# iacopo97/Multimodal-SAM-Adapter

Hardware: AMD Instinct MI355X
Metric: images/sec encoder fwd @1024x1024 RGB+LiDAR ViT-L (higher is better)
Workload: dtype split-operand MFMA: fp16 hi + e5m2 cross terms (h8c / h8 planes, ViT / interaction / up-conv GEMMs) fp16 hi/lo pairs x3 (TwinConvNeXt: f3 planes) and bf16 hi/lo x3 (neck, head); attention blocks with the rel-pos terms fused: every contraction on one fp16 MFMA (q, k, v, P rounded to fp16) in the bloc

## Files before the change

### include/mmsa.h

```cpp
#ifndef MMSA_H
#define MMSA_H
#include <stddef.h>
#include <stdint.h>
#ifdef __cplusplus
extern "C" {
#endif

#ifdef MMSA_BUILDING_LIBRARY
typedef hipStream_t mmsa_stream_t;
#else
typedef void* mmsa_stream_t;
#endif

#include "mmsa_version.h"
int mmsa_version(void);
const char* mmsa_last_error(void);

int mmsa_debug_poison_lds(unsigned pattern, mmsa_stream_t stream);
int mmsa_event_create(void** ev);
int mmsa_event_record(void* ev, mmsa_stream_t stream);
int mmsa_event_elapsed_ms(void* start, void* stop, float* ms);
int mmsa_event_destroy(void* ev);

enum { MMSA_ACT_NONE = 0, MMSA_ACT_GELU = 1, MMSA_ACT_RELU = 2, MMSA_ACT_RELU6 = 3, MMSA_ACT_HSWISH = 4, MMSA_ACT_SIGMOID = 5 };

enum { MMSA_DT_F32 = 0, MMSA_DT_F16 = 1, MMSA_DT_F64 = 2 };

enum { MMSA_FMT_B3 = 0, MMSA_FMT_H8 = 1, MMSA_FMT_H8C = 2, MMSA_FMT_F3 = 3, MMSA_FMT_W8 = 4  };

int mmsa_ms_deform_attn_forward(const void* value, const int64_t* spatial_shapes, const int64_t* level_start_index,
                                const void* sampling_loc, const void* attn_weight, void* out, int batch,
                                int spatial_size, int num_heads, int channels, int num_levels, int num_query,
                                int num_point, int im2col_step, int dtype, mmsa_stream_t stream);

int mmsa_ms_deform_attn_backward(const void* value, const int64_t* spatial_shapes, const int64_t* level_start_index,
                                 const void* sampling_loc, const void* attn_weight, const void* grad_output,
                                 void* grad_value, void* grad_sampling_loc, void* grad_attn_weight, int batch,
                                 int spatial_size, int num_heads, int channels, int num_levels, int num_query,
                                 int num_point, int im2col_step, int dtype, mmsa_stream_t stream);

int mmsa_msda_fused(const float* value, const int64_t* spatial_shapes, const int64_t* level_start_index,
                    const float* raw, long ldraw, const float* ref_points, float* out, long ldo,
                    uint16_t* out_planes, long ldop , int out_fmt , int batch,
                    int spatial_size, int num_heads, int channels, int num_levels, int num_query, int num_point,
                    float* clamp_max , mmsa_stream_t stream);

int mmsa_msda_fused_planes(const uint16_t* value_planes, long ldvp, int lo_bytes, const int64_t* spatial_shapes, const int64_t* level_start_index,
                           const float* raw, long ldraw, const float* ref_points, float* out, long ldo,
                           uint16_t* out_planes, long ldop, int out_fmt, int batch,
                           int spatial_size, int num_heads, int channels, int num_levels, int num_query, int num_point,
                           float* clamp_max, mmsa_stream_t stream);

int mmsa_rowstats_finalize(const float* rowstats, int rows, int strips, int D, float eps, float* mean_rstd, mmsa_stream_t stream);

int mmsa_zero_bytes(void* p, size_t bytes, mmsa_stream_t stream);
int mmsa_gemm_split3(const float* A, const uint16_t* Ap, long lda, long strideA,
                     const uint16_t* Wp, long strideW,
                     const float* bias, long strideBias, const float* colscale, const float* resid, long ldr,
                     long strideR, int resid_mod, float beta, float* C, long ldc, long strideC,
                     uint16_t* Cp, long ldcp, long strideCp, int M, int N, int K,
                     int batch, int act, float alpha, int out_mode, int ps_H, int ps_W, int ps_C, int fmt, int cp_fmt,
                     int max_grid, float* rowstats_out, const float* rownorm_mean_rstd, const float* rownorm_colsum, int flavour,
                     float* clamp_max , mmsa_stream_t stream);

int mmsa_convnext_mlp_fused(const uint16_t* Ap, long lda, long strideA, const uint16_t* W1p, long strideW1, const uint16_t* W2p,
                            long strideW2, const float* b1, const float* b2, const float* gamma, float* x, long ldx, long strideX,
                            int M, int C, int batch, int max_grid, int fmt,
                            float* clamp_max , mmsa_stream_t stream);

int mmsa_split_planes(const float* src, long ld, int rows, int cols, int cols_pad, uint16_t* planes, int kind,
                      float* clamp_max , mmsa_stream_t stream);

int mmsa_attention(const float* qkv, long ldq, const float* qkv_bias, const float* rp, float* out, long ldo, int B,
                   int H, int W, int heads, int head_dim, int window_size, float scale, mmsa_stream_t stream);
int mmsa_attention_planes(const uint16_t* qkv_planes, long ldq, const uint16_t* bias_planes, const float* rp,
                          uint16_t* out_planes, long ldo, int B, int H, int W, int heads, int head_dim,
                          int window_size, float scale, int out_fmt ,
                          int v_fmt ,
                          float* max_abs_logit , mmsa_stream_t stream);

int mmsa_relpos_bias(const float* qkv, long ldq, const float* Rh, const float* Rw, float* rp, int B, int H, int W,
                     int heads, int head_dim, int window_size, mmsa_stream_t stream);
int mmsa_relpos_bias_planes(const uint16_t* qkv_planes, long ldq, const float* Rh, const float* Rw,
                            float* rp, int B, int H, int W, int heads, int head_dim, int window_size, mmsa_stream_t stream);

int mmsa_layernorm_rows(const float* x, long ldx, const float* w, const float* b, float eps, float* y, long ldy,
                        float* y2, long ldy2, uint16_t* y_planes, long ldp ,
                        int rows, int C, int map_mode, int map_H, int map_W, int group_rows, long w_gstride, long y_gcol,
                        int y_wrap, int plane_fmt , float* clamp_max ,
                        mmsa_stream_t stream);

int mmsa_colstats(const float* x, long ldx, long strideB, const float* wrow, int B, int HW, int C, double* out,
                  int out_is_zero , mmsa_stream_t stream);

int mmsa_ffrm_finalize(const double* stats, int B, int HW, int C, float mean_w, float mean_b, const float* Wc,
                       const float* gn_w, const float* gn_b, float* mean_o, float* rstd_o, float* mult_o,
                       float* scratch , mmsa_stream_t stream);
int mmsa_lnhw_apply(const float* x, long ldx, const float* mean, const float* rstd, const float* mult, const float* w,
                    const float* bias, float* y, long ldy, int B, int HW, int C, mmsa_stream_t stream);

int mmsa_dwconv_nhwc(const float* x, long ldx, long xstrideB, const float* w, const float* bias, float* y, long ldy,
                     long ystrideB, uint16_t* y_planes, long ldp, long pstrideB , int planes_fmt ,
                     int B, int H, int W, int C, int k, int act,
                     int imgs_per_group ,
                     float* rowstats ,
                     float* clamp_max , mmsa_stream_t stream);
int mmsa_gconv_nhwc(const float* x, long ldx, const float* w, const float* bias, float* y, long ldy, int B, int H,
                    int W, int G, int cin_g, int cout_g, int k, int act, mmsa_stream_t stream);
int mmsa_gfe_qkv_conv(const float* x, long ldx, const float* w, float* y, long ldy, int B, int H, int W, int G, int cin_g, int cout_g,
                      int* covered, mmsa_stream_t stream);
int mmsa_dwpair_gate(const float* x, long ldx, const float* w, float* y, long ldy, uint16_t* y_planes, long ldp, int B, int H,
                     int W, int C, mmsa_stream_t stream);
int mmsa_im2col_nchw(const float* x, int B, int Ctot, int c0, int Cin, int H, int W, int p, float* out, int Kpad,
                     mmsa_stream_t stream);

long mmsa_gram_tn_scratch_bytes(int B, int P, int c);
int mmsa_gram_tn(const float* X, long ldx, const float* Y, long ldy, long strideB, double* G , int B, int P, int c,
                 int nblk, void* scratch, long scratch_bytes, mmsa_stream_t stream);
int mmsa_chanattn_build(const double* G, const double* sq, long sq_strideB, const double* sk, long sk_strideB,
                        const float* temp, const float* Wp, uint16_t* planes , int B, int c, int cpad,
                        int heads, mmsa_stream_t stream);
int mmsa_gffm_build(const double* E, uint16_t* x_planes, uint16_t* y_planes , int B, int c,
                    int cpad, mmsa_stream_t stream);
int mmsa_gelu_gate(const float* x, long ldx, float* y, long ldy, long rows, int C, mmsa_stream_t stream);
int mmsa_pool_hw(const float* z, long ldz, float* out, long ldo, int B, int H, int W, int C, mmsa_stream_t stream);
int mmsa_ca_apply(const float* z, long ldz, const float* att, long lda, float* out, long ldo,
                  uint16_t* out_planes, long ldp , int B, int H, int W, int C, mmsa_stream_t stream);

int mmsa_tail_fuse(const float* cmap, long ldc, long cstrideB, const float* xtok, long ldx, const float* bn_scale,
                   const float* bn_shift, float* out, uint16_t* out_planes , long ldp,
                   int B, int Hc, int Wc, int Hx, int Wx, int C, mmsa_stream_t stream);

int mmsa_global_attention_planes(const uint16_t* qkv_planes, long ldq, const uint16_t* bias_planes, const uint16_t* relpos_planes,
                                 uint16_t* out_planes, long ldo, int B, int H, int W, int heads, int head_dim, float scale,
                                 int out_fmt , int v_fmt ,
                                 float* max_abs_logit , mmsa_stream_t stream);

int mmsa_window_attention_planes(const uint16_t* qkv_planes, long ldq, const uint16_t* bias_planes,
                                 const uint16_t* relpos_planes, const uint16_t* selector, uint16_t* out_planes, long ldo, int B, int H, int W,
                                 int heads, int head_dim, int window_size, float scale, int out_fmt ,
                                 int v_fmt , float* max_abs_logit , mmsa_stream_t stream);

int mmsa_nchw_to_planes(const float* src, long strideB, uint16_t* planes, long ldp, int B, int C, long HW,
                        mmsa_stream_t stream);
int mmsa_head_fuse(const float* z0, const float* z1, int H1, int W1, const float* z2, int H2, int W2, const float* z3,
                   int H3, int W3, long ld, const float* bn_scale, const float* bn_shift, uint16_t* planes, long ldp,
                   float* out32, long ldo, int B, int H, int W, int C, int act, mmsa_stream_t stream);
int mmsa_tokens_to_nchw(const float* src, long ld, float* dst, int B, long HW, int C, mmsa_stream_t stream);

int mmsa_bilinear_accum_nchw(const float* src, long src_strideB, int B, int C, int hs, int ws, float* dst, int Hd, int Wd, int y0, int x0,
                             int hc, int wc, float* count, int accumulate, mmsa_stream_t stream);
int mmsa_div_count_nchw(float* x, const float* count, int B, int C, long HW, mmsa_stream_t stream);
int mmsa_argmax_nchw(const float* x, unsigned char* out, int B, int C, long HW, mmsa_stream_t stream);
int mmsa_crop_batch_nchw(const float* src, int B, int C, int H, int W, const int* windows, int n, float* dst, int hc, int wc,
                         mmsa_stream_t stream);
int mmsa_slide_argmax(const float* logits, int n, int C, int hs, int ws, const int* windows, unsigned char* out, int B, int H, int W,
                      int hc, int wc, int* uncovered, mmsa_stream_t stream);
int mmsa_slide_argmax_resized(const float* logits, int n, int C, int hs, int ws, const int* windows, unsigned char* out, int B, int H, int W,
                              int hc, int wc, int Hd, int Wd, int Hcut, int Wcut, int* uncovered, mmsa_stream_t stream);

int mmsa_softmax_flip_accum_nchw(const float* logits, float* acc, int B, int C, int H, int W, int flip, int accumulate, int finish_div, mmsa_stream_t stream);
int mmsa_aug_argmax(const float* const* logits, const int* views, int A, int C, const int* windows, const int* windows_host, int total,
                    unsigned char* out, int B, int Ho, int Wo, int* uncovered, mmsa_stream_t stream);

int mmsa_argmax_max_nchw(const float* x, unsigned char* out, float* maxval, int B, int C, long HW, mmsa_stream_t stream);
int mmsa_slide_argmax_conf(const float* logits, int n, int C, int hs, int ws, const int* windows, unsigned char* out, float* conf, int B, int H, int W,
                           int hc, int wc, int* uncovered, mmsa_stream_t stream);
int mmsa_slide_argmax_resized_conf(const float* logits, int n, int C, int hs, int ws, const int* windows, unsigned char* out, float* conf, int B, int H,
                                   int W, int hc, int wc, int Hd, int Wd, int Hcut, int Wcut, int* uncovered, mmsa_stream_t stream);
int mmsa_aug_argmax_conf(const float* const* logits, const int* views, int A, int C, const int* windows, const int* windows_host, int total,
                         unsigned char* out, float* conf, int B, int Ho, int Wo, int* uncovered, mmsa_stream_t stream);

enum { MMSA_PRE_U8 = 0, MMSA_PRE_F32 = 1 };
int mmsa_preprocess_nhwc(const void* src0, int dtype0, const void* src1, int dtype1, int B, int Hs, int Ws, const float* mean,
                         const float* sinv, const int* div255, const int* swap, const float* pad_val, float* dst, int H, int W,
                         mmsa_stream_t stream);
int mmsa_preprocess_crops(const void* src0, int dtype0, const void* src1, int dtype1, int B, int Hs, int Ws, const float* mean,
                          const float* sinv, const int* div255, const int* swap, const float* pad_val, int H, int W, const int* windows,
                          int n, float* dst, int hc, int wc, mmsa_stream_t stream);
int mmsa_preprocess_resize_nhwc(const void* src0, int dtype0, const void* src1, int dtype1, int B, int Hs, int Ws, const float* mean,
                                const float* sinv, const int* div255, const int* swap, const float* pad_val, float* dst, int H, int W,
                                int Hr, int Wr, const int* xofs, const void* xcoef, const int* yofs, const void* ycoef, int fixed_point,
                                mmsa_stream_t stream);
int mmsa_preprocess_resize_crops(const void* src0, int dtype0, const void* src1, int dtype1, int B, int Hs, int Ws, const float* mean,
                                 const float* sinv, const int* div255, const int* swap, const float* pad_val, int H, int W, const int* windows,
                                 int n, float* dst, int hc, int wc, int Hr, int Wr, const int* xofs, const void* xcoef, const int* yofs,
                                 const void* ycoef, int fixed_point, mmsa_stream_t stream);

int mmsa_eval_confusion_u8(const unsigned char* pred, const unsigned char* label, int B, int H, int W, int Hl, int Wl, const unsigned char* lut,
                           int C, const int* ymap, const int* xmap, const int* slots, int n_slots, int64_t* counts, mmsa_stream_t stream);
int mmsa_slide_argmax_eval(const float* logits, int n, int C, int hs, int ws, const int* windows, unsigned char* out, int B, int H, int W,
                           int hc, int wc, int* uncovered, const unsigned char* label, int Hl, int Wl, const unsigned char* lut, const int* ymap,
                           const int* xmap, const int* slots, int n_slots, int64_t* counts, mmsa_stream_t stream);

int mmsa_eval_calibration(const unsigned char* pred, const float* conf, const unsigned char* label, int B, int H, int W, int Hl, int Wl,
                          const unsigned char* lut, int C, const int* ymap, const int* xmap, const int* slots, int n_slots, int bins, int64_t* cal,
                          mmsa_stream_t stream);

int mmsa_eval_selective(const unsigned char* pred, const float* conf, const unsigned char* label, int B, int H, int W, int Hl, int Wl,
                        const unsigned char* lut, int C, const int* ymap, const int* xmap, const int* slots, int n_slots, int bins, int64_t* counts,
                        mmsa_stream_t stream);
int mmsa_abstain_u8(const unsigned char* pred, const float* conf, long n, int bins, int min_bin, unsigned char* out, mmsa_stream_t stream);

int mmsa_slide_argmax_conf_t(const float* logits, int n, int C, int hs, int ws, const int* windows, unsigned char* out, float* conf, int B, int H, int W,
                             int hc, int wc, int* uncovered, float inv_temperature, mmsa_stream_t stream);
int mmsa_slide_argmax_resized_conf_t(const float* logits, int n, int C, int hs, int ws, const int* windows, unsigned char* out, float* conf, int B, int H,
                                     int W, int hc, int wc, int Hd, int Wd, int Hcut, int Wcut, int* uncovered, float inv_temperature, mmsa_stream_t stream);
int mmsa_softmax_flip_accum_nchw_t(const float* logits, float* acc, int B, int C, int H, int W, int flip, int accumulate, int finish_div,
                                   float inv_temperature, mmsa_stream_t stream);
int mmsa_temperature_sweep_nchw(const float* logits, const unsigned char* label, int B, int C, int H, int W, int Hl, int Wl, const unsigned char* lut,
                                const int* ymap, const int* xmap, const int* slots, int n_slots, const float* inv_temperatures, int J, int bins,
                                int64_t* sweep, mmsa_stream_t stream);

int mmsa_render_u8(const unsigned char* pred, long pred_image_stride, long pred_row_stride, int B, int h, int w, const unsigned* palette, int npal,
                   int palette_reverse, const unsigned char* src, int Hs, int Ws, int src_reverse, double opacity, double one_minus_opacity,
                   unsigned char* out, mmsa_stream_t stream);
int mmsa_render_denorm_f32(const unsigned char* pred, long pred_image_stride, long pred_row_stride, int B, int h, int w, const unsigned* palette, int npal,
                           int palette_reverse, const float* src, int Cs, int Hs, int Ws, const float* mean, const float* std, int to_rgb, int mul255,
                           double opacity, double one_minus_opacity, unsigned char* out, mmsa_stream_t stream);

#ifdef __cplusplus
}
#endif
#endif
```

### multimodal-sam-adapter_amd/csrc/gemm_h8c.hip

```cpp
#include "common.h"
#include "gemm_h8c_shared.h"

#define HC_H_UNIT 49152
#define HC_L_UNIT 24576
#define HC_LDS_H(i_) ((i_) * HC_H_UNIT)
#define HC_LDS_L(i_) (2 * HC_H_UNIT + (i_) * (HC_L_UNIT + 16384))
#define HC_LDS_TOTAL (2 * HC_H_UNIT + 2 * HC_L_UNIT + 16384)

#ifdef HC_EPI_STAMP
__device__ unsigned long long g_hc_estamps[8 * 16];
extern "C" int mmsa_debug_epi_stamps(unsigned long long* host_out) { return (int)hipMemcpyFromSymbol(host_out, HIP_SYMBOL(g_hc_estamps), sizeof(g_hc_estamps)); }
#define EPI_STAMP(i_) { if (estamp_on_) { __builtin_amdgcn_sched_barrier(0); et_[i_] = __builtin_readcyclecounter(); __builtin_amdgcn_sched_barrier(0); } }
#define EPI_STAMP_WAIT() { if (estamp_on_) asm volatile("s_waitcnt vmcnt(0)" ::: "memory"); }
#else
#define EPI_STAMP(i_)
#define EPI_STAMP_WAIT()
#endif
template <bool GEN, int ACT>
__global__ __launch_bounds__(512, 1) void gemm_h8c_kernel(GemmV2Args a) {
  constexpr bool PP = true;
  constexpr bool EPI_UNROLL = ACT >= 0;
  constexpr int V2_BM = 256;
  constexpr int V2_NST = 3;
  extern __shared__ __attribute__((aligned(16))) unsigned char smem[];
  const int tid = threadIdx.x, lane = tid & 63;
  const int wave = __builtin_amdgcn_readfirstlane(tid >> 6);
  const int wm = wave >> 1, wn = wave & 1, grp = wave >> 2;
  const int l15 = lane & 15, g = lane >> 4;
  const int K = a.K;
  const int np = K >> 6;
  const bool ni4 = true;
  const int swid = 64;
  const int G = gridDim.x;
  int rb = blockIdx.x;
  V2_XCD_REMAP(rb, G)
  const int my_tiles = (a.ntiles - rb + G - 1) / G;
  if (my_tiles <= 0) return;
  V2_SLACK_STAGGER(a, rb, G)
  const int total = my_tiles * np;

  H8C_DMA_LANE();
  const int lds_ha = wave * 32 * 128, lds_hw = 32768 + wave * 16 * 128;
  const int lds_la = wave * 2048, lds_lw = 16384 + wave * 1024;
  const unsigned ldaB = (unsigned)(a.lda * 2), ldwB = (unsigned)(a.ldw * 2);
  const unsigned K2 = (unsigned)K * 2u, K4 = (unsigned)K * 4u;
  H8C_A_LANE_HI();
  const unsigned LW_E = (unsigned)(drow >> 1) * ldwB + (unsigned)(drow & 1) * K2 + dpiece, LW_O = LW_E ^ 64u;
  H8C_A_LANE_LO();
  const unsigned LLW = (unsigned)drow * ldwB + K4 + lq;

  const unsigned char *hA, *hW, *lA, *lW;
  int h_m0 = 0, h_n0 = 0, l_m0 = 0, l_n0 = 0;
  bool h_edge = false, l_edge = false;
  int hp_tile = rb, hp_p = 0, hp_j = 0, lp_tile = rb, lp_p = 0, lp_j = 0;
#define HC_SET_H(t_)                                                                                        \
  { int bz_; H8C_TILE(t_, 256, bz_, h_m0, h_n0)                                                             \
    hA = reinterpret_cast<const unsigned char*>(a.Ap + (long)bz_ * a.strideA + (long)(h_m0 >> 1) * a.lda);  \
    hW = reinterpret_cast<const unsigned char*>(a.Wp + (long)bz_ * a.strideW + (long)(h_n0 >> 1) * a.ldw);  \
    h_edge = h_m0 + 256 > a.M || h_n0 + 128 > a.N; }
#define HC_SET_L(t_)                                                                                        \
  { int bz_; H8C_TILE(t_, 256, bz_, l_m0, l_n0)                                                             \
    lA = reinterpret_cast<const unsigned char*>(a.Ap + (long)bz_ * a.strideA + (long)(l_m0 >> 1) * a.lda);  \
    lW = reinterpret_cast<const unsigned char*>(a.Wp + (long)bz_ * a.strideW + (long)(l_n0 >> 1) * a.ldw);  \
    l_edge = l_m0 + 256 > a.M || l_n0 + 128 > a.N; }
  HC_SET_H(hp_tile) HC_SET_L(lp_tile)
#define HC_H_ISSUE_FAST()                                                                                   \
  { unsigned char* d_ = smem + HC_LDS_H(hp_j & 1);                                                          \
    const unsigned char* sa_ = hA + (long)hp_p * 128 + (unsigned long)((unsigned)(wave * 16) * ldaB);       \
    const unsigned char* sw_ = hW + (long)hp_p * 128 + (unsigned long)((unsigned)(wave * 8) * ldwB);        \
    H8C_A_HI_FAST(sa_, d_)                                                                                  \
    GLDS16(sw_ + LW_E, d_ + lds_hw); GLDS16(sw_ + 4u * ldwB + LW_O, d_ + lds_hw + 1024); }
#define HC_L_ISSUE_FAST()                                                                                   \
  { unsigned char* d_ = smem + HC_LDS_L(lp_j & 1);                                                          \
    const unsigned char* sa_ = lA + (long)lp_p * 128 + (unsigned long)((unsigned)(wave * 16) * ldaB);       \
    const unsigned char* sw_ = lW + (long)lp_p * 128 + (unsigned long)((unsigned)(wave * 8) * ldwB);        \
    H8C_A_LO_FAST(sa_, d_)                                                                                  \
    GLDS16(sw_ + LLW, d_ + lds_lw); }
#define HC_H_ISSUE()                                                                                        \
  if (!h_edge) HC_H_ISSUE_FAST() else {                                                                     \
    unsigned char* d_ = smem + HC_LDS_H(hp_j & 1); const long ko_ = (long)hp_p * 128;                       \
    const int ab_ = h_m0 + wave * 32 + drow, wb_ = h_n0 + wave * 16 + drow;                                  \
    H8C_A_HI_EDGE(hA + ko_, ab_, h_m0, d_)                                                                  \
    GLDS16(hW + ko_ + (unsigned long)(H8C_HOFF(min(wb_, a.N - 1), h_n0, ldwB) + dpiece), d_ + lds_hw);       \
    GLDS16(hW + ko_ + (unsigned long)(H8C_HOFF(min(wb_ + 8, a.N - 1), h_n0, ldwB) + (dpiece ^ 64)), d_ + lds_hw + 1024); }
#define HC_H_ADVANCE() { ++hp_j; if (++hp_p == np) { hp_p = 0; hp_tile += G; if (hp_j < total) HC_SET_H(hp_tile) } }
#define HC_L_ISSUE()                                                                                        \
  if (!l_edge) HC_L_ISSUE_FAST() else {                                                                     \
    unsigned char* d_ = smem + HC_LDS_L(lp_j & 1); const long ko_ = (long)lp_p * 128;                       \
    const int aj_ = (l_m0 >> 1) + wave * 16 + drow, wj_ = (l_n0 >> 1) + wave * 8 + drow;                     \
    GLDS16(lA + ko_ + (unsigned long)H8C_A_LO_OFF(aj_, l_m0), d_ + lds_la);                                  \
    GLDS16(lA + ko_ + (unsigned long)H8C_A_LO_OFF(aj_ + 8, l_m0), d_ + lds_la + 1024);                       \
    GLDS16(lW + ko_ + (unsigned long)((unsigned)(min(wj_, (a.N - 1) >> 1) - (l_n0 >> 1)) * ldwB + K4 + lq), d_ + lds_lw); }
#define HC_L_ADVANCE() { ++lp_j; if (++lp_p == np) { lp_p = 0; lp_tile += G; if (lp_j < total) HC_SET_L(lp_tile) } }

  H8C_FRAG_HI();
  const int fha = (wm * 64) * 128, fhw = 32768 + (wn * 64) * 128;
  H8C_FRAG_LO();
  const int fla = (wm * 4) * 1024 + lo_off, flw = 16384 + (wn * 4) * 1024 + lo_off;

  f32x4 acc[4][4];
  H8C_ZERO_ACC()
  h8c_u4 ah0[4], ah1[4], wh0[4], wh1[4];
  mx_v8i opA[4], opW[4];

  HC_H_ISSUE() HC_H_ADVANCE()
  if (total > 1) { HC_H_ISSUE() HC_H_ADVANCE() }
  HC_L_ISSUE() HC_L_ADVANCE()
  H8C_WAIT(0);
  __builtin_amdgcn_s_barrier();

  int j = 0, tile = rb, nowait = 0;
#define HC_PAIR(FAST_)                                                                                                \
  {                                                                                                                   \
    const unsigned char* hb = smem + HC_LDS_H(j & 1);                                                                 \
    const unsigned char* lb = smem + HC_LDS_L(j & 1);                                                                 \
    const bool last = !(FAST_) && p == np - 1;                                                                        \
    const bool tail = !(FAST_) && j + 2 >= total;                                                                     \
    const bool skipw = !(FAST_) && nowait > 0;                                                                        \
                                                                                     \
    _Pragma("unroll") for (int i = 0; i < 4; ++i) {                                                                   \
      ah0[i] = *reinterpret_cast<const h8c_u4*>(hb + fha + i * 2048 + frag0);                                         \
      ah1[i] = *reinterpret_cast<const h8c_u4*>(hb + fha + i * 2048 + frag1);                                         \
    }                                                                                                                 \
    _Pragma("unroll") for (int i = 0; i < 4; ++i) {                                                                   \
      wh0[i] = *reinterpret_cast<const h8c_u4*>(hb + fhw + i * 2048 + frag0);                                         \
      wh1[i] = *reinterpret_cast<const h8c_u4*>(hb + fhw + i * 2048 + frag1);                                         \
    }                                                                                                                 \
    H8C_SB();                                                                                                         \
    const bool do_l = (FAST_) || lp_j < total;                                                                        \
    if (FAST_) { HC_L_ISSUE_FAST() } else if (do_l) { HC_L_ISSUE() }                                                   \
    H8C_SB();                                                                                                         \
    asm volatile("s_waitcnt lgkmcnt(0)" ::: "memory");                                                                \
    if (FAST_) H8C_WAIT(9); else if (tail) H8C_WAIT(0); else if (!skipw) H8C_WAIT(9);                                 \
    H8C_BAR()                                                                                                         \
     \
    _Pragma("unroll") for (int ni = 0; ni < 4; ++ni)                                                                  \
      _Pragma("unroll") for (int mi = 0; mi < 4; ++mi)                                                                \
        acc[ni][mi] = __builtin_amdgcn_mfma_f32_16x16x32_f16(__builtin_bit_cast(mx_h8, wh0[ni]), __builtin_bit_cast(mx_h8, ah0[mi]), acc[ni][mi], 0, 0, 0); \
    H8C_SB();                                                                                                         \
    _Pragma("unroll") for (int ni = 0; ni < 4; ++ni)                                                                  \
      _Pragma("unroll") for (int mi = 0; mi < 4; ++mi)                                                                \
        acc[ni][mi] = __builtin_amdgcn_mfma_f32_16x16x32_f16(__builtin_bit_cast(mx_h8, wh1[ni]), __builtin_bit_cast(mx_h8, ah1[mi]), acc[ni][mi], 0, 0, 0); \
    H8C_SB();                                                                                                         \
    if (FAST_) H8C_WAIT(9); else if (tail) H8C_WAIT(0); else if (!skipw) H8C_WAIT(9);                                 \
    H8C_BAR()                                                                                                         \
                                                             \
    H8C_FP8_TUPLES(lb)                                                                                                \
    H8C_SB();                                                                                                         \
    const bool do_h = (FAST_) || hp_j < total;                                                                        \
    if (FAST_) { HC_H_ISSUE_FAST() } else if (do_h) { HC_H_ISSUE() }                                                   \
    H8C_SB();                                                                                                         \
    asm volatile("s_waitcnt lgkmcnt(0)" ::: "memory");                                                                \
    if (FAST_) H8C_WAIT(9); else if (tail) H8C_WAIT(0); else if (!skipw) H8C_WAIT(9);                                 \
    H8C_BAR()                                                                                                         \
                                              \
    _Pragma("unroll") for (int ni = 0; ni < 4; ++ni)                                                                  \
      _Pragma("unroll") for (int mi = 0; mi < 4; ++mi)                                                                \
        acc[ni][mi] = __builtin_amdgcn_mfma_scale_f32_16x16x128_f8f6f4(opW[ni], opA[mi], acc[ni][mi], 1, 1, 0, MMSA_H8_MFMA_SCALE, 0, 0x7f7f7f7f); \
    H8C_SB();                                                                                                         \
     \
     \
    if (FAST_) { ++lp_j; ++lp_p; ++hp_j; ++hp_p; } else { if (do_l) HC_L_ADVANCE() if (do_h) HC_H_ADVANCE() }          \
    H8C_SB();                                                                                                         \
    if (FAST_) H8C_WAIT(9); else if (tail || last) H8C_WAIT(0); else if (!skipw) H8C_WAIT(9);                         \
    H8C_BAR()                                                                                                         \
    if (!(FAST_)) nowait = 0;                                                                                         \
    ++j;                                                                                                              \
  }

  for (int tdone = 0; tdone < my_tiles; ++tdone) {
    if (grp) H8C_BAR()
    bool interior;
    { int bz_, m0_, n0_; H8C_TILE(tile, 256, bz_, m0_, n0_) interior = m0_ + 256 <= a.M && n0_ + 128 <= a.N; }
    int p = 0;
    HC_PAIR(0)
    ++p;
    if (interior) {
#pragma unroll 1
      for (; p < np - 2; ++p) HC_PAIR(1)
      if (hp_p == np) { hp_p = 0; hp_tile += G; if (hp_j < total) HC_SET_H(hp_tile) }
    }
#pragma unroll 1
    for (; p < np; ++p) HC_PAIR(0)
    if (!grp) H8C_BAR()
    if (V2_DBG(a) == 2) H8C_NO_EPILOGUE() else {
#ifdef HC_EPI_STAMP
      unsigned long long et_[9] = {0, 0, 0, 0, 0, 0, 0, 0, 0};
      const bool estamp_on_ = blockIdx.x == 0 && tdone == 1;
#endif
      EPI_STAMP(0)
#define EPI_STAGING_BASE (smem + (((j - 1) & 1) ? 2 * HC_H_UNIT + HC_L_UNIT : 2 * HC_H_UNIT))
#include "gemm_v2_epilogue.inc"
      EPI_STAMP(7)
#ifdef HC_EPI_STAMP
      asm volatile("s_waitcnt lgkmcnt(0)" ::: "memory");
      H8C_BAR()
      EPI_STAMP(8)
      if (estamp_on_ && (threadIdx.x & 63) == 0) {
#pragma unroll
        for (int q_ = 0; q_ < 9; ++q_) g_hc_estamps[wave * 16 + q_] = et_[q_];
      }
#endif
    }
    asm volatile("s_waitcnt lgkmcnt(0)" ::: "memory");
    H8C_BAR()
    tile += G;
  }
}

int mmsa_gemm_h8c_dispatch(const GemmV2Args& a, int grid, bool gen, int act, hipStream_t stream) {
  static MmsaPerDevice per_dev_ = {};
  (void)mmsa_per_device(per_dev_, [] {
#define HC_ATTR(GEN_, ACT_) (void)hipFuncSetAttribute((const void*)gemm_h8c_kernel<GEN_, ACT_>, hipFuncAttributeMaxDynamicSharedMemorySize, HC_LDS_TOTAL);
    V2_EPI_TABLE(HC_ATTR)
#undef HC_ATTR
  });
#define HC_LAUNCH(GEN_, ACT_) if (v2_epi_serves(gen, act, GEN_, ACT_)) hipLaunchKernelGGL((gemm_h8c_kernel<GEN_, ACT_>), dim3(grid), dim3(512), HC_LDS_TOTAL, stream, a);
  V2_EPI_TABLE(HC_LAUNCH)
#undef HC_LAUNCH
  MMSA_CHECK_LAUNCH("gemm_split3(h8c)");
  return MMSA_OK;
}
```

### multimodal-sam-adapter_amd/csrc/gemm_v2.hip

```cpp
#include "common.h"
#include "gemm_v2_shared.h"
template <bool GEN, int ACT, bool PP, int NW, int FMT>
__global__ __launch_bounds__(NW * 64, NW == 4 ? 2 : 1) void gemm_v2_kernel(GemmV2Args a) {
  static_assert(NW == 8 || (NW == 4 && !PP), "4-wave workgroups run the in-phase main loop");
  static_assert(FMT == MMSA_FMT_B3 || (PP && NW == 8), "the h8 and f3 operand formats run on the ping-pong kernel");
  constexpr bool EPI_UNROLL = ACT >= 0;
  constexpr int V2_BM = NW * 32;
  constexpr int V2_A_BYTES = V2_BM * 128;
  constexpr int V2_STAGE = V2_A_BYTES + V2_W_BYTES;
  constexpr int V2_NST = NW == 8 ? 3 : 2;
  constexpr int WROWS = V2_BN / NW;
  constexpr int NDMA = 4 + WROWS / 8;
  extern __shared__ __attribute__((aligned(16))) unsigned char smem[];
  const int tid = threadIdx.x;
  const int lane = tid & 63;
  const int wave = __builtin_amdgcn_readfirstlane(tid >> 6);
  const int wm = wave >> 1, wn = wave & 1;
  const int grp = wave >> 2;
  const int l15 = lane & 15, g = lane >> 4;
  const int K = a.K;
  const int nk = K / V2_BK;

  const int G = gridDim.x;
  int rb = blockIdx.x;
  V2_XCD_REMAP(rb, G)
  const int my_tiles = (a.ntiles - rb + G - 1) / G;
  if (my_tiles <= 0) return;
  V2_SLACK_STAGGER(a, rb, G)
  CLK_SAMPLE(0)
  const int total = my_tiles * nk;

  const int drow = lane >> 3;
  const int dpiece = ((lane & 7) ^ (drow >> 1)) * 8;
  const int lds_a = wave * 32 * 128;
  const int lds_w = wave * WROWS * 128;
  const unsigned char *gA, *gW;
  unsigned oa0, oa1, oa2, oa3, ow0, ow1, ow2 = 0, ow3 = 0;
#define SA(i_, ko_) reinterpret_cast<const unsigned short*>(gA + (long)(ko_) * 2 + (unsigned long)oa##i_)
#define SW(i_, ko_) reinterpret_cast<const unsigned short*>(gW + (long)(ko_) * 2 + (unsigned long)ow##i_)

#define SET_TILE_SRC(tile_)                                                      \
  do {                                                                           \
    const int t_ = (tile_);                                                      \
    const int per_b_ = a.nbm * a.nbn;                                            \
    const int bz_ = t_ / per_b_;                                                 \
    const int r_ = t_ - bz_ * per_b_;                                            \
    int tmi_, tni_;                                                              \
    V2_TILE_MN(r_, tmi_, tni_);                                                  \
    const int m0_ = tmi_ * V2_BM, n0_ = tni_ * a.bn;                             \
    const int ab_ = m0_ + wave * 32 + drow, wb_ = n0_ + wave * WROWS + drow;     \
    gA = reinterpret_cast<const unsigned char*>(a.Ap + (long)bz_ * a.strideA + (long)m0_ * a.lda);  \
    gW = reinterpret_cast<const unsigned char*>(a.Wp + (long)bz_ * a.strideW + (long)n0_ * a.ldw);  \
    oa0 = (unsigned)((min(ab_, a.M - 1) - m0_) * (int)a.lda + dpiece) * 2u;           \
    oa1 = (unsigned)((min(ab_ + 8, a.M - 1) - m0_) * (int)a.lda + (dpiece ^ 32)) * 2u;  \
    oa2 = (unsigned)((min(ab_ + 16, a.M - 1) - m0_) * (int)a.lda + dpiece) * 2u;      \
    oa3 = (unsigned)((min(ab_ + 24, a.M - 1) - m0_) * (int)a.lda + (dpiece ^ 32)) * 2u; \
    ow0 = (unsigned)((min(wb_, a.N - 1) - n0_) * (int)a.ldw + dpiece) * 2u;           \
    ow1 = (unsigned)((min(wb_ + 8, a.N - 1) - n0_) * (int)a.ldw + (dpiece ^ 32)) * 2u;  \
    if constexpr (NW == 4) {                                                     \
      ow2 = (unsigned)((min(wb_ + 16, a.N - 1) - n0_) * (int)a.ldw + dpiece) * 2u;    \
      ow3 = (unsigned)((min(wb_ + 24, a.N - 1) - n0_) * (int)a.ldw + (dpiece ^ 32)) * 2u; \
    }                                                                            \
    if (V2_DBG(a) == 4 || V2_DBG(a) == 5) { oa1 = oa2 = oa3 = oa0; gW = gA; ow0 = ow1 = oa0; }    \
  } while (0)

#define ISSUE_DMA(kt_, st_)                                                       \
  do {                                                                            \
    unsigned char* sb_ = smem + (st_) * V2_STAGE;                                 \
    const int ko_ = V2_DBG(a) == 3 ? 0 : (kt_) * 64;    \
    GLDS16(SA(0, ko_), sb_ + lds_a);                                               \
    GLDS16(SA(1, ko_), sb_ + lds_a + 1024);                                        \
    GLDS16(SA(2, ko_), sb_ + lds_a + 2048);                                        \
    GLDS16(SA(3, ko_), sb_ + lds_a + 3072);                                        \
    GLDS16(SW(0, ko_), sb_ + V2_A_BYTES + lds_w);                                  \
    GLDS16(SW(1, ko_), sb_ + V2_A_BYTES + lds_w + 1024);                           \
    if constexpr (NW == 4) {                                                      \
      GLDS16(SW(2, ko_), sb_ + V2_A_BYTES + lds_w + 2048);                         \
      GLDS16(SW(3, ko_), sb_ + V2_A_BYTES + lds_w + 3072);                         \
    }                                                                             \
  } while (0)

  f32x4 acc[4][4];
  mx_v8i opA[4] = {}, opW[4] = {};
#pragma unroll
  for (int i = 0; i < 4; ++i)
#pragma unroll
    for (int j = 0; j < 4; ++j) acc[i][j] = (f32x4){0.f, 0.f, 0.f, 0.f};

  const int fslot = g ^ ((l15 >> 1) & 7);
  const int frag_hi = l15 * 128 + fslot * 16;
  const int frag_lo = l15 * 128 + (fslot ^ 4) * 16;
  const int fa = (wm * 64) * 128;
  const bool ni4 = a.bn == V2_BN;
  const int swid = ni4 ? 64 : 48;
  const int fw = V2_A_BYTES + (wn * swid) * 128;

  int pf_tile = rb, pf_kt = 0, pf_st = 0, pf_j = 0;
  SET_TILE_SRC(pf_tile);
#define PREFETCH_NEXT()                                     \
  do {                                                      \
    ISSUE_DMA(pf_kt, pf_st);                                \
    pf_st = pf_st == V2_NST - 1 ? 0 : pf_st + 1;            \
    ++pf_j;                                                 \
    if (++pf_kt == nk) {                                    \
      pf_kt = 0;                                            \
      pf_tile += G;                                         \
      if (pf_j < total) SET_TILE_SRC(pf_tile);              \
    }                                                       \
  } while (0)
  PREFETCH_NEXT();
  if (V2_NST == 3 && total > 1) PREFETCH_NEXT();

  int st = 0, tile = rb, nowait = 0, j = 0;
  if constexpr (PP) {
    if (total > 1) asm volatile("s_waitcnt vmcnt(6)" ::: "memory");
    else asm volatile("s_waitcnt vmcnt(0)" ::: "memory");
    __builtin_amdgcn_s_barrier();
  }

#define MX_SET(dst_, src_, par_)                                                                            \
  { const uint4 u_ = __builtin_bit_cast(uint4, src_);                                                       \
    if ((par_) == 0) { dst_[0] = (int)u_.x; dst_[1] = (int)u_.y; dst_[2] = (int)u_.z; dst_[3] = (int)u_.w; }  \
    else { dst_[4] = (int)u_.x; dst_[5] = (int)u_.y; dst_[6] = (int)u_.z; dst_[7] = (int)u_.w; } }
#define MFMA_FP8_ALL(NI4_, DEFER_)                                                                          \
  if constexpr (FMT == MMSA_FMT_H8) {                                                                       \
    if (MXPAR && V2_FP8_FIRST && !V2_EXP_NO_FP8) {                                                          \
      _Pragma("unroll") for (int ni = 0; ni < 4; ++ni)                                                      \
        if (ni < 3 || (NI4_)) {                                                                             \
          _Pragma("unroll") for (int mi = 0; mi < 4; ++mi)                                                  \
              acc[ni][mi] = __builtin_amdgcn_mfma_scale_f32_16x16x128_f8f6f4(opW[ni], opA[mi], acc[ni][mi], 1, 1, 0, MMSA_H8_MFMA_SCALE, 0, 0x7f7f7f7f); \
        }                                                                                                   \
      __builtin_amdgcn_sched_barrier(0);                                                                    \
    }                                                                                                       \
  }
#define MFMA_CHUNK(ni)                                                                                      \
  if constexpr (FMT == MMSA_FMT_H8) {                                                                       \
    _Pragma("unroll") for (int mi = 0; mi < 4; ++mi) {                                                      \
      acc[ni][mi] = __builtin_amdgcn_mfma_f32_16x16x32_f16(__builtin_bit_cast(mx_h8, wh[ni]), __builtin_bit_cast(mx_h8, ah[mi]), acc[ni][mi], 0, 0, 0); \
      if (MXPAR && !V2_FP8_FIRST && !V2_EXP_NO_FP8) acc[ni][mi] = __builtin_amdgcn_mfma_scale_f32_16x16x128_f8f6f4(opW[ni], opA[mi], acc[ni][mi], 1, 1, 0, MMSA_H8_MFMA_SCALE, 0, 0x7f7f7f7f); \
    }                                                                                                       \
  } else {                                                                                                  \
    _Pragma("unroll") for (int mi = 0; mi < 4; ++mi) {                                                      \
      if constexpr (FMT == MMSA_FMT_F3) {                    \
        acc[ni][mi] = __builtin_amdgcn_mfma_f32_16x16x32_f16(__builtin_bit_cast(mx_h8, wl[ni]), __builtin_bit_cast(mx_h8, ah[mi]), acc[ni][mi], 0, 0, 0); \
        acc[ni][mi] = __builtin_amdgcn_mfma_f32_16x16x32_f16(__builtin_bit_cast(mx_h8, wh[ni]), __builtin_bit_cast(mx_h8, al[mi]), acc[ni][mi], 0, 0, 0); \
        acc[ni][mi] = __builtin_amdgcn_mfma_f32_16x16x32_f16(__builtin_bit_cast(mx_h8, wh[ni]), __builtin_bit_cast(mx_h8, ah[mi]), acc[ni][mi], 0, 0, 0); \
      } else {                                                                                              \
      acc[ni][mi] = __builtin_amdgcn_mfma_f32_16x16x32_bf16(wl[ni], ah[mi], acc[ni][mi], 0, 0, 0);          \
      acc[ni][mi] = __builtin_amdgcn_mfma_f32_16x16x32_bf16(wh[ni], al[mi], acc[ni][mi], 0, 0, 0);          \
      acc[ni][mi] = __builtin_amdgcn_mfma_f32_16x16x32_bf16(wh[ni], ah[mi], acc[ni][mi], 0, 0, 0);          \
      }                                                                                                     \
    }                                                                                                       \
  }
#define K_STEP()                                                                                            \
  {                                                                                                         \
    if (nowait > 0) --nowait;                                                                               \
    else if (V2_NST == 3 && j + 1 < total) asm volatile("s_waitcnt vmcnt(6)" ::: "memory");                  \
    else asm volatile("s_waitcnt vmcnt(0)" ::: "memory");                                                   \
    __builtin_amdgcn_s_barrier();                                                                           \
    const bool do_pf = pf_j < total;                                                                        \
    unsigned char* pfb = smem + pf_st * V2_STAGE;                                                           \
    const int pko = V2_DBG(a) == 3 ? 0 : pf_kt * 64;                                                          \
    const unsigned char* base = smem + st * V2_STAGE;                                                       \
    bf16x8 ah[4], al[4], wh[4], wl[4];                                                                      \
    _Pragma("unroll") for (int i = 0; i < 4; ++i) {                                                         \
      ah[i] = *reinterpret_cast<const bf16x8*>(base + fa + i * 2048 + frag_hi);                             \
      al[i] = *reinterpret_cast<const bf16x8*>(base + fa + i * 2048 + frag_lo);                             \
    }                                                                                                       \
    _Pragma("unroll") for (int i = 0; i < 4; ++i) {                                                         \
      if (i < 3 || ni4) {                                                                                   \
        wh[i] = *reinterpret_cast<const bf16x8*>(base + fw + i * 2048 + frag_hi);                           \
        wl[i] = *reinterpret_cast<const bf16x8*>(base + fw + i * 2048 + frag_lo);                           \
      }                                                                                                     \
    }                                                                                                       \
    __builtin_amdgcn_sched_barrier(0);                                                                      \
    MFMA_CHUNK(0)                                                                                           \
    __builtin_amdgcn_sched_barrier(0);                                                                      \
    if (do_pf) { GLDS16(SA(0, pko), pfb + lds_a); GLDS16(SA(1, pko), pfb + lds_a + 1024); }                   \
    __builtin_amdgcn_sched_barrier(0);                                                                      \
    MFMA_CHUNK(1)                                                                                           \
    __builtin_amdgcn_sched_barrier(0);                                                                      \
    if (do_pf) { GLDS16(SA(2, pko), pfb + lds_a + 2048); GLDS16(SA(3, pko), pfb + lds_a + 3072); }            \
    __builtin_amdgcn_sched_barrier(0);                                                                      \
    MFMA_CHUNK(2)                                                                                           \
    __builtin_amdgcn_sched_barrier(0);                                                                      \
    if (do_pf) { GLDS16(SW(0, pko), pfb + V2_A_BYTES + lds_w); GLDS16(SW(1, pko), pfb + V2_A_BYTES + lds_w + 1024); } \
    if constexpr (NW == 4) { if (do_pf) { GLDS16(SW(2, pko), pfb + V2_A_BYTES + lds_w + 2048); GLDS16(SW(3, pko), pfb + V2_A_BYTES + lds_w + 3072); } } \
    __builtin_amdgcn_sched_barrier(0);                                                                      \
    if (ni4) { MFMA_CHUNK(3) }                                                                              \
    __builtin_amdgcn_sched_barrier(0);                                                                      \
    if (do_pf) {    \
      pf_st = pf_st == V2_NST - 1 ? 0 : pf_st + 1;                                                          \
      ++pf_j;                                                                                               \
      if (++pf_kt == nk) {                                                                                  \
        pf_kt = 0;                                                                                          \
        pf_tile += G;                                                                                       \
        if (pf_j < total) SET_TILE_SRC(pf_tile);                                                            \
      }                                                                                                     \
    }                                                                                                       \
    st = st == V2_NST - 1 ? 0 : st + 1;                                                                     \
    ++j;                                                                                                    \
  }

#ifdef V2_STAMP
#define STAMP_DECL() unsigned long long tt[9]; const bool stamp_on = blockIdx.x == 0 && tdone == 0 && kt >= 8 && kt < 12;
#define STAMP_STORE() if (stamp_on && lane == 0) { _Pragma("unroll") for (int q_ = 0; q_ < 9; ++q_) g_v2_stamps[(wave * 4 + (kt - 8)) * 10 + q_] = tt[q_]; }
#else
#define STAMP_DECL()
#define STAMP_STORE()
#endif
#define V2_PP_NR 6
#define V2_STR_(x) #x
#define V2_STR(x) V2_STR_(x)
#define PP_WAIT(cnt_)                                                                                       \
  {                                                                                                         \
    if (nowait > 0) --nowait;                                                                               \
    else if (j + 2 < total) asm volatile("s_waitcnt vmcnt(" V2_STR(cnt_) ")" ::: "memory");                  \
    else asm volatile("s_waitcnt vmcnt(0)" ::: "memory");                                                   \
  }
#define PP_PIECE(i_)                                                                                        \
  if (do_pf) {                                                                                              \
    if ((i_) == 0) GLDS16(SA(0, pko), pfb + lds_a);                                                          \
    if ((i_) == 1) GLDS16(SA(1, pko), pfb + lds_a + 1024);                                                   \
    if ((i_) == 2) GLDS16(SA(2, pko), pfb + lds_a + 2048);                                                   \
    if ((i_) == 3) GLDS16(SA(3, pko), pfb + lds_a + 3072);                                                   \
    if ((i_) == 4) GLDS16(SW(0, pko), pfb + V2_A_BYTES + lds_w);                                             \
    if ((i_) == 5) GLDS16(SW(1, pko), pfb + V2_A_BYTES + lds_w + 1024);                                      \
  }
#define MX_FILL() if constexpr (FMT == MMSA_FMT_H8) { _Pragma("unroll") for (int i = 0; i < 4; ++i) { MX_SET(opA[i], al[i], MXPAR) MX_SET(opW[i], wl[i], MXPAR) } }
#ifdef V2_KABL
#define KABL(x_) (V2_DBG(a) >= 64 && ((V2_DBG(a) >> ((x_) - 6)) & 1))
#define KABL_INIT() _Pragma("unroll") for (int i = 0; i < 4; ++i) { ah[i] = al[i] = wh[i] = wl[i] = __builtin_bit_cast(bf16x8, make_uint4(lane + i, 0x3c003c00u, lane, 0x3c003c00u)); }
#define KABL_UNDEF() _Pragma("unroll") for (int i = 0; i < 4; ++i) { asm volatile("" : "=v"(ah[i]), "=v"(al[i]), "=v"(wh[i]), "=v"(wl[i])); }
#else
#define KABL(x_) false
#define KABL_INIT()
#define KABL_UNDEF()
#endif
#define K_STEP_PP()                                                                                         \
  {                                                                                                         \
    const bool do_pf = pf_j < total && !KABL(8);                                                            \
    const bool last_k = kt == nk - 1;                                                                       \
    STAMP_DECL()                                                                                            \
    STAMP(0)                                                                                                \
    unsigned char* pfb = smem + pf_st * V2_STAGE;                                                           \
    const int pko = V2_DBG(a) >= 3 && V2_DBG(a) <= 5 ? 0 : pf_kt * 64;                                          \
    const unsigned char* base = smem + st * V2_STAGE;                                                       \
    bf16x8 ah[4], al[4], wh[4], wl[4];                                                                      \
    KABL_INIT()                                                                                             \
    if (!KABL(7)) _Pragma("unroll") for (int i = 0; i < 4; ++i) {                                           \
      ah[i] = *reinterpret_cast<const bf16x8*>(base + fa + i * 2048 + frag_hi);                             \
      al[i] = *reinterpret_cast<const bf16x8*>(base + fa + i * 2048 + frag_lo);                             \
    }                                                                                                       \
    if (!KABL(7)) _Pragma("unroll") for (int i = 0; i < 4; ++i) {                                           \
      if (i < 3 || ni4) {                                                                                   \
        wh[i] = *reinterpret_cast<const bf16x8*>(base + fw + i * 2048 + frag_hi);                           \
        wl[i] = *reinterpret_cast<const bf16x8*>(base + fw + i * 2048 + frag_lo);                           \
      }                                                                                                     \
    }                                                                                                       \
    MX_FILL()                                                                                               \
    __builtin_amdgcn_sched_barrier(0);                                                                      \
    STAMP(1)                                                                                                \
    _Pragma("unroll") for (int pi_ = 0; pi_ < V2_PP_NR; ++pi_) PP_PIECE(pi_)                                \
    __builtin_amdgcn_sched_barrier(0);                                                                      \
    STAMP(2)                                                                                                \
    asm volatile("s_waitcnt lgkmcnt(0)" ::: "memory");                                                      \
    STAMP(3)                                                                                                \
    if (grp && !last_k) PP_WAIT(V2_PP_NR)                                                                   \
    STAMP(4)                                                                                                \
    if (!KABL(9)) __builtin_amdgcn_s_barrier();                                                             \
    STAMP(5)                                                                                                \
    __builtin_amdgcn_sched_barrier(0);                                                                      \
    if (!KABL(6)) {                                                                                         \
    MFMA_FP8_ALL(ni4, !last_k)                                                                              \
    MFMA_CHUNK(0)                                                                                           \
    MFMA_CHUNK(1)                                                                                           \
    MFMA_CHUNK(2)                                                                                           \
    if (ni4) { MFMA_CHUNK(3) }                                                                              \
    }                                                                                                       \
    __builtin_amdgcn_sched_barrier(0);                                                                      \
    if (do_pf) {                                                                                            \
      pf_st = pf_st == 2 ? 0 : pf_st + 1;                                                                   \
      ++pf_j;                                                                                               \
      if (++pf_kt == nk) {                                                                                  \
        pf_kt = 0;                                                                                          \
        pf_tile += G;                                                                                       \
        if (pf_j < total) SET_TILE_SRC(pf_tile);                                                            \
      }                                                                                                     \
    }                                                                                                       \
    STAMP(6)                                                                                                \
    if (last_k) asm volatile("s_waitcnt vmcnt(0)" ::: "memory");                                            \
    else if (!grp) PP_WAIT(6)                                                                               \
    STAMP(7)                                                                                                \
    if (!KABL(9)) __builtin_amdgcn_s_barrier();                                                             \
    STAMP(8)                                                                                                \
    STAMP_STORE()                                                                                           \
    st = st == 2 ? 0 : st + 1;                                                                              \
    ++j;                                                                                                    \
  }

#define K_STEP_PP_FAST(NI4_)                                                                                \
  {                                                                                                         \
    unsigned char* pfb = smem + pf_st * V2_STAGE;                                                           \
    const int pko = pf_kt * 64;                                                                             \
    const unsigned char* base = smem + st * V2_STAGE;                                                       \
    bf16x8 ah[4], al[4], wh[4], wl[4];                                                                      \
    if (KABL(7)) { KABL_UNDEF() } else {                                                                    \
    _Pragma("unroll") for (int i = 0; i < 4; ++i) {                                                         \
      ah[i] = *reinterpret_cast<const bf16x8*>(base + fa + i * 2048 + frag_hi);                             \
      al[i] = *reinterpret_cast<const bf16x8*>(base + fa + i * 2048 + frag_lo);                             \
    }                                                                                                       \
    _Pragma("unroll") for (int i = 0; i < 4; ++i) {                                                         \
      if (i < 3 || NI4_) {                                                                                  \
        wh[i] = *reinterpret_cast<const bf16x8*>(base + fw + i * 2048 + frag_hi);                           \
        wl[i] = *reinterpret_cast<const bf16x8*>(base + fw + i * 2048 + frag_lo);                           \
      }                                                                                                     \
    }                                                                                                       \
    }                                                                                                       \
    MX_FILL()                                                                                               \
    __builtin_amdgcn_sched_barrier(0);                                                                      \
    if (!KABL(8)) {                                                                                         \
    GLDS16(SA(0, pko), pfb + lds_a);                                                                        \
    GLDS16(SA(1, pko), pfb + lds_a + 1024);                                                                 \
    GLDS16(SA(2, pko), pfb + lds_a + 2048);                                                                 \
    GLDS16(SA(3, pko), pfb + lds_a + 3072);                                                                 \
    GLDS16(SW(0, pko), pfb + V2_A_BYTES + lds_w);                                                           \
    GLDS16(SW(1, pko), pfb + V2_A_BYTES + lds_w + 1024);                                                    \
    }                                                                                                       \
    __builtin_amdgcn_sched_barrier(0);                                                                      \
    asm volatile("s_waitcnt lgkmcnt(0)" ::: "memory");                                                      \
    asm volatile("s_waitcnt vmcnt(6)" ::: "memory");                                                        \
    __builtin_amdgcn_s_barrier();                                                                           \
    ISTAMP(0)                                                                                               \
    __builtin_amdgcn_sched_barrier(0);                                                                      \
    if (!KABL(6)) {                                                                                         \
    MFMA_FP8_ALL(NI4_, true)                                                                                \
    MFMA_CHUNK(0)                                                                                           \
    MFMA_CHUNK(1)                                                                                           \
    MFMA_CHUNK(2)                                                                                           \
    if (NI4_) { MFMA_CHUNK(3) }                                                                             \
    }                                                                                                       \
    __builtin_amdgcn_sched_barrier(0);                                                                      \
    pf_st = pf_st == 2 ? 0 : pf_st + 1;                                                                     \
    ++pf_j;                                                                                                 \
    ++pf_kt;                                                                                                \
    asm volatile("s_waitcnt vmcnt(6)" ::: "memory");                                                        \
    __builtin_amdgcn_s_barrier();                                                                           \
    ISTAMP(1)                                                                                               \
    st = st == 2 ? 0 : st + 1;                                                                              \
    ++j;                                                                                                    \
  }
#ifdef V2_STAMP
#ifndef V2_ISTAMP_KT0
#define V2_ISTAMP_KT0 8
#endif
#define ISTAMP(h_) if (blockIdx.x == 0 && tdone == 0 && kt >= V2_ISTAMP_KT0 && kt < V2_ISTAMP_KT0 + 8 && (wave & 3) == 0 && lane == 0) g_v2_stamps[grp * 16 + (kt + MXPAR - V2_ISTAMP_KT0) * 2 + (h_)] = __builtin_readcyclecounter();
#else
#define ISTAMP(h_)
#endif

  for (int tdone = 0; tdone < my_tiles; ++tdone) {
    if constexpr (PP) {
      if (grp) __builtin_amdgcn_s_barrier();
      const bool fast_ok = V2_FAST_STEPS && nk >= 6 && (V2_DBG(a) < 3 || V2_DBG(a) == 10 || V2_DBG(a) >= 64) && (FMT != MMSA_FMT_H8 || ni4);
      const int kt_a = fast_ok ? 2 : nk, kt_b = fast_ok ? nk - 2 : nk;
      if constexpr (FMT == MMSA_FMT_H8) {
#pragma unroll 1
        for (int kt = 0; kt < kt_a; ++kt) {
#define MXPAR 0
          K_STEP_PP()
#undef MXPAR
          ++kt;
#define MXPAR 1
          K_STEP_PP()
#undef MXPAR
        }
#pragma unroll 1
        for (int kt = kt_a; kt < kt_b; kt += 2) {
#define MXPAR 0
          K_STEP_PP_FAST(true)
#undef MXPAR
#define MXPAR 1
          K_STEP_PP_FAST(true)
#undef MXPAR
        }
        if (fast_ok) {
          pf_kt = 0;
          pf_tile += G;
          if (pf_j < total) SET_TILE_SRC(pf_tile);
        }
#pragma unroll 1
        for (int kt = kt_b; kt < nk; ++kt) {
#define MXPAR 0
          K_STEP_PP()
#undef MXPAR
          ++kt;
#define MXPAR 1
          K_STEP_PP()
#undef MXPAR
        }
      } else {
#define MXPAR 0
#pragma unroll 1
        for (int kt = 0; kt < kt_a; ++kt) K_STEP_PP()
        if (ni4) {
#pragma unroll 1
          for (int kt = kt_a; kt < kt_b; ++kt) K_STEP_PP_FAST(true)
        } else {
#pragma unroll 1
          for (int kt = kt_a; kt < kt_b; ++kt) K_STEP_PP_FAST(false)
        }
        if (fast_ok) {
          pf_kt = 0;
          pf_tile += G;
          if (pf_j < total) SET_TILE_SRC(pf_tile);
        }
#pragma unroll 1
        for (int kt = kt_b; kt < nk; ++kt) K_STEP_PP()
#undef MXPAR
      }
      if (!grp) __builtin_amdgcn_s_barrier();
    } else {
#define MXPAR 0
#pragma unroll 1
      for (int kt = 0; kt < nk; ++kt) K_STEP()
#undef MXPAR
    }
    const int st_cur = st == 0 ? V2_NST - 1 : st - 1;

    if (V2_DBG(a) == 2 || V2_DBG(a) == 5 || V2_DBG(a) >= 64) { tile += G; continue; }
#define EPI_STAGING_BASE (smem + st_cur * V2_STAGE)
#include "gemm_v2_epilogue.inc"
    if constexpr (PP) {
      asm volatile("s_waitcnt lgkmcnt(0)" ::: "memory");
      __builtin_amdgcn_s_barrier();
    }
    tile += G;
  }
  CLK_SAMPLE(2)
#undef K_STEP
#undef K_STEP_PP
#undef K_STEP_PP_FAST
#undef PP_WAIT
#undef PP_PIECE
#undef MFMA_CHUNK
#undef MFMA_FP8_ALL
}

int mmsa_gemm_h8c_dispatch(const GemmV2Args& a, int grid, bool gen, int act, hipStream_t stream);
int mmsa_gemm_h8c_w8_dispatch(const GemmV2Args& a, int grid, bool gen, int act, hipStream_t stream);
int mmsa_gemm_stream_try(const unsigned short* Ap, long lda, const unsigned short* Wp, const float* bias, const float* colscale, const float* resid, long ldr, float beta,
                         float* C, long ldc, unsigned short* Cp, long ldcp, int M, int N, int K, int batch, int act, float alpha, int out_mode, int resid_mod,
                         int fmt, int cp_fmt, int max_grid, const float* rs_out, const float* rn_mr, int flavour, float* clamp_max, hipStream_t stream);
int mmsa_gemm_h8c4_dispatch(const GemmV2Args& a, int grid, hipStream_t stream);

int mmsa_gemm_v2_launch(const unsigned short* Ap, long lda, long strideA,
                        const unsigned short* Wp, long strideW,
                        const float* bias, long strideBias, const float* colscale,
                        const float* resid, long ldr, long strideR, int resid_mod, float beta,
                        float* C, long ldc, long strideC,
                        unsigned short* Cp, long ldcp, long strideCp,
                        int M, int N, int K, int batch, int act, float alpha,
                        int out_mode, int ps_H, int ps_W, int ps_C, int fmt, int cp_fmt, int max_grid, hipStream_t stream,
                        float* rs_out, const float* rn_mr, const float* rn_cs, int flavour, float* clamp_max) {
  {
    const int rc_ = mmsa_gemm_stream_try(Ap, lda, Wp, bias, colscale, resid, ldr, beta, C, ldc, Cp, ldcp, M, N, K, batch, act, alpha, out_mode, resid_mod, fmt, cp_fmt,
                                         max_grid, rs_out, rn_mr, flavour, clamp_max, stream);
    if (rc_ != 0) return rc_ < 0 ? rc_ : MMSA_OK;
  }
  GemmV2Args a;
  a.clamp_max = clamp_max;
  MMSA_CHECK_ARG(!rs_out || (C && out_mode == 0 && resid_mod <= 0 && act == ACT_NONE && (N & 63) == 0 && (ldc & 3) == 0 && (!resid || (ldr & 3) == 0) && (!Cp || (ldcp & 3) == 0)),
                 "gemm(v2): row statistics need a plain fp32 output, no activation, N %% 64 == 0 (N=%d)", N);
  MMSA_CHECK_ARG(!rn_mr || (rn_cs && !resid && out_mode == 0 && resid_mod <= 0 && (N & 127) == 0 && ((((uintptr_t)bias) | ((uintptr_t)colscale) | ((uintptr_t)rn_cs)) & 15) == 0 && (strideBias & 3) == 0 &&
                            ((Cp && !C && (act == ACT_NONE || act == ACT_GELU || act == ACT_RELU)) ||
                             (C && !Cp && act == ACT_NONE && (M & 255) == 0 && !colscale && alpha == 1.0f && (ldc & 3) == 0 && (((uintptr_t)C) & 15) == 0))),
                 "gemm(v2): the row-normalising epilogue needs N %% 128 == 0 (N=%d), 16-byte aligned column vectors and either a planes-only output or a plain fp32 output with M %% 256 == 0 (M=%d), no activation / scale", N, M);
  a.rs_out = rs_out; a.rs_strips = N >> 6; a.rn_mr = rn_mr; a.rn_cs = rn_cs;
  a.Ap = Ap; a.lda = lda; a.strideA = strideA;
  a.Wp = Wp; a.strideW = strideW;
  const bool w8 = fmt == MMSA_FMT_W8;
  const bool h8c = fmt == MMSA_FMT_H8C || w8;
  MMSA_CHECK_ARG(!w8 || ((K & 127) == 0 && batch == 1), "gemm(v2): W8 weights need K %% 128 == 0 and one batch (K=%d, batch=%d)", K, batch);
  a.ldw = w8 ? K / 2 : h8c ? 3L * K : 2L * K;
  a.bias = bias; a.strideBias = strideBias; a.colscale = colscale;
  a.resid = resid; a.ldr = ldr; a.strideR = strideR; a.resid_mod = resid_mod; a.beta = beta;
  a.C = C; a.ldc = C ? ldc : 0; a.strideC = strideC;
  a.Cp = Cp; a.ldcp = Cp ? ldcp : 0; a.strideCp = strideCp;
  a.M = M; a.N = N; a.K = K; a.act = act; a.alpha = alpha;
  a.out_mode = out_mode; a.ps_H = ps_H; a.ps_W = ps_W; a.ps_C = ps_C;
  auto log2_exact = [](int v) { int s_ = -1; if (v > 0 && (v & (v - 1)) == 0) { s_ = 0; while ((1 << s_) < v) ++s_; } return s_; };
  a.ps_sw = log2_exact(ps_W); a.ps_sh = log2_exact(ps_H);
  a.cp_fmt = cp_fmt;
  const bool h8 = fmt == MMSA_FMT_H8 || h8c;
  MMSA_CHECK_ARG(!h8 || (K & 63) == 0, "gemm(v2): h8 operands need K %% 64 == 0 (K=%d)", K);
  MMSA_CHECK_ARG(flavour == 0 || flavour == 4 || flavour == 8, "gemm(v2): flavour %d (0 = by shape, 4, 8)", flavour);
  static MmsaPerDevice per_dev_ = {};
  const int num_cus = mmsa_per_device(per_dev_, [] {
#define V2_ATTR(GEN_, ACT_)                                                                                                   \
  (void)hipFuncSetAttribute((const void*)gemm_v2_kernel<GEN_, ACT_, false, 8, MMSA_FMT_B3>, hipFuncAttributeMaxDynamicSharedMemorySize, V2_LDS_BYTES(8)); \
  (void)hipFuncSetAttribute((const void*)gemm_v2_kernel<GEN_, ACT_, true, 8, MMSA_FMT_B3>, hipFuncAttributeMaxDynamicSharedMemorySize, V2_LDS_BYTES(8));  \
  (void)hipFuncSetAttribute((const void*)gemm_v2_kernel<GEN_, ACT_, true, 8, MMSA_FMT_H8>, hipFuncAttributeMaxDynamicSharedMemorySize, V2_LDS_BYTES(8));  \
  (void)hipFuncSetAttribute((const void*)gemm_v2_kernel<GEN_, ACT_, true, 8, MMSA_FMT_F3>, hipFuncAttributeMaxDynamicSharedMemorySize, V2_LDS_BYTES(8));  \
  (void)hipFuncSetAttribute((const void*)gemm_v2_kernel<GEN_, ACT_, false, 4, MMSA_FMT_B3>, hipFuncAttributeMaxDynamicSharedMemorySize, V2_LDS_BYTES(4));
    V2_EPI_TABLE(V2_ATTR)
#undef V2_ATTR
  });
  const int cus = (max_grid > 0 && max_grid < num_cus) ? max_grid : num_cus;
  const bool h8c4 = flavour == 4 && h8c && !w8 && out_mode == 0 && resid_mod <= 0 && act == ACT_NONE && M >= 128;
  const int nw = h8c4 ? 4 : (h8 || rs_out || rn_mr || fmt == MMSA_FMT_F3) ? 8 : flavour ? flavour : (K <= MMSA_KNOB("MMSA_GEMM_NW4_MAXK", 256) && max_grid <= 0 ? 4 : 8);
  const int bm = nw * 32, wg_per_cu = nw == 4 ? 2 : 1;
  a.nbm = cdiv(M, bm);
  a.bn = V2_BN;
  a.nbn = cdiv(N, V2_BN);
  a.ntiles = a.nbm * a.nbn * batch;
#ifdef MMSA_DEBUG_KNOBS
  a.debug = MMSA_KNOB("MMSA_GEMM_DEBUG", 0);
#endif
  if (!Cp && out_mode == 0 && resid_mod <= 0 && N >= 96 && N % 96 == 0 && !rs_out && !rn_mr && !h8c) {
    const bool no96 = MMSA_KNOB("MMSA_GEMM_NO96", 0) != 0;
    const int nbn96 = cdiv(N, 96);
    const long t96 = (long)a.nbm * nbn96 * batch;
    const int slots = cus * wg_per_cu;
    const double c128 = (double)cdiv(a.ntiles, slots), c96 = 0.75 * (double)cdiv(t96, slots);
    if (!no96 && c96 < c128 - 1e-9) {
      a.bn = 96;
      a.nbn = nbn96;
      a.ntiles = (int)t96;
    }
  }
  const bool rowmajor = MMSA_KNOB("MMSA_GEMM_ROWMAJOR", 0) != 0;
  a.tm = a.tn = 0;
  if (!rowmajor) {
    double best = 0.0;
    for (int tn = 1; tn <= 32; tn <<= 1) {
      const int tm = 32 / tn;
      if (a.nbn % tn != 0 || a.nbm % tm != 0) continue;
      const double cost = (double)(a.nbn / tn) * M + (double)(a.nbm / tm) * N;
      if (a.tm == 0 || cost < best) { best = cost; a.tm = tm; a.tn = tn; }
    }
  }
  const int slots_ = cus * wg_per_cu;
  const int rounds_ = cdiv(a.ntiles, slots_);
  int grid = cdiv(a.ntiles, rounds_);
  a.stagger = 0;
#ifndef MMSA_GEMM_STAGGER
#define MMSA_GEMM_STAGGER 0
#endif
  if (MMSA_GEMM_STAGGER && MMSA_KNOB("MMSA_GEMM_STAGGER", 1) && nw == 8 && rounds_ >= 2 && a.ntiles % slots_ != 0) {
    grid = slots_;
    a.stagger = h8c ? (K >> 6) * 3800 + 16000 : (K >> 5) * (fmt == MMSA_FMT_H8 ? 1700 : 1900) + 16000;
  }
  const bool gen = out_mode != 0 || resid_mod > 0;
  if (w8) return mmsa_gemm_h8c_w8_dispatch(a, grid, gen, act, stream);
  if (h8c4) return mmsa_gemm_h8c4_dispatch(a, grid, stream);
  if (h8c) return mmsa_gemm_h8c_dispatch(a, grid, gen, act, stream);
  const bool pp = MMSA_KNOB("MMSA_GEMM_PP", 1) != 0;
#define V2_LAUNCH(GEN_, ACT_)                                                                                              \
  if (v2_epi_serves(gen, act, GEN_, ACT_)) {                                                                               \
    if (fmt == MMSA_FMT_H8) hipLaunchKernelGGL((gemm_v2_kernel<GEN_, ACT_, true, 8, MMSA_FMT_H8>), dim3(grid), dim3(512), V2_LDS_BYTES(8), stream, a);          \
    else if (fmt == MMSA_FMT_F3) hipLaunchKernelGGL((gemm_v2_kernel<GEN_, ACT_, true, 8, MMSA_FMT_F3>), dim3(grid), dim3(512), V2_LDS_BYTES(8), stream, a);     \
    else if (nw == 4) hipLaunchKernelGGL((gemm_v2_kernel<GEN_, ACT_, false, 4, MMSA_FMT_B3>), dim3(grid), dim3(256), V2_LDS_BYTES(4), stream, a);     \
    else if (pp) hipLaunchKernelGGL((gemm_v2_kernel<GEN_, ACT_, true, 8, MMSA_FMT_B3>), dim3(grid), dim3(512), V2_LDS_BYTES(8), stream, a);     \
    else hipLaunchKernelGGL((gemm_v2_kernel<GEN_, ACT_, false, 8, MMSA_FMT_B3>), dim3(grid), dim3(512), V2_LDS_BYTES(8), stream, a);            \
  }
  V2_EPI_TABLE(V2_LAUNCH)
#undef V2_LAUNCH
  MMSA_CHECK_LAUNCH("gemm_split3(v2)");
  return MMSA_OK;
}
```

### multimodal-sam-adapter_amd/csrc/gemm_v2_shared.h

```cpp
#pragma once
#include "common.h"
#include <type_traits>
typedef __attribute__((ext_vector_type(8))) int mx_v8i;
typedef __attribute__((ext_vector_type(8))) _Float16 mx_h8;

struct GemmV2Args {
  const unsigned short* Ap; long lda; long strideA;
  const unsigned short* Wp; long strideW; long ldw;
  const float* bias; long strideBias;
  const float* colscale;
  const float* resid; long ldr; long strideR; int resid_mod; float beta;
  float* C; long ldc; long strideC;
  unsigned short* Cp; long ldcp; long strideCp;
  int M, N, K;
  int act; float alpha;
  int out_mode; int ps_H, ps_W, ps_C;
  int ps_sw, ps_sh;
  int nbm, nbn, ntiles;
  int tm, tn;
  int bn;
  int cp_fmt;
  float* rs_out; int rs_strips;
  const float* rn_mr; const float* rn_cs;
  float* clamp_max;
  int stagger;
#ifdef MMSA_DEBUG_KNOBS
  int debug;
#endif
};
#ifdef MMSA_DEBUG_KNOBS
#define V2_DBG(a_) ((a_).debug)
#else
#define V2_DBG(a_) 0
#endif

#define V2_BN 128
#define V2_BK 32
#define V2_W_BYTES (V2_BN * 128)
#define V2_LDS_BYTES(NW_) (((NW_) == 8 ? 3 : 2) * ((NW_) * 32 * 128 + V2_W_BYTES))
#ifndef V2_FP8_FIRST
#define V2_FP8_FIRST 1
#endif
#ifndef V2_EXP_NO_FP8
#define V2_EXP_NO_FP8 0
#endif
#ifndef V2_FAST_STEPS
#define V2_FAST_STEPS 1
#endif

#define V2_SLACK_STAGGER(a_, rb_, G_)                                                                       \
  if ((a_).stagger > 0) {                                                                                   \
    const int rem_ = (a_).ntiles % (G_);                                                                    \
    if (rem_ > 0 && (rb_) >= rem_) {                                                                        \
      const unsigned long long d_ = ((unsigned long long)(a_).stagger * (unsigned)((((rb_) - rem_) & 15) * 2 + 1)) >> 5;  \
      const unsigned long long t0_ = __builtin_readcyclecounter();                                          \
      while (__builtin_readcyclecounter() - t0_ < d_) __builtin_amdgcn_s_sleep(8);                          \
    }                                                                                                       \
  }

#define GLDS16(gptr, lptr)                                                                                  \
  __builtin_amdgcn_global_load_lds((const __attribute__((address_space(1))) void*)(gptr),                   \
                                   (__attribute__((address_space(3))) void*)(lptr), 16, 0, 0)

#ifdef V2_STAMP
__device__ unsigned long long g_v2_stamps[8 * 4 * 10 + 4];
extern "C" int mmsa_debug_stamps(unsigned long long* host_out) {
  return (int)hipMemcpyFromSymbol(host_out, HIP_SYMBOL(g_v2_stamps), sizeof(unsigned long long) * (8 * 4 * 10 + 4));
}
#define STAMP(i_) if (stamp_on) tt[i_] = __builtin_readcyclecounter();
#define CLK_SAMPLE(o_) if (blockIdx.x == 0 && threadIdx.x == 0) { g_v2_stamps[320 + (o_)] = __builtin_readcyclecounter(); g_v2_stamps[321 + (o_)] = __builtin_amdgcn_s_memrealtime(); }
#else
#define CLK_SAMPLE(o_)
#define STAMP(i_)
#endif

#define V2_XCD_REMAP(rb_, G_) { const int xcd = rb_ & 7, q = (G_) >> 3, r = (G_) & 7; rb_ = (xcd < r ? xcd * (q + 1) : r * (q + 1) + (xcd - r) * q) + (rb_ >> 3); }

#define V2_EPI_TABLE(X_) X_(false, ACT_NONE) X_(false, ACT_GELU) X_(false, ACT_RELU) X_(false, -1) X_(true, -1) X_(true, ACT_NONE)
inline bool v2_epi_serves(bool gen, int act, bool GEN, int ACT) {
  bool listed = false;
#define V2_EPI_LISTED_(GEN_, ACT_) listed = listed || (gen == (GEN_) && act == (ACT_));
  V2_EPI_TABLE(V2_EPI_LISTED_)
#undef V2_EPI_LISTED_
  return gen == GEN && (listed ? act == ACT : ACT == -1);
}

#define V2_TILE_MN(r_, mi_, ni_)                                                 \
  do {                                                                           \
    if (a.tm > 0) {                                                              \
      const int blk_ = (r_) >> 5, loc_ = (r_) & 31;                              \
      const int bpr_ = a.nbn / a.tn;                                             \
      const int bi_ = blk_ / bpr_, bj_ = blk_ - bi_ * bpr_;                      \
      const int lm_ = loc_ / a.tn;                                               \
      mi_ = bi_ * a.tm + lm_;                                                    \
      ni_ = bj_ * a.tn + (loc_ - lm_ * a.tn);                                    \
    } else {                                                                     \
      mi_ = (r_) / a.nbn;                                                        \
      ni_ = (r_) - mi_ * a.nbn;                                                  \
    }                                                                            \
  } while (0)
```

### multimodal-sam-adapter_amd/mmsa/backbone.py

```python
import contextlib
import functools
import math
import os

import torch
import torch.nn as nn

from . import ops, pack
from .pack import PackPlan, _linear_resize_rows, fold_gfe_qkv
from .params import CONVNEXT_ARCH, build_tree

_VIT_DEFAULTS = dict(img_size=1024, patch_size=16, in_chans=3, embed_dim=1024, depth=24, mlp_ratio=4.0,
                     qkv_bias=True, use_abs_pos=True, use_rel_pos=True, rel_pos_zero_init=True, window_size=14,
                     global_attn_indexes=[5, 11, 17, 23], pretrained_size=1024, fix=False)


class OperandRangeError(RuntimeError):
    """A forward converted a value beyond the range of an fp16-based operand format (the clamp watch word, include/mmsa.h) and nothing is left to
    re-route: `range_fallback` is off, or the value is a q / k / v (or a qkv bias / rel-pos table entry) beyond +-65504 inside the attention kernels,
    which read fp16-based planes in every mode.  The outputs of that forward are invalid."""


class Workspace:

    def __init__(self, device):
        self.device = device
        self.bufs = {}
        self.zeroed = set()

    def get(self, name, rows, cols, dtype=torch.float32, zero=False):
        n = rows * cols
        b = self.bufs.get(name)
        if b is None or b.numel() < n or b.dtype != dtype:
            b = torch.zeros(n, dtype=dtype, device=self.device) if zero else torch.empty(n, dtype=dtype, device=self.device)
            self.bufs[name] = b
        if zero:
            self.zeroed.add(name)
        return b[:n].view(rows, cols)

    def poison(self):
        for name, b in self.bufs.items():
            if name in self.zeroed:
                continue
            if b.dtype in (torch.float32, torch.float64):
                b.fill_(float("nan"))
            elif b.dtype == torch.int16:
                b.fill_(0x7fc0)

    def planes(self, name, rows, cols, zero=False, fmt=ops.FMT_B3):
        tr, tc, cp = ops.planes_shape(rows, cols, fmt)
        return ops.Planes(self.get(name + ".pl", tr, tc, torch.int16, zero or cp != cols), rows, cols, cp, fmt)

    def nbytes(self):
        return sum(b.numel() * b.element_size() for b in self.bufs.values())


class _Tagged:

    def __init__(self, ws, tag):
        self.ws, self.tag = ws, tag

    def get(self, name, *a, **k):
        return self.ws.get(self.tag + name, *a, **k)

    def planes(self, name, *a, **k):
        return self.ws.planes(self.tag + name, *a, **k)

    @property
    def device(self):
        return self.ws.device

    def poison(self):
        return self.ws.poison()

    def nbytes(self):
        return self.ws.nbytes()


class SAMAdapterbimodalMixModNewInTwinConvNEW(nn.Module):
    def __init__(self, pretrain_size=1024, num_heads=12, conv_inplane=64, n_points=4,
                 modalities_name=['rgb', 'depth', 'lidar', 'event'], modalities_ch=[3, 3, 3, 1],
                 deform_num_heads=6, init_values=0., gamma_init_values=0., interaction_indexes=None, with_cffn=True,
                 cffn_ratio=0.25, deform_ratio=1.0, add_vit_feature=True, pretrained=None,
                 use_extra_extractor=True, with_cp=True, drop_path_rate=0.4, drop_rate=0., drop_multimodal_path=0.2,
                 arch='base', checkpoint='check', *args, **kwargs):
        super().__init__()
        vit = dict(_VIT_DEFAULTS)
        for k in list(kwargs):
            if k in vit:
                vit[k] = kwargs.pop(k)
        if 'rgb' not in modalities_name or len(modalities_name) != 2:
            raise NotImplementedError("mmsa: the MI355X path implements the bimodal (rgb + one auxiliary modality) encoder; "
                                      f"got modalities_name={modalities_name}")
        if list(modalities_ch) != [3, 3]:
            raise NotImplementedError("mmsa: TwinConvNeXt takes two 3-channel streams (TC:296-316)")
        if not vit["use_abs_pos"]:
            raise NotImplementedError("mmsa: use_abs_pos=False is not a working configuration of the reference either (its forward interpolates "
                                      "self.pos_embed unconditionally, BK:276, which is None then: IE:113-114)")
        if interaction_indexes is None:
            raise ValueError("interaction_indexes is required")
        D = vit["embed_dim"]
        self.cfg = dict(embed_dim=D, depth=vit["depth"], num_heads=num_heads, mlp_ratio=vit["mlp_ratio"],
                        patch_size=vit["patch_size"], pretrained_size=vit["pretrained_size"], img_size=vit["img_size"],
                        window_size=vit["window_size"], global_attn_indexes=list(vit["global_attn_indexes"]),
                        conv_inplane=conv_inplane, n_points=n_points, deform_num_heads=deform_num_heads,
                        init_values=init_values, interaction_indexes=[list(i) for i in interaction_indexes],
                        cffn_ratio=cffn_ratio, deform_ratio=deform_ratio, arch=arch,
                        use_extra_extractor=bool(use_extra_extractor), with_cffn=bool(with_cffn), add_vit_feature=bool(add_vit_feature),
                        use_rel_pos=bool(vit["use_rel_pos"]), qkv_bias=bool(vit["qkv_bias"]))
        a = CONVNEXT_ARCH[arch] if isinstance(arch, str) else arch
        self.depths, self.channels = list(a["depths"]), list(a["channels"])
        if [2 * c for c in self.channels] != [conv_inplane * m for m in (4, 8, 16, 32)]:
            raise ValueError("conv_inplane*{4,8,16,32} must equal twice the ConvNeXt stage widths (AM:894-907)")
        for c in self.channels:
            if c % 32 != 0:
                raise ValueError("ConvNeXt stage widths must be multiples of 32 (groups=32 convs, GroupNorm(32))")
        hd = D // num_heads
        if D % num_heads or ops.pad32(hd) not in (32, 64, 96):
            raise NotImplementedError(f"mmsa: attention head_dim {hd} not supported by the HIP kernels (up to 96; widths that are "
                                      "not multiples of 32 run zero-padded per head, e.g. ViT-H's 80 as 96)")
        self.img_size = vit["img_size"]
        self.embed_dim = D
        self.interaction_indexes = self.cfg["interaction_indexes"]
        self.modalities_name, self.modalities_ch = modalities_name, modalities_ch
        self.in_ch_im = 3
        build_tree(self, self.cfg)
        self._packed = None
        self._ws = None
        self._taps = None
        self.register_load_state_dict_post_hook(lambda m, _: m.invalidate())
        self.init_weights(pretrained)
        if isinstance(checkpoint, str) and checkpoint not in ("", "check"):
            local = checkpoint if os.path.isfile(checkpoint) else os.environ.get("MMSA_CONVNEXT_CKPT", "")
            if os.path.isfile(local):
                self.load_convnext_checkpoint(local)
            else:
                import warnings
                warnings.warn(f"mmsa: ConvNeXt checkpoint '{checkpoint}' is not a local file and MMSA_CONVNEXT_CKPT names no mirror: "
                              "TwinConvNeXt keeps its random initialisation (the reference downloads and loads it, TC:382-443)")
        self.eval()

    def init_weights(self, pretrained=None):
        if isinstance(pretrained, str):
            from .checkpoint import load_pretrained
            self._pretrained_report = load_pretrained(self, pretrained)

    def load_convnext_checkpoint(self, path):
        ck = torch.load(path, map_location="cpu")
        sd = ck.get("state_dict", ck.get("model", ck)) if isinstance(ck, dict) else ck
        sd = {(k[9:] if k.startswith("backbone.") else k): v for k, v in sd.items()}
        if list(sd.keys())[0].startswith("module."):
            sd = {k[7:]: v for k, v in sd.items()}
        own = self.state_dict()
        loaded, new = [], {}
        for k, v in sd.items():
            dot = k.find(".")
            for sfx in ("_x", "_y"):
                nk = (k[:dot] + sfx + k[dot:]) if dot != -1 else k + sfx
                full = "spm.twin_conv." + nk
                if full in own:
                    new[full] = v
                    loaded.append(full)
        self.load_state_dict(new, strict=False)
        return loaded

    def invalidate(self):
        self._packed = None
        self._wide_range = False
        self._carry_modes = None
        self._inter_pairs = set()

    def train(self, mode=True):
        if mode:
            raise NotImplementedError("mmsa: the MI355X backbone implements the inference forward path only")
        return super().train(False)

    H8_DEFAULT = ("vit", "inter", "up", "attnv")
    attention_precision = "auto"

    range_fallback = True

    inter_follow_blocks = True

    fp8_weights = False

    fuse_gfe_qkv = True

    def _inter_pair_set(self):
        return set(getattr(self, "_inter_pairs", ()) or ())

    def _interaction_of_block(self, bi):
        for i, idx in enumerate(self.interaction_indexes):
            if idx[0] <= bi <= idx[-1]:
                return i
        return None

    def _wide(self):
        return bool(getattr(self, "_wide_range", False))

    def _h8_sites(self):
        return PackPlan.of(self).h8_sites

    @contextlib.contextmanager
    def chain(self, index):
        base = self._ws
        if base is None:
            raise RuntimeError("mmsa: run one forward() before opening a chain (workspace not created yet)")
        self._ws = _Tagged(base, f"chain{index}_")
        try:
            yield self
        finally:
            self._ws = base

    @torch.no_grad()
    def effective_state_dict(self):
        sd = self.state_dict()
        out = type(sd)((k, v.detach().clone()) for k, v in sd.items())
        plan = PackPlan.of(self)
        if not plan.fp8_weights:
            return out
        fold = plan.fold_ln
        dev = torch.device("cuda", torch.cuda.current_device()) if torch.cuda.is_available() else torch.device("cpu")
        for i in range(self.cfg["depth"]):
            b = f"blocks.{i}."
            for key, ln in (("attn.qkv.weight", "norm1.weight"), ("attn.proj.weight", None), ("mlp.lin1.weight", "norm2.weight"), ("mlp.lin2.weight", None)):
                w = sd[b + key].detach().to(dev, torch.float32)
                lnw = sd[b + ln].detach().to(dev, torch.float32) if (fold and ln) else None
                out[b + key] = pack.fp8_effective(w, lnw)[1].to(sd[b + key].device, sd[b + key].dtype)
        return out

    def _fold_ln_wanted(self):
        return PackPlan.of(self).fold_ln

    def _pack(self, dev):
        return pack.pack(self, dev)

    _hd_true = property(lambda self: self.cfg["embed_dim"] // self.cfg["num_heads"])
    _hd_pad = property(lambda self: ops.pad32(self._hd_true))

    @torch.no_grad()
    def _geometry(self, H, W, dev):
        pk = self._packed
        key = (H, W)
        if key in pk["geom"]:
            return pk["geom"][key]
        cfg = self.cfg
        p = cfg["patch_size"]
        Hp, Wp = H // p, W // p
        g = {}
        g["pos"] = _bicubic_resize(pk["pos_src"][0], Hp, Wp).reshape(Hp * Wp, -1).contiguous()
        ss1 = torch.tensor([(H // 8, W // 8), (H // 16, W // 16), (H // 32, W // 32)], dtype=torch.int64)
        ss2 = torch.tensor([(H // 16, W // 16)], dtype=torch.int64)
        g["ss1"], g["ss2"] = ss1.to(dev), ss2.to(dev)
        g["lsi1"] = torch.cat((ss1.new_zeros(1), ss1.prod(1).cumsum(0)[:-1])).to(dev)
        g["lsi2"] = ss2.new_zeros(1).to(dev)
        g["ref1"] = _ref_points([(H // 16, W // 16)]).to(dev)
        g["ref2"] = _ref_points([(H // 8, W // 8), (H // 16, W // 16), (H // 32, W // 32)]).to(dev)
        g["rel"] = []
        ws = cfg["window_size"]
        hd_ = self._hd_pad
        g["relg"] = []
        for blk in pk["blocks"]:
            relg = None
            if blk["ws"]:
                g["rel"].append((_rel_table(ws, blk["rph"]), _rel_table(ws, blk["rpw"])) if blk.get("relp") is None else None)
            elif hd_ == 64 and Wp == 64 and Hp <= 64 and Hp % 4 == 0:
                th = blk["rph"] if blk["rph"].shape[0] == 2 * Hp - 1 else _linear_resize_rows(blk["rph"], 2 * Hp - 1)
                tw = blk["rpw"] if blk["rpw"].shape[0] == 2 * Wp - 1 else _linear_resize_rows(blk["rpw"], 2 * Wp - 1)
                relg = (ops.global_relpos_planes(th, tw, fmt=ops.FMT_F3),
                        ops.global_relpos_planes(th, tw, fmt=ops.FMT_H8) if blk["qkv_bp16"] is not None else None)
                g["rel"].append(None)
            else:
                g["rel"].append((_rel_table(Hp, blk["rph"]), _rel_table(Wp, blk["rpw"])))
            g["relg"].append(relg)
        pk["geom"][key] = g
        return g

    @torch.no_grad()
    def _prepare(self, x):
        if not x.is_cuda:
            raise RuntimeError("mmsa: input must be a GPU tensor; the MI355X backbone has no CPU path")
        if x.dim() != 4 or x.shape[1] != 6:
            raise RuntimeError(f"mmsa: expected [B, 6, H, W] (rgb + auxiliary modality), got {tuple(x.shape)}")
        B, _, H, W = x.shape
        if H != self.img_size or W != self.img_size:
            raise RuntimeError(f"mmsa: H=W=img_size={self.img_size} is required (GFFM LayerNorm length, AM:240-241); got {H}x{W}")
        if H % 32 != 0:
            raise RuntimeError("mmsa: img_size must be a multiple of 32")
        dev = x.device
        x = x.contiguous().float()
        if self._packed is None or self._packed.get("dev") != dev or pack.packed_settings(self._packed) != PackPlan.of(self).settings():
            self._packed = self._pack(dev)
            self._packed["dev"] = dev
        if self._ws is None or self._ws.device != dev:
            self._ws = Workspace(dev)
        return x, B, H, W

    def _cbufs(self, B, H, W, tag=""):
        D = self.cfg["embed_dim"]
        Nc = (H // 8) * (W // 8) + (H // 16) * (W // 16) + (H // 32) * (W // 32)
        return self._ws.get("c1" + tag, B * (H // 4) * (W // 4), D), self._ws.get("c" + tag, B * Nc, D), Nc

    def forward(self, x):
        if not x.is_cuda:
            raise RuntimeError("mmsa: input must be a GPU tensor; the MI355X backbone has no CPU path")
        with torch.cuda.device(x.device):
            guard = self.attention_guard == "sync" and not torch.cuda.is_current_stream_capturing()
            depth = self.cfg["depth"]
            for _ in range(depth + 2):
                x, B, H, W = self._prepare(x)
                with ops.clamp_watch(self._packed["attn_guard"][depth:]):
                    c1, cbuf, Nc = self._cbufs(B, H, W)
                    c1_ready = self._spm(x, B, H, W, c1, cbuf, Nc)
                    outs = self._vit(x, B, H, W, c1, cbuf, c1_ready)
                if not guard or not self.check_attention_guard():
                    break
            return outs, None

    @torch.no_grad()
    def forward_taps(self, x):
        self._taps = {}
        try:
            outs, _ = self.forward(x)
            torch.cuda.synchronize(x.device)
            taps = self._taps
        finally:
            self._taps = None
        B, _, H, W = x.shape
        D = self.cfg["embed_dim"]
        res = {}
        for k, v in taps.items():
            if k.startswith(("twin", "fuse")):
                i = int(k[-1])
                h, w = H // (4 << i), W // (4 << i)
                res[k] = v.reshape(B, h, w, -1).permute(0, 3, 1, 2).contiguous()
            else:
                res[k] = v.reshape(B, -1, D)
        for i, f in enumerate(outs):
            res[f"f{i + 1}"] = f
        return outs, res

    def forward_pipelined(self, x_next):
        cur = getattr(self, "_pl_cur", None)
        dev_ = x_next.device if x_next is not None else (cur["x"].device if cur is not None else None)
        if dev_ is None:
            return None
        with torch.cuda.device(dev_):
            return self._forward_pipelined(x_next, cur)

    def _forward_pipelined(self, x_next, cur):
        main = torch.cuda.current_stream()
        nxt = None
        if x_next is not None:
            x_next, B, H, W = self._prepare(x_next)
            q = 1 - cur["set"] if cur is not None else 0
            c1, cbuf, Nc = self._cbufs(B, H, W, f"_p{q}")
            if getattr(self, "_pipe_stream", None) is None or self._pipe_stream.device != x_next.device:
                self._pipe_stream = torch.cuda.Stream(device=x_next.device)
            sa = self._pipe_stream
            ops.zero_(self._ws.get("pl_tick", 1, 1))
            sa.wait_stream(main)
            with torch.cuda.stream(sa):
                joins = self._spm(x_next, B, H, W, c1, cbuf, Nc, join=False)
            nxt = dict(x=x_next, set=q, dims=(B, H, W), c1=c1, c=cbuf)
        outs = None
        if cur is not None:
            B, H, W = cur["dims"]
            outs = self._vit(cur["x"], B, H, W, cur["c1"], cur["c"], None)
        if nxt is not None:
            for e in joins:
                main.wait_event(e)
            main.wait_stream(self._pipe_stream)
        self._pl_cur = nxt
        return (outs, None) if outs is not None else None

    def _vit(self, x, B, H, W, c1, cbuf, c1_ready):
        pk, ws, cfg = self._packed, self._ws, self.cfg
        dev = x.device
        geo = self._geometry(H, W, dev)
        D = cfg["embed_dim"]
        p = cfg["patch_size"]
        Hp, Wp = H // p, W // p
        T = Hp * Wp
        n2, n3, n4 = (H // 8) * (W // 8), T, (H // 32) * (W // 32)
        Nc = n2 + n3 + n4

        a = ws.get("pe_a", B * T, pk["pe_w"].kpad)
        ops.im2col_nchw(x, 0, 3, p, a)
        xs = [ws.get(f"x{i}", B * T, D) for i in range(len(self.interaction_indexes) + 1)]
        ops.gemm(a, pk["pe_w"], xs[0], bias=pk["pe_b"], resid=geo["pos"], resid_mod=T)
        taps = self._taps
        if taps is not None:
            taps["x_in"], taps["c_in"] = xs[0].clone(), cbuf[:B * Nc].clone()

        self._cfold = None
        n_inter = len(self.interaction_indexes)
        for i, idx in enumerate(self.interaction_indexes):
            it = pk["inter"][i]
            self._injector(it["inj"], xs[i], xs[i + 1], cbuf, geo, B, T, Nc)
            for bi in range(idx[0], idx[-1] + 1):
                self._block(pk["blocks"][bi], geo["rel"][bi], xs[i + 1], B, Hp, Wp, geo["relg"][bi],
                            next_fmt=pk["blocks"][bi + 1]["qkv"].afmt if bi < idx[-1] else None)
            for j, ex in enumerate(it["ext"]):
                self._extractor(ex, cbuf, xs[i + 1], geo, B, T, Nc, H, W, last=(i == n_inter - 1 and j == len(it["ext"]) - 1))
            if taps is not None:
                taps[f"x{i}"], taps[f"c{i}"] = xs[i + 1].clone(), cbuf[:B * Nc].clone()
        self._cfold = None

        if c1_ready is not None:
            torch.cuda.current_stream().wait_event(c1_ready)
        if taps is not None:
            taps["c1_map"] = c1.clone()
        outs = []
        c2p = ws.planes("up_a", B * n2, D, fmt=pk["up"].fmt)
        for bi in range(B):
            ops.split_planes(cbuf[bi * Nc:bi * Nc + n2], kpad=D, out=c2p.rows(bi * n2, (bi + 1) * n2))
        ops.gemm(c2p, pk["up"], c1, bias=pk["up_b"], resid=c1, batch=B, m=n2, stride_a=c2p.batch_stride(n2),
                 stride_r=(H // 4) * (W // 4) * D, stride_c=(H // 4) * (W // 4) * D, pixel_shuffle=(H // 8, W // 8, D))
        emit = bool(getattr(self, "emit_planes", False)) and D % 32 == 0
        ctag = getattr(self._ws, "tag", "")
        if not hasattr(self, "_planes_gens"):
            self._planes_gens = {}
        pgen = self._planes_gens.setdefault(ctag, [0])
        pgen[0] += 1
        outs = []
        for k, (src, cs, (hh, wwd)) in enumerate(((c1, (H // 4) * (W // 4) * D, (H // 4, W // 4)), (cbuf, Nc * D, (H // 8, W // 8)),
                                                  (cbuf[n2:], Nc * D, (Hp, Wp)), (cbuf[n2 + n3:], Nc * D, (H // 32, W // 32)))):
            f = torch.empty(B, D, hh, wwd, device=dev)
            fpl = ws.planes(f"f{k + 1}_out", B * hh * wwd, D) if emit else None
            ops.tail_fuse(src, cs, xs[k + 1] if self.cfg["add_vit_feature"] else None, *pk["bn"][k], f, B, hh, wwd, Hp, Wp, out_planes=fpl)
            if emit:
                f._mmsa_planes = fpl.stamp(pgen)
            outs.append(f)
        f1, f2, f3, f4 = outs
        return [f1, f2, f3, f4]

    def _stream_planes(self, rows, fmt):
        D = self.cfg["embed_dim"]
        return (self._ws.planes("blk_xp", rows, D, fmt=fmt), self._ws.get("blk_rs", rows, 2 * (D // 64)))

    def _block(self, bp, rel, x, B, Hp, Wp, relg=None, next_fmt=None):
        ws, cfg = self._ws, self.cfg
        D, heads = cfg["embed_dim"], cfg["num_heads"]
        hd = self._hd_pad
        scale = self._hd_true ** -0.5
        Da = heads * hd
        T = Hp * Wp
        folded_w = self._packed["fold_ln"]
        fold = folded_w and B * T >= 128
        fused = bp.get("relp") is not None or relg is not None
        f16 = bp["qkv_bp16"] is not None and self._attn_mode(bp) == "f16"
        vf = bp["qkv"].afmt
        gw = self._packed["attn_guard"][bp["index"]:bp["index"] + 1]
        if fold:
            xp, rs = self._stream_planes(B * T, vf)
            mr = ws.get("blk_mr", B * T, 2)
            ops.rowstats_finalize(rs, B * T, D, 1e-6, mr)
            n = None
        else:
            n = ws.planes("blk_n", B * T, D, fmt=vf)
            if folded_w:
                ops.layernorm(x, self._packed["ln_one"], self._packed["ln_zero"], 1e-6, out_planes=n)
            else:
                ops.layernorm(x, bp["n1w"], bp["n1b"], 1e-6, out_planes=n)
        all16 = fused and f16
        qkv = ws.planes("blk_qkv", B * T, 3 * Da, fmt=ops.FMT_H8 if all16 else ops.FMT_F3)
        if all16:
            bias_p = bp["qkv_bp16"]
        elif f16 and not fused:
            bias_p = bp["qkv_bp"]
            qkv.split = bias_p.split
        else:
            bias_p = bp["qkv_bp_b3"]
        if fold:
            ops.gemm(xp, bp["qkv"], bias=bp["qkv_bf"], out_planes=qkv, row_norm=(mr, bp["qkv_cs"]))
        else:
            ops.gemm(n, bp["qkv"], bias=bp["qkv_bf"] if folded_w else bp["qkv_b"], out_planes=qkv)
        wsz = bp["ws"]
        ao = ws.planes("blk_ao", B * T, Da, fmt=bp["proj"].afmt)
        if bp.get("relp") is not None:
            ops.window_attention(qkv, bias_p, bp["relp16"] if all16 else bp["relp"], ao, B, Hp, Wp, heads, hd, wsz, scale, max_logit=gw)
        elif relg is not None:
            ops.global_attention(qkv, bias_p, relg[1] if all16 else relg[0], ao, B, Hp, Wp, heads, hd, scale, max_logit=gw)
        else:
            kk = 2 * wsz if wsz else Hp + Wp
            rp = ws.get("blk_rp", B * heads * T, kk)
            ops.relpos_bias(qkv, rel[0], rel[1], rp, B, Hp, Wp, heads, hd, wsz)
            ops.attention(qkv, bias_p, rp, ao, B, Hp, Wp, heads, hd, wsz, scale, max_logit=gw)
        vf = bp["lin1"].afmt
        h = ws.planes("blk_h", B * T, bp["lin1"].n, fmt=vf)
        if fold:
            xp, rs = self._stream_planes(B * T, vf)
            ops.gemm(ao, bp["proj"], x, bias=bp["proj_b"], resid=x, out_planes=xp, rowstats_out=rs)
            ops.rowstats_finalize(rs, B * T, D, 1e-6, mr)
            ops.gemm(xp, bp["lin1"], bias=bp["lin1_bf"], act="gelu", out_planes=h, row_norm=(mr, bp["lin1_cs"]))
            if next_fmt is not None:
                xp, rs = self._stream_planes(B * T, next_fmt)
                ops.gemm(h, bp["lin2"], x, bias=bp["lin2_b"], resid=x, out_planes=xp, rowstats_out=rs)
            else:
                ops.gemm(h, bp["lin2"], x, bias=bp["lin2_b"], resid=x)
            return
        ops.gemm(ao, bp["proj"], x, bias=bp["proj_b"], resid=x)
        n = ws.planes("blk_n", B * T, D, fmt=vf)
        if folded_w:
            ops.layernorm(x, self._packed["ln_one"], self._packed["ln_zero"], 1e-6, out_planes=n)
        else:
            ops.layernorm(x, bp["n2w"], bp["n2b"], 1e-6, out_planes=n)
        ops.gemm(n, bp["lin1"], bias=bp["lin1_bf"] if folded_w else bp["lin1_b"], act="gelu", out_planes=h)
        ops.gemm(h, bp["lin2"], x, bias=bp["lin2_b"], resid=x)

    ATTN_F16_MAX_LOGIT = 8.0

    attention_guard = "sync"

    def _attn_policy(self):
        return getattr(self, "attention_precision", "auto")

    def _attn_mode(self, bp):
        pol = self._attn_policy()
        if pol in ("f16", "b3"):
            return pol
        return bp.get("amode") or "f16"

    def attention_guard_words(self):
        return self._packed["attn_guard"] if self._packed is not None else None

    @torch.no_grad()
    def check_attention_guard(self, reroute=True, vals=None):
        pk = self._packed
        if pk is None:
            return []
        if vals is None:
            vals = pk["attn_guard"].tolist()
        depth = self.cfg["depth"]
        clamped = max(float(vals[depth]) if len(vals) > depth else 0.0, float(pk.get("weights_clamped", 0.0)))
        if clamped > 0.0:
            if self.range_fallback and not self._wide():
                if reroute:
                    self._carry_modes = [(bp.get("amode"), bp.get("max_logit", 0.0)) for bp in pk["blocks"]]
                    self._wide_range = True
                    self._packed = None
                return list(range(depth))
            if len(vals) > depth and vals[depth] > 0.0:
                pk["attn_guard"][depth:].zero_()
            raise OperandRangeError(f"mmsa: a value of magnitude {clamped:.6g} or more (the GEMM's register epilogue reports the format's limit, not the value) was clamped on its way "
                                    "into fp16-based operand planes (h8 / h8c hold |x| <= 57344, f3 |x| <= 65504): the outputs since the last check are not the reference's.  "
                                    + ("The model is in its wide-range state already: what clamped is an operand of the attention kernels (q / k / v, a qkv bias or a rel-pos table "
                                       "entry beyond +-65504)." if self._wide() else "`range_fallback = True` (the default) re-routes instead of refusing."))
        auto = self._attn_policy() == "auto"
        moved = []
        dev, plan = pk["attn_guard"].device, PackPlan.of(self)
        sd_dev = functools.lru_cache(None)(lambda: pack.float_state_dict(self, dev))
        for bp, v in zip(pk["blocks"], vals):
            bp["max_logit"] = max(float(v), bp.get("max_logit", 0.0))
            if not auto or bp["qkv_bp16"] is None:
                continue
            if bp.get("amode") != "b3" and bp["max_logit"] > self.ATTN_F16_MAX_LOGIT:
                moved.append(bp["index"])
                if reroute:
                    bp["amode"] = "b3"
                    pack.repack_block_on_pairs(pk, bp, sd_dev, plan, dev)
            elif bp.get("amode") is None:
                bp["amode"] = "f16"
        if moved and reroute and auto and self.inter_follow_blocks and "inter" in self._h8_sites():
            want = self._inter_pair_set() | {i for i in (self._interaction_of_block(b) for b in moved) if i is not None}
            if want != self._inter_pair_set():
                self._inter_pairs = want
                self._carry_modes = [(bp.get("amode"), bp.get("max_logit", 0.0)) for bp in pk["blocks"]]
                self._packed = None
        return moved

    def attention_modes(self):
        return [(self._attn_mode(bp), bp.get("max_logit", 0.0)) for bp in self._packed["blocks"]] if self._packed else []

    def calibrate_attention(self, x):
        keep = self.attention_guard
        before = [bp.get("amode") for bp in self._packed["blocks"]] if self._packed else None
        self.attention_guard = "sync"
        try:
            self(x)
        finally:
            self.attention_guard = keep
        after = [bp.get("amode") for bp in self._packed["blocks"]]
        return [i for i, m in enumerate(after) if m == "b3" and (before is None or before[i] != "b3")]

    def _msda(self, ap, qn, fn, resid, out, ss, lsi, ref, B, Lq, S, L, colscale=None, stream_out=None, q_rn=None, f_rn=None):
        ws, cfg = self._ws, self.cfg
        M, Pn = cfg["deform_num_heads"], cfg["n_points"]
        dv = ap["val"].n
        vmode = getattr(self, "msda_value", "f32")
        if vmode in ("f16", "f16lo") and not self._wide() and (dv // M) % 8 == 0 and dv % 32 == 0:
            val = ws.planes("msda_valp", B * S, dv, fmt=ops.FMT_H8)
            ops.gemm(fn, ap["val"], bias=ap["val_b"], row_norm=f_rn, out_planes=val)
        else:
            val = ws.get("msda_val", B * S, dv)
            ops.gemm(fn, ap["val"], val, bias=ap["val_b"], row_norm=f_rn)
        raw = ws.get("msda_raw", B * Lq, ap["oa"].n)
        ops.gemm(qn, ap["oa"], raw, bias=ap["oa_b"], row_norm=q_rn)
        samp = ws.planes("msda_s", B * Lq, dv, fmt=ap["out"].fmt)
        ops.msda_fused(val, ss, lsi, raw, ref, None, B, S, M, dv // M, L, Lq, Pn, out_planes=samp, lo_bytes=vmode == "f16lo")
        if stream_out is not None:
            ops.gemm(samp, ap["out"], out, bias=ap["out_b"], resid=resid, colscale=colscale, out_planes=stream_out[0], rowstats_out=stream_out[1])
        else:
            ops.gemm(samp, ap["out"], out, bias=ap["out_b"], resid=resid, colscale=colscale)

    def _c_fold_on(self, rows):
        return bool(self._packed.get("fold_adapter_ln")) and rows % 256 == 0

    def _c_buffers(self, rows, fmt):
        D = self.cfg["embed_dim"]
        return self._ws.planes("inj_fn", rows, D, fmt=fmt), self._ws.get("c_rs", rows, 2 * (D // 64)), self._ws.get("c_mr", rows, 2)

    def _c_produced(self, rows, fmt):
        cp, crs, cmr = self._c_buffers(rows, fmt)
        ops.rowstats_finalize(crs, rows, self.cfg["embed_dim"], 1e-6, cmr)
        self._cfold = dict(planes=cp, mr=cmr)

    def _injector(self, ip, x_in, x_out, c, geo, B, T, Nc):
        ws, D = self._ws, self.cfg["embed_dim"]
        qn = ws.planes("inj_qn", B * T, D, fmt=ip["attn"]["oa"].fmt)
        ops.layernorm(x_in, ip["qnw"], ip["qnb"], 1e-6, out_planes=qn)
        st = self._cfold
        f_rn = None
        if st is not None and "val_cs" in ip["attn"]:
            fn, f_rn = st["planes"], (st["mr"], ip["attn"]["val_cs"])
        else:
            fn = ws.planes("inj_fn", B * Nc, D, fmt=ip["attn"]["val"].fmt)
            if ip["fold_c"]:
                pk = self._packed
                ops.layernorm(c, pk["ln_one"], pk["ln_zero"], 1e-6, out_planes=fn)
            else:
                ops.layernorm(c, ip["fnw"], ip["fnb"], 1e-6, out_planes=fn)
        self._msda(ip["attn"], qn, fn, x_in, x_out, geo["ss1"], geo["lsi1"], geo["ref1"], B, T, Nc, 3, colscale=ip["gamma"],
                   stream_out=(self._stream_planes(B * T, self._packed["blocks"][ip["first_block"]]["qkv"].afmt)
                               if self._packed["fold_ln"] and B * T >= 128 else None), f_rn=f_rn)

    def _extractor(self, ep, c, x, geo, B, T, Nc, H, W, last=False):
        ws, D = self._ws, self.cfg["embed_dim"]
        pk = self._packed
        rows = B * Nc
        fold = self._c_fold_on(rows) and ep["fold_c"]
        cfmt = ep["attn"]["oa"].fmt
        st = self._cfold
        q_rn = None
        if fold and st is not None and "oa_cs" in ep["attn"]:
            qn, q_rn = st["planes"], (st["mr"], ep["attn"]["oa_cs"])
        else:
            qn = ws.planes("inj_fn", rows, D, fmt=cfmt)
            if not (ep["fold_c"] and ep["first"]):
                if ep["fold_c"]:
                    ops.layernorm(c, pk["ln_one"], pk["ln_zero"], 1e-6, out_planes=qn)
                else:
                    ops.layernorm(c, ep["qnw"], ep["qnb"], 1e-6, out_planes=qn)
        fn = ws.planes("inj_qn", B * T, D, fmt=ep["attn"]["val"].fmt)
        ops.layernorm(x, ep["fnw"], ep["fnb"], 1e-6, out_planes=fn)
        produce = fold and (ep["cffn"] or not last)
        if produce:
            cp, crs, _ = self._c_buffers(rows, cfmt)
            self._cfold = None
            self._msda(ep["attn"], qn, fn, c, c, geo["ss2"], geo["lsi2"], geo["ref2"], B, Nc, T, 1, stream_out=(cp, crs), q_rn=q_rn)
            self._c_produced(rows, cfmt)
        else:
            self._cfold = None
            self._msda(ep["attn"], qn, fn, c, c, geo["ss2"], geo["lsi2"], geo["ref2"], B, Nc, T, 1, q_rn=q_rn)
        if not ep["cffn"]:
            return
        hid = ep["fc1"].n
        hp = ep["fc2"].kpad
        h1 = ws.get("ffn_h1", rows, hid)
        h2f = ws.planes(f"ffn_h2_{hp}", rows, hp, zero=True, fmt=ep["fc2"].fmt)
        st = self._cfold
        if st is not None and "fc1_cs" in ep:
            ops.gemm(st["planes"], ep["fc1"], h1, bias=ep["fc1_b"], row_norm=(st["mr"], ep["fc1_cs"]))
        else:
            qn = ws.planes("inj_fn", rows, D, fmt=ep["fc1"].fmt)
            if ep["fold_c"]:
                ops.layernorm(c, pk["ln_one"], pk["ln_zero"], 1e-6, out_planes=qn)
            else:
                ops.layernorm(c, ep["ffw"], ep["ffb"], 1e-6, out_planes=qn)
            ops.gemm(qn, ep["fc1"], h1, bias=ep["fc1_b"])
        off = 0
        for (hh, wwd) in ((H // 8, W // 8), (H // 16, W // 16), (H // 32, W // 32)):
            ops.dwconv(h1[off:], ep["dw"], ep["dw_b"], None, B, hh, wwd, 3, act="gelu",
                       xstride_b=Nc * hid, out_planes=h2f.rows(off), pstride_b=Nc * 2 * hp)
            off += hh * wwd
        self._cfold = None
        if fold and not last:
            cp, crs, _ = self._c_buffers(rows, cfmt)
            ops.gemm(h2f, ep["fc2"], c, bias=ep["fc2_b"], resid=c, out_planes=cp, rowstats_out=crs)
            self._c_produced(rows, cfmt)
        else:
            ops.gemm(h2f, ep["fc2"], c, bias=ep["fc2_b"], resid=c)

    def _spm(self, x, B, H, W, c1_out, cbuf, Nc, join=True):
        pk, ws = self._packed, self._ws
        D = self.cfg["embed_dim"]
        chans = self.channels
        sizes = [(H // 4, W // 4), (H // 8, W // 8), (H // 16, W // 16), (H // 32, W // 32)]
        tcat = [ws.get(f"tcat{i}", B * sizes[i][0] * sizes[i][1], 2 * chans[i]) for i in range(4)]
        tcat_p = [ws.planes(f"tcat{i}", B * sizes[i][0] * sizes[i][1], 2 * chans[i]) if chans[i] % 32 == 0 else None for i in range(4)]
        main = torch.cuda.current_stream()
        multi = getattr(self, "multistream", True)
        if multi:
            if not hasattr(self, "_sides"):
                self._sides = {}
            skey = (getattr(self._ws, "tag", ""), x.device)
            if skey not in self._sides:
                self._sides[skey] = [torch.cuda.Stream(device=x.device) for _ in range(4)]
            s_neck = self._sides[skey]
        else:
            s_neck = [main] * 4
        ev_x = []
        self._twin_batched(x, B, sizes, tcat, ev_x, tcat_p)
        if self._taps is not None:
            for i in range(4):
                self._taps[f"twin{i}"] = tcat[i].clone()
        offs = [0, 0, sizes[1][0] * sizes[1][1], sizes[1][0] * sizes[1][1] + sizes[2][0] * sizes[2][1]]
        joins = []
        for i in range(4):
            sn = s_neck[i]
            sn.wait_event(ev_x[i])
            with torch.cuda.stream(sn):
                if i == 0:
                    self._neck_level(0, pk["neck"][0], tcat[0], B, sizes[0][0], sizes[0][1], chans[0], c1_out, 0, tcat_p[0])
                else:
                    self._neck_level(i, pk["neck"][i], tcat[i], B, sizes[i][0], sizes[i][1], chans[i], cbuf[offs[i]:], Nc * D, tcat_p[i])
                e = torch.cuda.Event()
                e.record(sn)
                joins.append(e)
        if not join:
            return joins
        for e in joins[1:]:
            main.wait_event(e)
        return joins[0]

    def _twin_batched(self, x, B, sizes, tcat, stage_events, tcat_p=None):
        pk, ws = self._packed, self._ws
        chans = self.channels
        st = pk["twin2"]
        t = "cnb_"
        h0, w0 = sizes[0]
        P0 = B * h0 * w0
        kp = st["stem"].kpad
        a = ws.get(t + "stem_a", 2 * P0, kp)
        for si in range(2):
            ops.im2col_nchw(x, 3 * si, 3, 4, a[si * P0:(si + 1) * P0])
        t0 = ws.get(t + "tmp", 2 * P0, chans[0])
        ops.gemm(a, st["stem"], t0, bias=st["stem_b"], batch=2, m=P0, stride_a=P0 * kp, stride_w=st["stem"].n * 2 * kp,
                 stride_bias=chans[0], stride_c=P0 * chans[0])
        cur = ws.get(t + "cur0", 2 * P0, chans[0])
        ops.layernorm(t0, st["stem_nw"], st["stem_nb"], 1e-6, cur, group_rows=P0, w_gstride=chans[0])
        for i in range(4):
            hh, wwd = sizes[i]
            P = B * hh * wwd
            c = chans[i]
            if i >= 1:
                ds = st["ds"][i - 1]
                cp = chans[i - 1]
                Pp = B * sizes[i - 1][0] * sizes[i - 1][1]
                pa = ws.planes(t + "patch", 2 * P, 4 * cp, fmt=ds["w"].fmt)
                ops.layernorm(cur, ds["nw"], ds["nb"], 1e-6, out_planes=pa, patchify=(sizes[i - 1][0], sizes[i - 1][1]),
                              group_rows=Pp, w_gstride=cp)
                cur = ws.get(t + f"cur{i}", 2 * P, c)
                ops.gemm(pa, ds["w"], cur, bias=ds["b"], batch=2, m=P, stride_a=P * 2 * pa.kpad, stride_w=ds["w"].n * 2 * ds["w"].kpad,
                         stride_bias=c, stride_c=P * c)
            d = ws.get(t + "tmp", 2 * P, c)
            wf = st["stages"][i][0]["pw1"].fmt
            n = ws.planes(t + "n", 2 * P, c, fmt=wf)
            hbuf = ws.planes(t + "h", 2 * P, 4 * c, fmt=st["stages"][i][0]["pw2"].fmt)
            fuse_mlp = ops.convnext_mlp_fused_supported(c) and bool(getattr(self, "fuse_convnext_mlp", True))
            fold = "pw1f" in st["stages"][i][0] and not fuse_mlp and hh % 8 == 0 and wwd % 8 == 0 and P >= 128
            if fold:
                rs = ws.get(t + "rs", 2 * P, 2 * (c // 64))
                mr = ws.get(t + "mr", 2 * P, 2)
            for blk in st["stages"][i]:
                if fold:
                    ops.dwconv(cur, blk["dw"], blk["dw_b"], None, 2 * B, hh, wwd, 7, imgs_per_group=B, out_planes=n, rowstats_out=rs)
                    ops.rowstats_finalize(rs, 2 * P, c, 1e-6, mr)
                    ops.gemm(n, blk["pw1f"], bias=blk["pw1_bf"], act="gelu", out_planes=hbuf, row_norm=(mr, blk["pw1_cs"]), batch=2, m=P,
                             stride_a=P * 2 * n.kpad, stride_w=blk["pw1f"].n * 2 * blk["pw1f"].kpad, stride_bias=4 * c, stride_cp=P * 2 * hbuf.kpad)
                    ops.gemm(hbuf, blk["pw2"], cur, bias=blk["pw2_b"], colscale=blk["gamma"], resid=cur, batch=2, m=P,
                             stride_a=P * 2 * hbuf.kpad, stride_w=blk["pw2"].n * 2 * blk["pw2"].kpad, stride_bias=c,
                             stride_r=P * c, stride_c=P * c)
                    continue
                ops.dwconv(cur, blk["dw"], blk["dw_b"], d, 2 * B, hh, wwd, 7, imgs_per_group=B)
                ops.layernorm(d, blk["nw"], blk["nb"], 1e-6, out_planes=n, group_rows=P, w_gstride=c)
                if fuse_mlp:
                    ops.convnext_mlp_fused(n, blk["pw1"], blk["pw2"], blk["pw1_b"], blk["pw2_b"], blk["gamma"], cur, P, batch=2,
                                           stride_a=P * 2 * n.kpad, stride_w1=blk["pw1"].n * 2 * blk["pw1"].kpad,
                                           stride_w2=blk["pw2"].n * 2 * blk["pw2"].kpad, stride_x=P * c)
                    continue
                ops.gemm(n, blk["pw1"], bias=blk["pw1_b"], act="gelu", out_planes=hbuf, batch=2, m=P, stride_a=P * 2 * n.kpad,
                         stride_w=blk["pw1"].n * 2 * blk["pw1"].kpad, stride_bias=4 * c, stride_cp=hbuf.batch_stride(P))
                ops.gemm(hbuf, blk["pw2"], cur, bias=blk["pw2_b"], colscale=blk["gamma"], resid=cur, batch=2, m=P,
                         stride_a=hbuf.batch_stride(P), stride_w=blk["pw2"].batch_stride(blk["pw2"].n), stride_bias=c,
                         stride_r=P * c, stride_c=P * c)
            nw, nb = st["out_norm"][i]
            ops.layernorm(cur, nw, nb, 1e-6, tcat[i], group_rows=P, w_gstride=c, y_gcol=c, y_wrap=True,
                          out_planes=tcat_p[i] if tcat_p is not None else None)
            ev = torch.cuda.Event()
            ev.record(torch.cuda.current_stream())
            stage_events.append(ev)

    def _neck_level(self, level, lv, t, B, h, w, c, out, out_stride_b, tp=None):
        ws = _Tagged(self._ws, f"nk{level}_")
        C = 2 * c
        HW = h * w
        P = B * HW
        gcat = ws.get("nk_g", P, C)
        lcat = ws.get("nk_l", P, C)
        pl_ok = tp is not None and c % 32 == 0
        gcat_p = ws.planes("nk_gp", P, C) if pl_ok else None
        lcat_p = ws.planes("nk_lp", P, C) if pl_ok else None
        n_st, n_g, n_st2 = B * 3 * 3 * c, B * c * c, B * 3 * C
        acc_blk = ws.get("nk_acc", 1, 2 * (n_st + n_g) + n_g + n_st2, dtype=torch.float64)
        ops.zero_(acc_blk[0, :2 * n_st + n_st2])
        gram_scr = ws.get("nk_gscr", 1, (ops.gram_tn_scratch_bytes(B, HW, c) + 3) // 4)
        acc_off = [0, 2 * n_st + n_st2]

        def acc_buf(rows, cols, gram=False):
            o = acc_off[int(gram)]
            acc_off[int(gram)] = o + rows * cols
            return acc_blk[0, o:o + rows * cols].view(rows, cols)
        for m in range(2):
            X = t[:, m * c:(m + 1) * c]
            gp = lv["gfe"][m]
            y = ws.get("nk_y", P, c)
            s = ws.get("nk_s", P, c)
            ops.layernorm(X, gp["nw"], gp["nb"], 1e-5, y, out2=s)
            q2 = ws.get("nk_q2", P, 3 * c)
            if not ("q12" in gp and getattr(self, "fuse_gfe_qkv", True) and ops.gfe_qkv(y, gp["q12"], q2, B, h, w, 32, c // 32, 3 * c // 32)):
                q1 = ws.get("nk_q1", P, 3 * c)
                ops.gconv(y, gp["q1"], None, q1, B, h, w, 32, c // 32, 3 * c // 32, 1)
                ops.gconv(q1, gp["q2"], None, q2, B, h, w, 32, 3 * c // 32, 3 * c // 32, 3)
            st = acc_buf(B * 3, 3 * c)
            ops.colstats(q2, HW * 3 * c, B, HW, st, out_is_zero=True)
            g = acc_buf(B * c, c, gram=True)
            ops.gram_tn(q2[:, :c], q2[:, c:2 * c], HW * 3 * c, g, B, HW, nblk=8, scratch=gram_scr)
            cp = ops.pad32(c)
            pl = ops.Planes(ws.get(f"nk_pp{c}", B * c, 2 * cp, dtype=torch.int16, zero=True), c, c, cp)
            base = st.data_ptr()
            ops.chanattn_build(g, base + 8 * (3 * c), 9 * c, base + 8 * (3 * c + c), 9 * c, gp["temp"], gp["proj"], pl, B, c, 8)
            ops.gemm(q2[:, 2 * c:], pl, gcat[:, m * c:(m + 1) * c], alpha=gp["scale2"], resid=s, batch=B, m=HW,
                     stride_a=HW * 3 * c, stride_w=c * 2 * cp, stride_r=HW * c, stride_c=HW * C,
                     out_planes=gcat_p.cols(m * c, (m + 1) * c) if pl_ok else None, stride_cp=HW * 2 * C)
            lp = lv["loc"][m]
            h1 = ws.get("nk_q1", P, 2 * c)
            h2 = ws.get("nk_q2", P, 2 * c)
            if pl_ok:
                ops.gemm(tp.cols(m * c, (m + 1) * c), lp["w1"], h1, act="relu6")
                h2p = ws.planes("nk_h2p", P, 2 * c)
                ops.dwconv(h1, lp["dw"], None, None, B, h, w, 3, act="relu6", out_planes=h2p)
                ops.gemm(h2p, lp["w3"], alpha=lp["scale"], resid=X, out_planes=lcat_p.cols(m * c, (m + 1) * c))
            else:
                ops.gemm(X, lp["w1"], h1, act="relu6")
                ops.dwconv(h1, lp["dw"], None, h2, B, h, w, 3, act="relu6")
                ops.gemm(h2, lp["w3"], lcat[:, m * c:(m + 1) * c], alpha=lp["scale"], resid=X)
        e = acc_buf(B * c, c, gram=True)
        ops.gram_tn(gcat[:, :c], gcat[:, c:], HW * C, e, B, HW, nblk=1, scratch=gram_scr)
        cp = ops.pad32(c)
        px = ops.Planes(ws.get(f"nk_pp{c}", B * c, 2 * cp, dtype=torch.int16, zero=True), c, c, cp)
        py = ops.Planes(ws.get(f"nk_pp2{c}", B * c, 2 * cp, dtype=torch.int16, zero=True), c, c, cp)
        ops.gffm_build(e, px, py, B, c)
        fbuf = ws.get("nk_f", P, C)
        ops.gemm(gcat_p.cols(c, C) if pl_ok else gcat[:, c:], px, fbuf[:, :c], alpha=lv["gx"], resid=gcat[:, :c], batch=B, m=HW,
                 stride_a=HW * C * (2 if pl_ok else 1), stride_w=c * 2 * cp, stride_r=HW * C, stride_c=HW * C)
        ops.gemm(gcat_p.cols(0, c) if pl_ok else gcat[:, :c], py, fbuf[:, c:], alpha=lv["gy"], resid=gcat[:, c:], batch=B, m=HW,
                 stride_a=HW * C * (2 if pl_ok else 1), stride_w=c * 2 * cp, stride_r=HW * C, stride_c=HW * C)
        st = acc_buf(B * 3, C)
        ops.colstats(fbuf, HW * C, B, HW, st, wrow=lv["lnw"], out_is_zero=True)
        mean = ws.get("nk_mean", B, C)
        rstd = ws.get("nk_rstd", B, C)
        mult = ws.get("nk_mult", B, C)
        ops.ffrm_finalize(st, B, HW, C, lv["lnw_mean"], lv["lnb_mean"], lv["ffrm_w"], lv["gn_w"], lv["gn_b"], mean, rstd, mult,
                          ws.get("nk_ffrm", 2 * B, C))
        fn = ws.get("nk_g", P, C)
        ops.lnhw_apply(fbuf, mean, rstd, mult, lv["lnw"], lv["lnb"], fn, B, HW)
        hm = ws.get("nk_hm", P, 2 * C)
        ops.gemm(lcat_p if pl_ok else lcat, lv["mlp_in"], hm)
        hg = ws.planes("nk_hg", P, C)
        ops.dwpair_gate(hm, lv["mlp_dw"], None, B, h, w, C, out_planes=hg)
        z = ws.get("nk_f", P, C)
        ops.gemm(hg, lv["mlp_out"], z, alpha=lv["s2"], resid=fn, beta=lv["s1"])
        pooled = ws.get("nk_pool", B * (h + w), C)
        ops.pool_hw(z, pooled, B, h, w)
        y1 = ws.get(f"nk_y1_{lv['mip_pad']}", B * (h + w), lv["mip_pad"], zero=True)
        ops.gemm(pooled, lv["ca1"], y1, bias=lv["ca1_b"], act="hswish")
        att = ws.get("nk_att", B * (h + w), C)
        ops.gemm(y1, lv["cah"], att, bias=lv["cah_b"], act="sigmoid", batch=B, m=h,
                 stride_a=(h + w) * lv["mip_pad"], stride_c=(h + w) * C)
        ops.gemm(y1[h:], lv["caw"], att[h:], bias=lv["caw_b"], act="sigmoid", batch=B, m=w,
                 stride_a=(h + w) * lv["mip_pad"], stride_c=(h + w) * C)
        if pl_ok:
            zo = ws.planes("nk_zop", P, C)
            ops.ca_apply(z, att, None, B, h, w, out_planes=zo)
            sa = HW * 2 * C
        else:
            zo = ws.get("nk_g", P, C)
            ops.ca_apply(z, att, zo, B, h, w)
            sa = HW * C
        if self._taps is not None:
            self._taps[f"fuse{level}"] = ops.planes_to_float(zo, cols=C) if pl_ok else zo[:, :C].clone()
        if out_stride_b == 0:
            ops.gemm(zo, lv["fc"], out, bias=lv["fc_b"])
        else:
            ops.gemm(zo, lv["fc"], out, bias=lv["fc_b"], batch=B, m=HW, stride_a=sa, stride_c=out_stride_b)


class SAMAdapterbimodalMixModNewInTwinConvNEWwithcp(SAMAdapterbimodalMixModNewInTwinConvNEW):
    """Second registered name (backbones/__init__.py:3-9): identical inference math, extra training-only kwargs."""


def _ref_points(shapes):
    refs = []
    for (h, w) in shapes:
        ys = torch.linspace(0.5, h - 0.5, h, dtype=torch.float32) / h
        xs = torch.linspace(0.5, w - 0.5, w, dtype=torch.float32) / w
        gy, gx = torch.meshgrid(ys, xs, indexing="ij")
        refs.append(torch.stack((gx.reshape(-1), gy.reshape(-1)), -1))
    return torch.cat(refs, 0).contiguous()


def rel_pos_index(q_size, k_size):
    q = torch.arange(q_size)[:, None] * max(k_size / q_size, 1.0)
    k = torch.arange(k_size)[None, :] * max(q_size / k_size, 1.0)
    return ((q - k) + (k_size - 1) * max(q_size / k_size, 1.0)).long()


def _rel_table(size, rel_pos):
    L = 2 * size - 1
    tab = rel_pos if rel_pos.shape[0] == L else _linear_resize_rows(rel_pos, L)
    return tab[rel_pos_index(size, size).to(tab.device)].contiguous()


def _cubic_w(t, A=-0.75):
    def c1(x):
        return ((A + 2) * x - (A + 3)) * x * x + 1

    def c2(x):
        return ((A * x - 5 * A) * x + 8 * A) * x - 4 * A
    return torch.stack([c2(t + 1), c1(t), c1(1 - t), c2(2 - t)], -1)


def _bicubic_matrix(n_in, n_out, device):
    scale = n_in / n_out
    x = (torch.arange(n_out, dtype=torch.float32, device=device) + 0.5) * scale - 0.5
    ix = x.floor()
    w = _cubic_w(x - ix)
    m = torch.zeros(n_out, n_in, dtype=torch.float32, device=device)
    for k in range(4):
        idx = (ix.long() - 1 + k).clamp(0, n_in - 1)
        m.scatter_add_(1, idx[:, None], w[:, k:k + 1])
    return m


def _bicubic_resize(src_hwc, H, W):
    h, w, _ = src_hwc.shape
    if (h, w) == (H, W):
        return src_hwc.contiguous()
    my = _bicubic_matrix(h, H, src_hwc.device)
    mx = _bicubic_matrix(w, W, src_hwc.device)
    return torch.einsum("Hh,hwc,Ww->HWc", my, src_hwc, mx).contiguous()
```

### multimodal-sam-adapter_amd/mmsa/head.py

```python
import torch
import torch.nn as nn

from . import lib
from . import ops
from .params import Node, _attach


class SegformerHead(nn.Module):
    def __init__(self, interpolate_mode="bilinear", in_channels=None, channels=None, *, num_classes=None, dropout_ratio=0.1,
                 conv_cfg=None, norm_cfg=None, act_cfg=dict(type="ReLU"), in_index=-1, input_transform="multiple_select",
                 loss_decode=None, ignore_index=255, sampler=None, align_corners=False, init_cfg=None, **kwargs):
        super().__init__()
        if in_channels is None or channels is None or num_classes is None:
            raise TypeError("SegformerHead: in_channels, channels and num_classes are required")
        if not isinstance(in_channels, (list, tuple)) or not isinstance(in_index, (list, tuple)) or len(in_channels) != len(in_index):
            raise AssertionError("SegformerHead: in_channels and in_index must be lists of equal length")
        if not 1 <= len(in_channels) <= 4:
            raise NotImplementedError("mmsa SegformerHead: 1..4 input maps")
        if interpolate_mode != "bilinear" or align_corners:
            raise NotImplementedError("mmsa SegformerHead: only interpolate_mode='bilinear', align_corners=False (the reference configs)")
        if norm_cfg is None or norm_cfg.get("type") not in ("BN", "SyncBN"):
            raise NotImplementedError("mmsa SegformerHead: norm_cfg must be BN / SyncBN (eval: running-statistics affine)")
        if act_cfg is None or act_cfg.get("type") != "ReLU":
            raise NotImplementedError("mmsa SegformerHead: act_cfg must be ReLU")
        if channels % 8:
            raise NotImplementedError("mmsa SegformerHead: channels must be a multiple of 8")
        self.in_channels, self.in_index, self.channels = list(in_channels), list(in_index), channels
        self.num_classes, self.dropout_ratio, self.align_corners = num_classes, dropout_ratio, align_corners
        self.interpolate_mode, self.ignore_index, self.norm_cfg, self.act_cfg = interpolate_mode, ignore_index, norm_cfg, act_cfg
        n = len(in_channels)
        g = torch.Generator().manual_seed(0)

        def conv_w(co, ci):
            return torch.randn(co, ci, 1, 1, generator=g) * (2.0 / ci) ** 0.5

        def bn(prefix):
            _attach(self, prefix + ".weight", torch.ones(channels))
            _attach(self, prefix + ".bias", torch.zeros(channels))
            _attach(self, prefix + ".running_mean", torch.zeros(channels), buffer=True)
            _attach(self, prefix + ".running_var", torch.ones(channels), buffer=True)
            _attach(self, prefix + ".num_batches_tracked", torch.zeros((), dtype=torch.long), buffer=True)

        _attach(self, "conv_seg.weight", torch.randn(num_classes, channels, 1, 1, generator=g) * 0.01)
        _attach(self, "conv_seg.bias", torch.zeros(num_classes))
        self.add_module("convs", Node())
        for i, ci in enumerate(in_channels):
            _attach(self, f"convs.{i}.conv.weight", conv_w(channels, ci))
            bn(f"convs.{i}.bn")
        _attach(self, "fusion_conv.conv.weight", conv_w(channels, channels * n))
        bn("fusion_conv.bn")
        self._packed = None
        self._bufs = {}
        self.register_load_state_dict_post_hook(lambda m, _: m.invalidate())
        self.eval()

    def invalidate(self):
        self._packed = None

    def train(self, mode=True):
        if mode:
            raise NotImplementedError("mmsa: the MI355X decode head implements the inference forward path only")
        return super().train(False)

    def init_weights(self):
        pass

    def forward_test(self, inputs, img_metas=None, test_cfg=None):
        return self.forward(inputs)

    def forward_train(self, inputs, img_metas, gt_semantic_seg, train_cfg):
        raise NotImplementedError("mmsa: the MI355X decode head implements the inference forward path only (no losses)")

    @torch.no_grad()
    def _pack(self, dev):
        sd = {k: v.detach().to(dev, torch.float32) for k, v in self.state_dict().items() if v.dtype.is_floating_point}
        ch, n = self.channels, len(self.in_channels)

        def bn_affine(p):
            s = sd[p + ".weight"] / torch.sqrt(sd[p + ".running_var"] + 1e-5)
            return s.contiguous(), (sd[p + ".bias"] - sd[p + ".running_mean"] * s).contiguous()

        pk = {"branch": []}
        wf = sd["fusion_conv.conv.weight"].reshape(ch, ch * n)
        for i, ci in enumerate(self.in_channels):
            s, t = bn_affine(f"convs.{i}.bn")
            w = sd[f"convs.{i}.conv.weight"].reshape(ch, ci) * s[:, None]
            pk["branch"].append(dict(w=ops.split_planes(w.contiguous()), shift=t,
                                     wf=ops.split_planes(wf[:, ch * i:ch * (i + 1)].contiguous())))
        pk["fs"], pk["ft"] = bn_affine("fusion_conv.bn")
        ncp = ops.pad32(self.num_classes)
        wc = torch.zeros(ncp, ch, device=dev)
        wc[:self.num_classes] = sd["conv_seg.weight"].reshape(self.num_classes, ch)
        bc = torch.zeros(ncp, device=dev)
        bc[:self.num_classes] = sd["conv_seg.bias"]
        pk["wc"], pk["bc"], pk["ncp"] = ops.split_planes(wc), bc, ncp
        return pk

    def _buf(self, name, shape, dtype=torch.float32, dev=None):
        name = getattr(self, "buf_tag", "") + name
        t = self._bufs.get(name)
        if t is None or tuple(t.shape) != tuple(shape) or t.device != dev:
            t = torch.zeros(shape, dtype=dtype, device=dev)
            self._bufs[name] = t
        return t

    def _planes(self, name, rows, cols, dev):
        kp = ops.pad32(cols)
        return ops.Planes(self._buf(name, (rows, 2 * kp), torch.int16, dev), rows, cols, kp)

    @torch.no_grad()
    def forward(self, inputs, out=None):
        x0 = inputs[self.in_index[0]]
        if not x0.is_cuda:
            raise RuntimeError("mmsa SegformerHead: inputs must live on the GPU (there is no CPU path)")
        with torch.cuda.device(x0.device):
            return self._forward(inputs, out)

    def _forward(self, inputs, out=None):
        xs = [inputs[i] for i in self.in_index]
        x0 = xs[0]
        dev = x0.device
        if self._packed is None or self._packed["wc"].p.device != dev:
            self._packed = self._pack(dev)
        pk = self._packed
        B, _, H, W = x0.shape
        ch = self.channels
        zs = []
        for i, (x, ci) in enumerate(zip(xs, self.in_channels)):
            if x.dtype != torch.float32 or x.dim() != 4 or x.shape[0] != B or x.shape[1] != ci:
                raise RuntimeError(f"mmsa SegformerHead: input {i} must be fp32 [B={B}, {ci}, h, w], got {tuple(x.shape)} {x.dtype}")
            x = x.contiguous()
            h, w = x.shape[2:]
            rows = B * h * w
            xp = getattr(inputs[self.in_index[i]], "_mmsa_planes", None)
            if not isinstance(xp, ops.Planes) or xp.n != rows or xp.k != ci or xp.p.device != dev or not xp.live():
                xp = self._planes(f"x{i}", rows, ci, dev)
                lib.call("mmsa_nchw_to_planes", x.data_ptr(), ci * h * w, xp.p.data_ptr(), 2 * xp.kpad, B, ci, h * w, ops._stream())
            br = pk["branch"][i]
            yp = self._planes(f"y{i}", rows, ch, dev)
            ops.gemm(xp, br["w"], bias=br["shift"], act="relu", out_planes=yp)
            z = self._buf(f"z{i}", (rows, ch), dev=dev)
            ops.gemm(yp, br["wf"], z)
            zs.append((z, h, w))
        fp = self._planes("fused", B * H * W, ch, dev)
        lv = zs[1:] + [(None, 0, 0)] * (4 - len(zs))
        lib.call("mmsa_head_fuse", zs[0][0].data_ptr(),
                 lv[0][0].data_ptr() if lv[0][0] is not None else None, lv[0][1], lv[0][2],
                 lv[1][0].data_ptr() if lv[1][0] is not None else None, lv[1][1], lv[1][2],
                 lv[2][0].data_ptr() if lv[2][0] is not None else None, lv[2][1], lv[2][2],
                 ch, pk["fs"].data_ptr(), pk["ft"].data_ptr(), fp.p.data_ptr(), 2 * fp.kpad, None, 0, B, H, W, ch, ops.ACT["relu"],
                 ops._stream())
        lt = self._buf("logit_tokens", (B * H * W, pk["ncp"]), dev=dev)
        ops.gemm(fp, pk["wc"], lt, bias=pk["bc"])
        if out is None:
            out = torch.empty(B, self.num_classes, H, W, device=dev)
        elif (tuple(out.shape) != (B, self.num_classes, H, W) or out.dtype != torch.float32 or out.device != dev or not out.is_contiguous()):
            raise RuntimeError(f"mmsa SegformerHead: out must be a contiguous fp32 [{B}, {self.num_classes}, {H}, {W}] tensor on {dev}")
        lib.call("mmsa_tokens_to_nchw", lt.data_ptr(), pk["ncp"], out.data_ptr(), B, H * W, self.num_classes, ops._stream())
        return out
```

### multimodal-sam-adapter_amd/mmsa/lib.py

```python
import ctypes
import os
from ctypes import c_char_p, c_double, c_float, c_int, c_long, c_void_p, POINTER

_HERE = os.path.dirname(os.path.abspath(__file__))
LIB_PATH = os.environ.get("MMSA_LIB") or os.path.join(_HERE, "libmmsa_hip.so")

if not os.path.exists(LIB_PATH):
    raise RuntimeError(
        f"{LIB_PATH} not found: the MI355X HIP library is required (no CPU/PyTorch fallback exists). "
        "Build it with: python multimodal-sam-adapter_amd/build.py")

import torch

_lib = ctypes.CDLL(LIB_PATH)

P = c_void_p
I = c_int
L = c_long
F = c_float

SIGNATURES = {
    "mmsa_version": [],
    "mmsa_last_error": [],
    "mmsa_debug_poison_lds": [ctypes.c_uint, P],
    "mmsa_event_create": [POINTER(c_void_p)],
    "mmsa_event_record": [P, P],
    "mmsa_event_elapsed_ms": [P, P, POINTER(c_float)],
    "mmsa_event_destroy": [P],
    "mmsa_ms_deform_attn_forward": [P, P, P, P, P, P, I, I, I, I, I, I, I, I, I, P],
    "mmsa_ms_deform_attn_backward": [P, P, P, P, P, P, P, P, P, I, I, I, I, I, I, I, I, I, P],
    "mmsa_msda_fused": [P, P, P, P, L, P, P, L, P, L, I, I, I, I, I, I, I, I, P, P],
    "mmsa_msda_fused_planes": [P, L, I, P, P, P, L, P, P, L, P, L, I, I, I, I, I, I, I, I, P, P],
    "mmsa_gemm_split3": [P, P, L, L, P, L, P, L, P, P, L, L, I, F, P, L, L, P, L, L, I, I, I, I, I, F, I, I, I, I, I, I, I, P, P, P, I, P, P],
    "mmsa_convnext_mlp_fused": [P, L, L, P, L, P, L, P, P, P, P, L, L, I, I, I, I, I, P, P],
    "mmsa_rowstats_finalize": [P, I, I, I, F, P, P],
    "mmsa_zero_bytes": [P, ctypes.c_size_t, P],
    "mmsa_split_planes": [P, L, I, I, I, P, I, P, P],
    "mmsa_attention": [P, L, P, P, P, L, I, I, I, I, I, I, F, P],
    "mmsa_attention_planes": [P, L, P, P, P, L, I, I, I, I, I, I, F, I, I, P, P],
    "mmsa_relpos_bias": [P, L, P, P, P, I, I, I, I, I, I, P],
    "mmsa_relpos_bias_planes": [P, L, P, P, P, I, I, I, I, I, I, P],
    "mmsa_layernorm_rows": [P, L, P, P, F, P, L, P, L, P, L, I, I, I, I, I, I, L, L, I, I, P, P],
    "mmsa_colstats": [P, L, L, P, I, I, I, P, I, P],
    "mmsa_ffrm_finalize": [P, I, I, I, F, F, P, P, P, P, P, P, P, P],
    "mmsa_lnhw_apply": [P, L, P, P, P, P, P, P, L, I, I, I, P],
    "mmsa_dwconv_nhwc": [P, L, L, P, P, P, L, L, P, L, L, I, I, I, I, I, I, I, I, P, P, P],
    "mmsa_dwpair_gate": [P, L, P, P, L, P, L, I, I, I, I, P],
    "mmsa_gconv_nhwc": [P, L, P, P, P, L, I, I, I, I, I, I, I, I, P],
    "mmsa_gfe_qkv_conv": [P, L, P, P, L, I, I, I, I, I, I, POINTER(c_int), P],
    "mmsa_im2col_nchw": [P, I, I, I, I, I, I, I, P, I, P],
    "mmsa_gram_tn": [P, L, P, L, L, P, I, I, I, I, P, L, P],
    "mmsa_gram_tn_scratch_bytes": [I, I, I],
    "mmsa_chanattn_build": [P, P, L, P, L, P, P, P, I, I, I, I, P],
    "mmsa_gffm_build": [P, P, P, I, I, I, P],
    "mmsa_gelu_gate": [P, L, P, L, L, I, P],
    "mmsa_pool_hw": [P, L, P, L, I, I, I, I, P],
    "mmsa_ca_apply": [P, L, P, L, P, L, P, L, I, I, I, I, P],
    "mmsa_tail_fuse": [P, L, L, P, L, P, P, P, P, L, I, I, I, I, I, I, P],
    "mmsa_global_attention_planes": [P, L, P, P, P, L, I, I, I, I, I, F, I, I, P, P],
    "mmsa_window_attention_planes": [P, L, P, P, P, P, L, I, I, I, I, I, I, F, I, I, P, P],
    "mmsa_nchw_to_planes": [P, L, P, L, I, I, L, P],
    "mmsa_head_fuse": [P, P, I, I, P, I, I, P, I, I, L, P, P, P, L, P, L, I, I, I, I, I, P],
    "mmsa_tokens_to_nchw": [P, L, P, I, L, I, P],
    "mmsa_bilinear_accum_nchw": [P, L, I, I, I, I, P, I, I, I, I, I, I, P, I, P],
    "mmsa_div_count_nchw": [P, P, I, I, L, P],
    "mmsa_argmax_nchw": [P, P, I, I, L, P],
    "mmsa_crop_batch_nchw": [P, I, I, I, I, P, I, P, I, I, P],
    "mmsa_slide_argmax": [P, I, I, I, I, P, P, I, I, I, I, I, P, P],
    "mmsa_slide_argmax_resized": [P, I, I, I, I, P, P, I, I, I, I, I, I, I, I, I, P, P],
    "mmsa_softmax_flip_accum_nchw": [P, P, I, I, I, I, I, I, I, P],
    "mmsa_aug_argmax": [P, P, I, I, P, P, I, P, I, I, I, P, P],
    "mmsa_argmax_max_nchw": [P, P, P, I, I, L, P],
    "mmsa_slide_argmax_conf": [P, I, I, I, I, P, P, P, I, I, I, I, I, P, P],
    "mmsa_slide_argmax_resized_conf": [P, I, I, I, I, P, P, P, I, I, I, I, I, I, I, I, I, P, P],
    "mmsa_aug_argmax_conf": [P, P, I, I, P, P, I, P, P, I, I, I, P, P],
    "mmsa_preprocess_nhwc": [P, I, P, I, I, I, I, P, P, P, P, P, P, I, I, P],
    "mmsa_preprocess_crops": [P, I, P, I, I, I, I, P, P, P, P, P, I, I, P, I, P, I, I, P],
    "mmsa_preprocess_resize_nhwc": [P, I, P, I, I, I, I, P, P, P, P, P, P, I, I, I, I, P, P, P, P, I, P],
    "mmsa_preprocess_resize_crops": [P, I, P, I, I, I, I, P, P, P, P, P, I, I, P, I, P, I, I, I, I, P, P, P, P, I, P],
    "mmsa_eval_confusion_u8": [P, P, I, I, I, I, I, P, I, P, P, P, I, P, P],
    "mmsa_eval_calibration": [P, P, P, I, I, I, I, I, P, I, P, P, P, I, I, P, P],
    "mmsa_eval_selective": [P, P, P, I, I, I, I, I, P, I, P, P, P, I, I, P, P],
    "mmsa_abstain_u8": [P, P, L, I, I, P, P],
    "mmsa_slide_argmax_conf_t": [P, I, I, I, I, P, P, P, I, I, I, I, I, P, F, P],
    "mmsa_slide_argmax_resized_conf_t": [P, I, I, I, I, P, P, P, I, I, I, I, I, I, I, I, I, P, F, P],
    "mmsa_softmax_flip_accum_nchw_t": [P, P, I, I, I, I, I, I, I, F, P],
    "mmsa_temperature_sweep_nchw": [P, P, I, I, I, I, I, I, P, P, P, P, I, P, I, I, P, P],
    "mmsa_slide_argmax_eval": [P, I, I, I, I, P, P, I, I, I, I, I, P, P, I, I, P, P, P, P, I, P, P],
    "mmsa_render_u8": [P, L, L, I, I, I, P, I, I, P, I, I, I, c_double, c_double, P, P],
    "mmsa_render_denorm_f32": [P, L, L, I, I, I, P, I, I, P, I, I, I, P, P, I, I, c_double, c_double, P, P],
}
_RESTYPES = {"mmsa_last_error": c_char_p, "mmsa_gram_tn_scratch_bytes": c_long}

for _name, _args in SIGNATURES.items():
    _fn = getattr(_lib, _name)
    _fn.argtypes = _args
    _fn.restype = _RESTYPES.get(_name, c_int)


ABI_VERSION = 114
if _lib.mmsa_version() != ABI_VERSION:
    raise RuntimeError(f"{LIB_PATH}: ABI version {_lib.mmsa_version()} but mmsa/lib.py binds version {ABI_VERSION} (include/mmsa.h MMSA_ABI_VERSION): "
                       "rebuild with python multimodal-sam-adapter_amd/build.py")


def last_error() -> str:
    return _lib.mmsa_last_error().decode()


POISON_LDS = os.environ.get("MMSA_DEBUG_POISON_LDS") == "1"


def call(name, *args):
    if POISON_LDS and not name.startswith(("mmsa_event", "mmsa_debug")) and args:
        _lib.mmsa_debug_poison_lds(0x7FC07FC0, args[-1])
    rc = getattr(_lib, name)(*args)
    if rc != 0:
        raise RuntimeError(f"{name} failed (rc={rc}): {last_error()}")


def version() -> int:
    return _lib.mmsa_version()


raw = _lib
```

### multimodal-sam-adapter_amd/mmsa/ops.py

```python
import ctypes

import os

import torch

from . import lib

ACT = {"none": 0, "gelu": 1, "relu": 2, "relu6": 3, "hswish": 4, "sigmoid": 5}

GEMM_PROFILE = None
CLAMP_WATCH = None
GEMM_MAX_GRID = 0
GEMM_FLAVOUR = 0
GEMM_SHAPES = None


def _event():
    ev = ctypes.c_void_p()
    lib.call("mmsa_event_create", ctypes.byref(ev))
    return ev


def collect_gemm_profile(prof):
    flops, ms = 0.0, 0.0
    collect_gemm_profile.bytes = sum(p[3] for p in prof)
    collect_gemm_profile.launches = []
    for f, e0, e1, by in prof:
        t = ctypes.c_float()
        lib.call("mmsa_event_elapsed_ms", e0, e1, ctypes.byref(t))
        flops += f
        ms += t.value
        collect_gemm_profile.launches.append((f, by, t.value))
        lib.call("mmsa_event_destroy", e0)
        lib.call("mmsa_event_destroy", e1)
    return flops, ms


def _stream():
    return torch.cuda.current_stream().cuda_stream


def _clamp_ptr():
    return CLAMP_WATCH.data_ptr() if CLAMP_WATCH is not None else None


class clamp_watch:

    def __init__(self, word):
        self.word = word

    def __enter__(self):
        global CLAMP_WATCH
        self.keep, CLAMP_WATCH = CLAMP_WATCH, self.word
        return self

    def __exit__(self, *exc):
        global CLAMP_WATCH
        CLAMP_WATCH = self.keep
        return False


def _chk(t, dtype=torch.float32, name="tensor"):
    if t is None:
        return None
    if not t.is_cuda:
        raise RuntimeError(f"mmsa: {name} must live on the GPU (got {t.device}); there is no CPU path")
    if t.dtype != dtype:
        raise RuntimeError(f"mmsa: {name} must be {dtype}, got {t.dtype}")
    if t.device.index != torch.cuda.current_device():
        raise RuntimeError(f"mmsa: {name} lives on {t.device} but the current device is cuda:{torch.cuda.current_device()}; "
                           "call under torch.cuda.device(tensor.device)")
    return t.data_ptr()


def _mat(t, name, dtype=torch.float32):
    if t.dim() != 2 or (t.shape[1] > 1 and t.stride(1) != 1):
        raise RuntimeError(f"mmsa: {name} must be a 2-D view with unit column stride, got shape {tuple(t.shape)} stride {t.stride()}")
    return _chk(t, dtype, name), t.shape[0], t.shape[1], t.stride(0)


FMT_B3, FMT_H8, FMT_H8C, FMT_F3 = 0, 1, 2, 3
FMT_W8 = 4
W8_EMIN, W8_EMAX = -15, 7
E4M3_MAX = 448.0


def _binade(a, lo):
    b = torch.floor(torch.log2(a.clamp_min(2.0 ** (lo - 1)))).clamp_min(lo)
    b = torch.where(a >= torch.exp2(b + 1), b + 1, b)
    return torch.where((b > lo) & (a < torch.exp2(b)), b - 1, b)


def fp8_quantize(w2d):
    w = w2d.detach().to(torch.float64)
    if w.dim() != 2 or not bool(torch.isfinite(w).all()):
        raise ValueError("mmsa.fp8_quantize: a finite 2-D weight is expected")
    amax = w.abs().amax(1) if w.shape[1] else w.new_zeros(w.shape[0])
    lim = E4M3_MAX * 2.0 ** W8_EMAX
    if bool((amax > lim).any()):
        n = int(torch.argmax(amax))
        raise ValueError(f"mmsa.fp8_quantize: row {n} has max |w| = {float(amax[n]):.6g} > {lim:g} = 448 * 2^{W8_EMAX}: not representable as fp8 weights")
    e = torch.ceil(torch.log2(amax.clamp_min(1e-300) / E4M3_MAX)).clamp(W8_EMIN, W8_EMAX)
    e = torch.where(amax > E4M3_MAX * torch.exp2(e), e + 1, e)
    e = torch.where((e > W8_EMIN) & (amax <= E4M3_MAX * torch.exp2(e - 1)), e - 1, e)
    v = w / torch.exp2(e)[:, None]
    a = v.abs()
    step = torch.exp2(_binade(a, -6) - 3)
    q = torch.round(a / step) * step
    b = _binade(q, -6)
    normal = q >= 2.0 ** -6
    code = torch.where(normal, (b + 7) * 8 + (q / torch.exp2(b) * 8 - 8), q * 512.0).to(torch.int32)
    code = code | torch.where((v < 0) & (q > 0), 128, 0)
    return code.to(torch.uint8), e.to(torch.int8)


def fp8_dequantize(codes, exps):
    c = codes.to(torch.int32)
    ex, m = (c >> 3) & 15, (c & 7).double()
    mag = torch.where(ex == 0, m * 2.0 ** -9, (8.0 + m) * torch.exp2(ex.double() - 10.0))
    return (torch.where(c >= 128, -mag, mag) * torch.exp2(exps.double())[:, None]).float()


def w8_planes(w2d):
    n, k = w2d.shape
    if k % 128:
        raise ValueError(f"mmsa.w8_planes: K={k} must be a multiple of 128")
    codes, exps = fp8_quantize(w2d)
    rows = n + -(-((n + 127) // 128 * 128) // k)
    buf = torch.zeros(rows * k, dtype=torch.uint8, device=w2d.device)
    buf[:n * k] = codes.reshape(n, k // 64, 2, 4, 8).permute(0, 1, 3, 2, 4).reshape(-1)
    buf[n * k:n * k + n] = exps.view(torch.uint8)
    return Planes(buf.view(torch.int16).view(rows, k // 2), n, k, k, FMT_W8, True)


def w8_codes(pl):
    n, k = pl.n, pl.kpad
    by = pl.p.contiguous().view(torch.uint8).view(-1)
    return by[:n * k].view(n, k // 64, 4, 2, 8).permute(0, 1, 3, 2, 4).reshape(n, k), by[n * k:n * k + n].view(torch.int8)


class Planes:

    def __init__(self, p, n=None, k=None, kpad=None, fmt=FMT_B3, weight=False, split=0):
        self.p = p
        self.split = split
        if fmt == FMT_H8C and (n is None or kpad is None):
            raise RuntimeError("mmsa.Planes: h8c planes need their row count and padded width (the tensor holds row pairs)")
        self.n = p.shape[0] if n is None else n
        self.kpad = p.shape[1] // 2 if kpad is None else kpad
        self.k = self.kpad if k is None else k
        self.fmt = fmt
        self.weight = weight
        self.gen = None

    @property
    def afmt(self):
        return FMT_H8C if self.fmt == FMT_W8 else self.fmt

    def stamp(self, cell):
        self.gen = (cell, cell[0])
        return self

    def live(self):
        return self.gen is None or self.gen[0][0] == self.gen[1]

    def rows(self, lo, hi=None):
        if self.fmt == FMT_H8C:
            hi = self.n if hi is None else hi
            if lo % 2 or (hi % 2 and hi != self.n):
                raise RuntimeError("mmsa.Planes.rows: h8c planes are stored by row pairs -- slices start and end at even rows")
            return Planes(self.p[lo // 2:(hi + 1) // 2], hi - lo, self.k, self.kpad, self.fmt, self.weight)
        return Planes(self.p[lo:hi], None, self.k, self.kpad, self.fmt, self.weight, self.split)

    def cols(self, lo, hi):
        if lo % 32 or hi % 32 or self.fmt == FMT_H8C:
            raise RuntimeError("mmsa.Planes.cols: column bounds must be multiples of 32 (and the planes bf16 hi/lo or h8 line planes)")
        return Planes(self.p[:, 2 * lo:2 * hi], self.n, hi - lo, hi - lo, self.fmt, self.weight)

    def batch_stride(self, rows):
        if self.fmt == FMT_H8C:
            if rows % 2:
                raise RuntimeError("mmsa.Planes.batch_stride: h8c batches hold an even number of rows")
            return (rows // 2) * self.p.stride(0)
        return rows * self.p.stride(0)

    def mat(self, name):
        ptr, rows, cols, ld = _mat(self.p, name, torch.int16)
        if ptr % 128 or ld % 64:
            raise RuntimeError(f"mmsa: {name} planes must be 128-byte aligned with a row stride that is a multiple of 64")
        if self.fmt == FMT_H8C:
            if ld < 3 * self.kpad or self.kpad % 64:
                raise RuntimeError(f"mmsa: {name}: h8c planes need kpad % 64 == 0 and a pair stride >= 3 * kpad")
            return ptr, self.n, self.kpad, ld
        return ptr, rows, cols // 2, ld


def pad32(k):
    return (k + 31) // 32 * 32


def pad64(k):
    return (k + 63) // 64 * 64


def planes_shape(rows, cols, fmt):
    if fmt == FMT_H8C:
        kp = pad64(cols)
        return (rows + 1) // 2, 3 * kp, kp
    kp = pad32(cols)
    return rows, 2 * kp, kp


def alloc_planes(rows, cols, device, zero=False, fmt=FMT_B3, split=0):
    f = torch.zeros if zero else torch.empty
    if split and (split % 32 or fmt not in (FMT_B3, FMT_F3) or not 0 < split < cols):
        raise RuntimeError(f"mmsa.alloc_planes: split={split} must be a multiple of 32 inside a bf16 hi/lo or f3 matrix of {cols} columns")
    tr, tc, kp = planes_shape(rows, cols, fmt)
    return Planes(f(tr, tc, dtype=torch.int16, device=device), rows, cols, kp, fmt, split=split)


def cp_format(pl):
    return FMT_B3 if pl is None else pl.fmt | ((pl.split // 32) << 8)


def planes_to_float(pl, cols=None):
    r, w = pl.p.shape
    if pl.split:
        lo_part = planes_to_float(Planes(pl.p[:, :2 * pl.split], pl.n, pl.split, pl.split, pl.fmt))
        hi_part = planes_to_float(Planes(pl.p[:, 2 * pl.split:], pl.n, pl.kpad - pl.split, pl.kpad - pl.split, FMT_H8))
        return torch.cat([lo_part, hi_part], 1)[:, :(pl.k if cols is None else cols)]
    if pl.fmt == FMT_W8:
        return fp8_dequantize(*w8_codes(pl))[:, :(pl.k if cols is None else cols)]
    if pl.fmt == FMT_H8C:
        kp = pl.kpad
        by = pl.p[:, :3 * kp].contiguous().view(torch.uint8).view(r, 6 * kp)
        hi = by[:, :4 * kp].contiguous().view(torch.float16).float().reshape(2 * r, kp)
        lo = by[:, 4 * kp:].reshape(r, kp // 64, 2, 4, 2, 8).permute(0, 2, 1, 4, 3, 5)
        lo = lo.contiguous().view(torch.float8_e5m2).float().reshape(2 * r, kp)
        return (hi + lo / (2048.0 * 1.09375))[:pl.n, :(pl.k if cols is None else cols)]
    if pl.fmt == FMT_H8:
        blk = pl.p.contiguous().view(torch.uint8).view(r, w // 64, 128)
        hi = blk[:, :, :64].contiguous().view(torch.float16).float()
        ch = blk[:, :, 64:].reshape(r, w // 64, 4, 2, 8)
        lo = ch[:, :, :, 1 if pl.weight else 0].contiguous().view(torch.float8_e5m2).float().reshape(r, w // 64, 32)
        out = (hi + lo / 2048.0).reshape(r, w // 2)
    elif pl.fmt == FMT_F3:
        v = pl.p.contiguous().view(torch.float16).float().view(r, w // 64, 2, 32)
        out = (v[:, :, 0] + v[:, :, 1]).reshape(r, w // 2)
    else:
        v = (pl.p.to(torch.int32) << 16).view(torch.float32).view(r, w // 64, 2, 32)
        out = (v[:, :, 0] + v[:, :, 1]).reshape(r, w // 2)
    return out[:, :(pl.k if cols is None else cols)]


def split_planes(w2d, kpad=None, out=None, fmt=FMT_B3, weight=False):
    p, n, k, ld = _mat(w2d, "weight")
    if out is None:
        kpad = kpad or (pad64(k) if fmt == FMT_H8C else pad32(k))
        if fmt == FMT_H8C:
            if kpad % 64:
                raise RuntimeError("mmsa.split_planes: h8c planes need kpad % 64 == 0")
            out = Planes(torch.zeros((n + 1) // 2, 3 * kpad, dtype=torch.int16, device=w2d.device), n, k, kpad, fmt, False)
        else:
            out = Planes(torch.empty(n, 2 * kpad, dtype=torch.int16, device=w2d.device), n, k, kpad, fmt, weight)
    kpad = out.kpad
    if out.fmt == FMT_H8C:
        if out.n != n or not out.p.is_contiguous() or out.p.shape[1] != 3 * kpad:
            raise RuntimeError("mmsa.split_planes: dense h8c planes of the source's row count expected")
        kind = 3
    else:
        kind = 0 if out.fmt == FMT_B3 else 4 if out.fmt == FMT_F3 else (2 if out.weight else 1)
    lib.call("mmsa_split_planes", p, ld, n, k, kpad, out.p.data_ptr(), kind, _clamp_ptr(), _stream())
    return out


def gemm(a, w, out=None, bias=None, act="none", alpha=1.0, colscale=None, resid=None, beta=1.0, resid_mod=0,
         batch=1, stride_a=0, stride_w=0, stride_bias=0, stride_r=0, stride_c=0, m=None, pixel_shuffle=None,
         out_planes=None, stride_cp=0, rowstats_out=None, row_norm=None):
    fmt = w.fmt
    if isinstance(a, Planes):
        pap, ma, ka, lda = a.mat("A")
        pa = None
        if ka < w.kpad:
            raise RuntimeError(f"mmsa.gemm: A planes have {ka} columns but the packed weight expects K={w.kpad}")
        if a.fmt != w.afmt or a.weight or (w.fmt == FMT_H8 and not w.weight) or (w.fmt == FMT_H8C and w.weight):
            raise RuntimeError(f"mmsa.gemm: operand formats differ (A fmt {a.fmt}, W fmt {w.fmt} weight={w.weight})")
    elif fmt not in (FMT_B3, FMT_F3):
        raise RuntimeError("mmsa.gemm: h8 weights need A as h8 planes")
    else:
        pa, ma, ka, lda = _mat(a, "A")
        pap = None
        if ka < w.kpad and lda < w.kpad:
            raise RuntimeError(f"mmsa.gemm: A has {ka} columns (ld {lda}) but the packed weight expects K={w.kpad}")
    m = ma if m is None else m
    pc, ldc = None, 0
    if out is not None:
        pc, _, _, ldc = _mat(out, "C")
    pcp, ldcp = None, 0
    if out_planes is not None:
        pcp, _, _, ldcp = out_planes.mat("Cplanes")
    pr, ldr = None, 0
    if resid is not None:
        pr, _, _, ldr = _mat(resid, "resid")
    ps = pixel_shuffle or (0, 0, 0)
    prof = GEMM_PROFILE
    if prof is not None:
        e0, e1 = _event(), _event()
        lib.call("mmsa_event_record", e0, _stream())
    lib.call("mmsa_gemm_split3", pa, pap, lda, stride_a, w.p.data_ptr(), stride_w,
             _chk(bias, name="bias"), stride_bias, _chk(colscale, name="colscale"), pr, ldr, stride_r, resid_mod, beta,
             pc, ldc, stride_c, pcp, ldcp, stride_cp, m, w.n, w.kpad, batch, ACT[act], alpha,
             1 if pixel_shuffle else 0, ps[0], ps[1], ps[2], fmt, cp_format(out_planes), GEMM_MAX_GRID,
             _chk(rowstats_out), _chk(row_norm[0]) if row_norm else None, _chk(row_norm[1]) if row_norm else None, GEMM_FLAVOUR, _clamp_ptr(), _stream())
    if prof is not None:
        lib.call("mmsa_event_record", e1, _stream())
        ob = 3.0 if fmt in (FMT_H8C, FMT_W8) else 4.0
        wb = 1.0 if fmt == FMT_W8 else ob
        pb = 0.0 if out_planes is None else (3.0 if out_planes.fmt == FMT_H8C else 4.0)
        prof.append((2.0 * m * w.n * w.k * batch, e0, e1,
                     batch * (ob * m * w.kpad + wb * w.n * w.kpad + m * w.n * (pb + 4.0 * ((1 if out is not None else 0) + (1 if resid is not None else 0))))))
        if GEMM_SHAPES is not None:
            GEMM_SHAPES.append((m, w.n, w.k, batch, act, resid is not None, ("C" if out is not None else "") + ("P" if out_planes is not None else ""),
                                "planes" if pap is not None else "fp32"))
    return out if out is not None else out_planes


def convnext_mlp_fused(a, w1, w2, b1, b2, gamma, x, m, batch=1, stride_a=0, stride_w1=0, stride_w2=0, stride_x=0):
    pa, _, _, lda = a.mat("A")
    px, _, c, ldx = _mat(x, "x")
    if a.fmt not in (FMT_B3, FMT_F3) or w1.fmt != a.fmt or w2.fmt != a.fmt:
        raise RuntimeError("mmsa.convnext_mlp_fused: bf16 hi/lo or f3 planes expected, the same format for A, W1 and W2")
    prof = GEMM_PROFILE
    if prof is not None:
        e0, e1 = _event(), _event()
        lib.call("mmsa_event_record", e0, _stream())
    lib.call("mmsa_convnext_mlp_fused", pa, lda, stride_a, w1.p.data_ptr(), stride_w1, w2.p.data_ptr(), stride_w2, _chk(b1), _chk(b2),
             _chk(gamma), px, ldx, stride_x, m, c, batch, GEMM_MAX_GRID, a.fmt, _clamp_ptr(), _stream())
    if prof is not None:
        lib.call("mmsa_event_record", e1, _stream())
        prof.append((2.0 * 2.0 * m * c * 4 * c * batch, e0, e1, 4.0 * batch * (m * c * 3 + 2 * 4 * c * c)))
        if GEMM_SHAPES is not None:
            GEMM_SHAPES.append((m, c, 4 * c, batch, "gelu", True, "C", "fused-pair"))
    return x


def convnext_mlp_fused_supported(c):
    return c == 96


def zero_(t):
    if not t.is_contiguous():
        raise RuntimeError("mmsa.ops.zero_: contiguous tensor expected")
    if t.numel():
        lib.call("mmsa_zero_bytes", _chk(t, t.dtype), t.numel() * t.element_size(), _stream())
    return t


def rowstats_finalize(rowstats, rows, d, eps, out):
    lib.call("mmsa_rowstats_finalize", _chk(rowstats), rows, d // 64, d, eps, _chk(out), _stream())
    return out


def layernorm(x, w, b, eps, out=None, out2=None, patchify=None, out_planes=None, group_rows=0, w_gstride=0, y_gcol=0, y_wrap=False):
    px, rows, c, ldx = _mat(x, "x")
    py, ldy = None, 0
    if out is not None:
        py, _, _, ldy = _mat(out, "y")
    p2, ld2 = None, 0
    if out2 is not None:
        p2, _, _, ld2 = _mat(out2, "y2")
    pp, ldp = None, 0
    if out_planes is not None:
        pp, _, _, ldp = out_planes.mat("y planes")
    mh, mw = patchify or (0, 0)
    lib.call("mmsa_layernorm_rows", px, ldx, _chk(w), _chk(b), eps, py, ldy, p2, ld2, pp, ldp, rows, c,
             1 if patchify else 0, mh, mw, group_rows, w_gstride, y_gcol, 1 if y_wrap else 0,
             out_planes.fmt if out_planes is not None else FMT_B3, _clamp_ptr(), _stream())
    return out if out is not None else out_planes


MSDA_DTYPES = {torch.float32: 0, torch.float16: 1, torch.float64: 2}


def _msda_args(value, spatial_shapes, level_start_index, sampling_loc, attn_weight, extra=()):
    dt = value.dtype
    if dt not in MSDA_DTYPES:
        raise RuntimeError(f"ms_deform_attn: dtype {dt} not supported (float32, float16, float64)")
    for t, n in ((value, "value"), (sampling_loc, "sampling_loc"), (attn_weight, "attn_weight")) + tuple(extra):
        if not t.is_contiguous():
            raise RuntimeError(f"{n} tensor has to be contiguous")
        if t.dtype != dt:
            raise RuntimeError(f"{n} must have the dtype of value ({dt}), got {t.dtype}")
    if not (spatial_shapes.is_contiguous() and level_start_index.is_contiguous()):
        raise RuntimeError("spatial_shapes / level_start_index tensor has to be contiguous")
    return dt


def msda_forward(value, spatial_shapes, level_start_index, sampling_loc, attn_weight, im2col_step=64):
    dt = _msda_args(value, spatial_shapes, level_start_index, sampling_loc, attn_weight)
    n, s, m, d = value.shape
    _, lq, _, l, p, _ = sampling_loc.shape
    out = torch.empty(n, lq, m * d, dtype=dt, device=value.device)
    lib.call("mmsa_ms_deform_attn_forward", _chk(value, dt), _chk(spatial_shapes, torch.int64), _chk(level_start_index, torch.int64),
             _chk(sampling_loc, dt), _chk(attn_weight, dt), out.data_ptr(), n, s, m, d, l, lq, p, im2col_step, MSDA_DTYPES[dt], _stream())
    return out


def msda_backward(value, spatial_shapes, level_start_index, sampling_loc, attn_weight, grad_output, im2col_step=64):
    dt = _msda_args(value, spatial_shapes, level_start_index, sampling_loc, attn_weight, extra=((grad_output, "grad_output"),))
    n, s, m, d = value.shape
    _, lq, _, l, p, _ = sampling_loc.shape
    if tuple(grad_output.shape) != (n, lq, m * d):
        raise RuntimeError(f"grad_output must be [{n}, {lq}, {m * d}], got {tuple(grad_output.shape)}")
    gv, gl, ga = torch.empty_like(value), torch.empty_like(sampling_loc), torch.empty_like(attn_weight)
    lib.call("mmsa_ms_deform_attn_backward", _chk(value, dt), _chk(spatial_shapes, torch.int64), _chk(level_start_index, torch.int64),
             _chk(sampling_loc, dt), _chk(attn_weight, dt), _chk(grad_output, dt), gv.data_ptr(), gl.data_ptr(), ga.data_ptr(),
             n, s, m, d, l, lq, p, im2col_step, MSDA_DTYPES[dt], _stream())
    return [gv, gl, ga]


def msda_fused(value2d, spatial_shapes, level_start_index, raw, ref_points, out, batch, spatial, heads, d, levels, lq, points,
               out_planes=None, lo_bytes=False):
    pr, _, _, ldraw = _mat(raw, "raw")
    if isinstance(value2d, Planes):
        if value2d.fmt != FMT_H8 or value2d.weight or value2d.split:
            raise RuntimeError("mmsa.msda_fused: value planes must be H8 activation planes")
        pvp, _, _, ldvp = value2d.mat("value planes")
        po, ldo = None, 0
        if out is not None:
            po, _, _, ldo = _mat(out, "out")
        pp, ldp = None, 0
        if out_planes is not None:
            pp, _, _, ldp = out_planes.mat("out planes")
        lib.call("mmsa_msda_fused_planes", pvp, ldvp, 1 if lo_bytes else 0, _chk(spatial_shapes, torch.int64), _chk(level_start_index, torch.int64), pr, ldraw,
                 _chk(ref_points), po, ldo, pp, ldp, out_planes.fmt if out_planes is not None else FMT_B3,
                 batch, spatial, heads, d, levels, lq, points, _clamp_ptr(), _stream())
        return out if out is not None else out_planes
    pv, vrows, vcols, ldv = _mat(value2d, "value")
    if vrows != batch * spatial or vcols != heads * d or (vrows > 1 and ldv != heads * d):
        raise RuntimeError(f"mmsa.msda_fused: value must be a dense [batch * spatial, heads * d] = [{batch * spatial}, {heads * d}] matrix, "
                           f"got shape {tuple(value2d.shape)} with row stride {ldv}")
    po, ldo = None, 0
    if out is not None:
        po, _, _, ldo = _mat(out, "out")
    pp, ldp = None, 0
    if out_planes is not None:
        pp, _, _, ldp = out_planes.mat("out planes")
    lib.call("mmsa_msda_fused", pv, _chk(spatial_shapes, torch.int64), _chk(level_start_index, torch.int64), pr, ldraw,
             _chk(ref_points), po, ldo, pp, ldp, out_planes.fmt if out_planes is not None else FMT_B3,
             batch, spatial, heads, d, levels, lq, points, _clamp_ptr(), _stream())
    return out if out is not None else out_planes


def relpos_bias(qkv, rh, rw, rp, b, h, w, heads, hd, ws):
    if isinstance(qkv, Planes):
        pq, _, _, ldq = qkv.mat("qkv")
        lib.call("mmsa_relpos_bias_planes", pq, ldq, _chk(rh), _chk(rw), _chk(rp), b, h, w, heads, hd, ws, _stream())
    else:
        pq, _, _, ldq = _mat(qkv, "qkv")
        lib.call("mmsa_relpos_bias", pq, ldq, _chk(rh), _chk(rw), _chk(rp), b, h, w, heads, hd, ws, _stream())
    return rp


def _v_fmt(qkv, qkv_bias, d, fused=False, rel=None):
    if qkv.fmt == FMT_H8 or qkv_bias.fmt == FMT_H8 or (rel is not None and rel.fmt == FMT_H8):
        if not (fused and qkv.fmt == FMT_H8 and qkv_bias.fmt == FMT_H8 and rel is not None and rel.fmt == FMT_H8
                and not (qkv.weight or qkv_bias.weight or rel.weight)):
            raise RuntimeError("mmsa attention: h8 planes need the fused rel-pos entry with qkv, bias AND rel-pos planes in the h8 (activation) format")
        return 2
    if qkv.split != qkv_bias.split or qkv.split not in (0, 2 * d) or (fused and qkv.split):
        raise RuntimeError(f"mmsa attention: qkv planes (split {qkv.split}) and bias planes (split {qkv_bias.split}) must both be f3 (fp16 hi/lo) "
                           f"planes, either plain or -- for the entry with a rel-pos prepass -- with the v columns from {2 * d} on as h8 planes")
    if qkv.fmt != FMT_F3 or qkv_bias.fmt != FMT_F3 or (rel is not None and rel.fmt != FMT_F3):
        raise RuntimeError("mmsa attention: the hi/lo operand form of the attention kernels reads f3 planes (fp16 hi/lo pairs: ops.FMT_F3) since round 4 -- "
                           "qkv, bias and rel-pos planes; bf16 hi/lo planes have the same layout and would be misread")
    return 1 if qkv.split else 0


def split_planes_qkv(x2d, d):
    if (2 * d) % 32 or d % 32:
        raise RuntimeError("mmsa.split_planes_qkv: embed dim must be a multiple of 32")
    qk = split_planes(x2d[:, :2 * d].contiguous(), fmt=FMT_F3)
    v = split_planes(x2d[:, 2 * d:].contiguous(), fmt=FMT_H8)
    return Planes(torch.cat([qk.p, v.p], 1).contiguous(), x2d.shape[0], 3 * d, 3 * d, FMT_F3, split=2 * d)


def _guard(g):
    if g is None:
        return None
    if g.dtype != torch.float32 or g.numel() != 1 or not g.is_cuda:
        raise RuntimeError("mmsa attention: max_logit must be a 1-element fp32 device tensor")
    return g.data_ptr()


def attention(qkv, qkv_bias, rp, out, b, h, w, heads, hd, ws, scale, max_logit=None):
    if isinstance(qkv, Planes):
        pq, _, _, ldq = qkv.mat("qkv")
        po, _, _, ldo = out.mat("out")
        lib.call("mmsa_attention_planes", pq, ldq, _chk(qkv_bias.p, torch.int16), _chk(rp),
                 po, ldo, b, h, w, heads, hd, ws, scale, out.fmt, _v_fmt(qkv, qkv_bias, heads * hd), _guard(max_logit), _stream())
    else:
        pq, _, _, ldq = _mat(qkv, "qkv")
        po, _, _, ldo = _mat(out, "out")
        lib.call("mmsa_attention", pq, ldq, _chk(qkv_bias), _chk(rp), po, ldo, b, h, w, heads, hd, ws, scale, _stream())
    return out


def window_relpos_planes(rel_pos_h, rel_pos_w, ws, fmt=FMT_B3):
    L = 2 * ws - 1
    if rel_pos_h.shape[0] != L or rel_pos_w.shape[0] != L or L > 27:
        raise RuntimeError(f"mmsa.window_relpos_planes: tables must have {L} <= 27 rows")
    m = torch.zeros(64, rel_pos_h.shape[1], dtype=torch.float32, device=rel_pos_h.device)
    m[:L] = rel_pos_h
    m[32:32 + L] = rel_pos_w
    return split_planes(m, fmt=fmt)


def global_relpos_planes(rel_pos_h, rel_pos_w, fmt=FMT_B3):
    if rel_pos_h.shape[0] > 127 or rel_pos_w.shape[0] > 127:
        raise RuntimeError("mmsa.global_relpos_planes: tables must have at most 127 rows")
    m = torch.zeros(256, rel_pos_h.shape[1], dtype=torch.float32, device=rel_pos_h.device)
    m[:rel_pos_h.shape[0]] = rel_pos_h
    m[128:128 + rel_pos_w.shape[0]] = rel_pos_w
    return split_planes(m, fmt=fmt)


def global_attention(qkv, qkv_bias, relg, out, b, h, w, heads, hd, scale, max_logit=None):
    pq, _, _, ldq = qkv.mat("qkv")
    po, _, _, ldo = out.mat("out")
    lib.call("mmsa_global_attention_planes", pq, ldq, _chk(qkv_bias.p, torch.int16), _chk(relg.p, torch.int16), po, ldo,
             b, h, w, heads, hd, scale, out.fmt, _v_fmt(qkv, qkv_bias, heads * hd, fused=True, rel=relg), _guard(max_logit), _stream())
    return out


_SELECTORS = {}


def window_selector(ws, device, f16=False):
    key = (ws, str(device), f16)
    if key not in _SELECTORS:
        sel = torch.zeros(208, 32, dtype=torch.int16)
        j = torch.arange(min(ws * ws, 208))
        one = 0x3C00
        sel[j, j // ws] = one
        sel[j, 14 + j % ws] = one
        _SELECTORS[key] = sel.to(device)
    return _SELECTORS[key]


def window_attention(qkv, qkv_bias, relp, out, b, h, w, heads, hd, ws, scale, max_logit=None):
    if not 1 <= ws <= 14:
        raise RuntimeError(f"mmsa.window_attention: window_size {ws} not supported (1..14)")
    pq, _, _, ldq = qkv.mat("qkv")
    po, _, _, ldo = out.mat("out")
    vf = _v_fmt(qkv, qkv_bias, heads * hd, fused=True, rel=relp)
    lib.call("mmsa_window_attention_planes", pq, ldq, _chk(qkv_bias.p, torch.int16), _chk(relp.p, torch.int16),
             _chk(window_selector(ws, qkv.p.device, f16=vf == 2), torch.int16), po, ldo, b, h, w, heads, hd, ws, scale, out.fmt,
             vf, _guard(max_logit), _stream())
    return out


def colstats(x, stride_b, b, hw, out, wrow=None, out_is_zero=False):
    px, _, c, ldx = _mat(x, "x")
    lib.call("mmsa_colstats", px, ldx, stride_b, _chk(wrow), b, hw, c, _chk(out, torch.float64), int(out_is_zero), _stream())
    return out


def ffrm_finalize(stats, b, hw, c, mean_w, mean_b, wc, gn_w, gn_b, mean_o, rstd_o, mult_o, scratch):
    lib.call("mmsa_ffrm_finalize", _chk(stats, torch.float64), b, hw, c, mean_w, mean_b, _chk(wc), _chk(gn_w), _chk(gn_b),
             _chk(mean_o), _chk(rstd_o), _chk(mult_o), _chk(scratch), _stream())


def lnhw_apply(x, mean, rstd, mult, w, bias, out, b, hw):
    px, _, c, ldx = _mat(x, "x")
    po, _, _, ldo = _mat(out, "y")
    lib.call("mmsa_lnhw_apply", px, ldx, _chk(mean), _chk(rstd), _chk(mult), _chk(w), _chk(bias), po, ldo, b, hw, c, _stream())
    return out


def dwconv(x, w, bias, out, b, h, wd, k, act="none", xstride_b=None, ystride_b=None, out_planes=None, pstride_b=None,
           imgs_per_group=0, rowstats_out=None):
    px, _, c, ldx = _mat(x, "x")
    po, ldo = None, 0
    if out is not None:
        po, _, _, ldo = _mat(out, "y")
    pp, ldp = None, 0
    if out_planes is not None:
        pp, _, _, ldp = out_planes.mat("y planes")
    xs = h * wd * ldx if xstride_b is None else xstride_b
    ys = h * wd * ldo if ystride_b is None else ystride_b
    ps = h * wd * ldp if pstride_b is None else pstride_b
    lib.call("mmsa_dwconv_nhwc", px, ldx, xs, _chk(w), _chk(bias), po, ldo, ys, pp, ldp, ps, out_planes.fmt if out_planes is not None else FMT_B3,
             b, h, wd, c, k, ACT[act], imgs_per_group, _chk(rowstats_out), _clamp_ptr(), _stream())
    return out if out is not None else out_planes


def gconv(x, w, bias, out, b, h, wd, groups, cin_g, cout_g, k, act="none"):
    px, _, _, ldx = _mat(x, "x")
    po, _, _, ldo = _mat(out, "y")
    lib.call("mmsa_gconv_nhwc", px, ldx, _chk(w), _chk(bias), po, ldo, b, h, wd, groups, cin_g, cout_g, k, ACT[act], _stream())


def gfe_qkv(x, w12, out, b, h, wd, groups, cin_g, cout_g):
    px, _, _, ldx = _mat(x, "x")
    po, _, _, ldo = _mat(out, "y")
    covered = ctypes.c_int(0)
    lib.call("mmsa_gfe_qkv_conv", px, ldx, _chk(w12), po, ldo, b, h, wd, groups, cin_g, cout_g, ctypes.byref(covered), _stream())
    return bool(covered.value)
    return out


def dwpair_gate(x, w_tap, out, b, h, wd, c, out_planes=None):
    px, _, _, ldx = _mat(x, "x")
    po, ldo = (None, 0)
    if out is not None:
        po, _, _, ldo = _mat(out, "y")
    pp, ldp = (None, 0)
    if out_planes is not None:
        pp, _, _, ldp = out_planes.mat("y planes")
    lib.call("mmsa_dwpair_gate", px, ldx, _chk(w_tap), po, ldo, pp, ldp, b, h, wd, c, _stream())
    return out if out is not None else out_planes


def im2col_nchw(x, c0, cin, p, out):
    b, ctot, h, w = x.shape
    if not x.is_contiguous():
        raise RuntimeError("mmsa.im2col_nchw: input image must be contiguous NCHW")
    po, _, kpad, ld = _mat(out, "out")
    if ld != kpad:
        raise RuntimeError("mmsa.im2col_nchw: output must be dense")
    lib.call("mmsa_im2col_nchw", _chk(x), b, ctot, c0, cin, h, w, p, po, kpad, _stream())
    return out


def gram_tn_scratch_bytes(b, p, c):
    return int(lib.raw.mmsa_gram_tn_scratch_bytes(b, p, c))


def gram_tn(x, y, stride_b, g, b, p, nblk=1, scratch=None):
    px, _, c, ldx = _mat(x, "X")
    py, _, _, ldy = _mat(y, "Y")
    need = gram_tn_scratch_bytes(b, p, c)
    if scratch is None:
        scratch = torch.empty((need + 3) // 4, dtype=torch.float32, device=x.device)
    if not scratch.is_cuda or not scratch.is_contiguous():
        raise RuntimeError("gram_tn: scratch must be a contiguous device tensor")
    lib.call("mmsa_gram_tn", px, ldx, py, ldy, stride_b, _chk(g, torch.float64, "G"), b, p, c, nblk, scratch.data_ptr(),
             scratch.numel() * scratch.element_size(), _stream())
    return g


def chanattn_build(g, sq, sq_stride, sk, sk_stride, temp, wp, planes, b, c, heads):
    lib.call("mmsa_chanattn_build", _chk(g, torch.float64, "G"), sq, sq_stride, sk, sk_stride, _chk(temp), _chk(wp),
             planes.p.data_ptr(), b, c, planes.kpad, heads, _stream())


def gffm_build(e, px_, py_, b, c):
    lib.call("mmsa_gffm_build", _chk(e, torch.float64, "E"), px_.p.data_ptr(), py_.p.data_ptr(), b, c, px_.kpad, _stream())


def gelu_gate(x, out, c):
    px, rows, _, ldx = _mat(x, "x")
    po, _, _, ldo = _mat(out, "y")
    lib.call("mmsa_gelu_gate", px, ldx, po, ldo, rows, c, _stream())
    return out


def pool_hw(z, out, b, h, w):
    pz, _, c, ldz = _mat(z, "z")
    po, _, _, ldo = _mat(out, "out")
    lib.call("mmsa_pool_hw", pz, ldz, po, ldo, b, h, w, c, _stream())
    return out


def ca_apply(z, att, out, b, h, w, out_planes=None):
    pz, _, c, ldz = _mat(z, "z")
    pa, _, _, lda = _mat(att, "att")
    po, ldo = (None, 0)
    if out is not None:
        po, _, _, ldo = _mat(out, "out")
    pp, ldp = (None, 0)
    if out_planes is not None:
        pp, _, _, ldp = out_planes.mat("out planes")
    lib.call("mmsa_ca_apply", pz, ldz, pa, lda, po, ldo, pp, ldp, b, h, w, c, _stream())
    return out if out is not None else out_planes


def tail_fuse(cmap, cstride_b, xtok, bn_scale, bn_shift, out, b, hc, wc, hx, wx, out_planes=None):
    pc, _, c, ldc = _mat(cmap, "cmap")
    px, ldx = None, 0
    if xtok is not None:
        px, _, _, ldx = _mat(xtok, "xtok")
    pp, ldp = (out_planes.p.data_ptr(), 2 * out_planes.kpad) if out_planes is not None else (None, 0)
    lib.call("mmsa_tail_fuse", pc, ldc, cstride_b, px, ldx, _chk(bn_scale), _chk(bn_shift), _chk(out), pp, ldp, b, hc, wc, hx, wx, c, _stream())
    return out
```

Measured before the change: 67.96.

## Add grouped GEMM launch for independent problems sharing K and formats

Adds a grouped GEMM entry point that packs up to four independent GEMM problems with the same K, format and activation into one persistent launch, with a per-tile cursor that maps global tile indices to problems. The MSDA value/offset projections and the Segformer head branch GEMMs now use it when eligible. The goal is to fill the GPU better and cut launch count for small GEMMs that alone underfill the CUs. The cost is extra per-tile problem lookup and a larger kernel parameter block.

```diff
diff --git a/include/mmsa.h b/include/mmsa.h
--- a/include/mmsa.h
+++ b/include/mmsa.h
@@ -62,6 +62,19 @@
                      int batch, int act, float alpha, int out_mode, int ps_H, int ps_W, int ps_C, int fmt, int cp_fmt,
                      int max_grid, float* rowstats_out, const float* rownorm_mean_rstd, const float* rownorm_colsum, int flavour,
                      float* clamp_max , mmsa_stream_t stream);
+
+typedef struct mmsa_gemm_problem {
+  const uint16_t* Ap; long lda;
+  const uint16_t* Wp;
+  const float* bias;
+  float* C; long ldc;
+  uint16_t* Cp; long ldcp;
+  int M, N, K;
+  int act, fmt, cp_fmt, out_mode;
+  const float* rowstats_out;
+  const float* rownorm_mean_rstd;
+} mmsa_gemm_problem;
+int mmsa_gemm_grouped(const mmsa_gemm_problem* problems, int count, int max_grid, int flavour, float* clamp_max, mmsa_stream_t stream);
 
 int mmsa_convnext_mlp_fused(const uint16_t* Ap, long lda, long strideA, const uint16_t* W1p, long strideW1, const uint16_t* W2p,
                             long strideW2, const float* b1, const float* b2, const float* gamma, float* x, long ldx, long strideX,
diff --git a/multimodal-sam-adapter_amd/csrc/gemm_h8c.hip b/multimodal-sam-adapter_amd/csrc/gemm_h8c.hip
--- a/multimodal-sam-adapter_amd/csrc/gemm_h8c.hip
+++ b/multimodal-sam-adapter_amd/csrc/gemm_h8c.hip
@@ -7,6 +7,9 @@
 #define HC_LDS_L(i_) (2 * HC_H_UNIT + (i_) * (HC_L_UNIT + 16384))
 #define HC_LDS_TOTAL (2 * HC_H_UNIT + 2 * HC_L_UNIT + 16384)
 
+#if V2_GROUPED
+#define gemm_h8c_kernel gemm_h8c_group_kernel
+#endif
 #ifdef HC_EPI_STAMP
 __device__ unsigned long long g_hc_estamps[8 * 16];
 extern "C" int mmsa_debug_epi_stamps(unsigned long long* host_out) { return (int)hipMemcpyFromSymbol(host_out, HIP_SYMBOL(g_hc_estamps), sizeof(g_hc_estamps)); }
@@ -17,7 +20,8 @@
 #define EPI_STAMP_WAIT()
 #endif
 template <bool GEN, int ACT>
-__global__ __launch_bounds__(512, 1) void gemm_h8c_kernel(GemmV2Args a) {
+__global__ __launch_bounds__(512, 1) void gemm_h8c_kernel(V2G_PARAM) {
+  V2G_PROLOGUE
   constexpr bool PP = true;
   constexpr bool EPI_UNROLL = ACT >= 0;
   constexpr int V2_BM = 256;
@@ -34,9 +38,9 @@
   const int G = gridDim.x;
   int rb = blockIdx.x;
   V2_XCD_REMAP(rb, G)
-  const int my_tiles = (a.ntiles - rb + G - 1) / G;
+  const int my_tiles = (V2G_BLOCK.ntiles - rb + G - 1) / G;
   if (my_tiles <= 0) return;
-  V2_SLACK_STAGGER(a, rb, G)
+  V2_SLACK_STAGGER(V2G_BLOCK, rb, G)
   const int total = my_tiles * np;
 
   H8C_DMA_LANE();
@@ -53,13 +57,14 @@
   int h_m0 = 0, h_n0 = 0, l_m0 = 0, l_n0 = 0;
   bool h_edge = false, l_edge = false;
   int hp_tile = rb, hp_p = 0, hp_j = 0, lp_tile = rb, lp_p = 0, lp_j = 0;
+  V2G_CURSOR(int h_pi = 0;) V2G_CURSOR(int l_pi = 0;)
 #define HC_SET_H(t_)                                                                                        \
-  { int bz_; H8C_TILE(t_, 256, bz_, h_m0, h_n0)                                                             \
+  { V2G_ENTER(t_, h_pi) int bz_; H8C_TILE(V2G_LOCAL(t_), 256, bz_, h_m0, h_n0)                              \
     hA = reinterpret_cast<const unsigned char*>(a.Ap + (long)bz_ * a.strideA + (long)(h_m0 >> 1) * a.lda);  \
     hW = reinterpret_cast<const unsigned char*>(a.Wp + (long)bz_ * a.strideW + (long)(h_n0 >> 1) * a.ldw);  \
     h_edge = h_m0 + 256 > a.M || h_n0 + 128 > a.N; }
 #define HC_SET_L(t_)                                                                                        \
-  { int bz_; H8C_TILE(t_, 256, bz_, l_m0, l_n0)                                                             \
+  { V2G_ENTER(t_, l_pi) int bz_; H8C_TILE(V2G_LOCAL(t_), 256, bz_, l_m0, l_n0)                              \
     lA = reinterpret_cast<const unsigned char*>(a.Ap + (long)bz_ * a.strideA + (long)(l_m0 >> 1) * a.lda);  \
     lW = reinterpret_cast<const unsigned char*>(a.Wp + (long)bz_ * a.strideW + (long)(l_n0 >> 1) * a.ldw);  \
     l_edge = l_m0 + 256 > a.M || l_n0 + 128 > a.N; }
@@ -77,7 +82,7 @@
     H8C_A_LO_FAST(sa_, d_)                                                                                  \
     GLDS16(sw_ + LLW, d_ + lds_lw); }
 #define HC_H_ISSUE()                                                                                        \
-  if (!h_edge) HC_H_ISSUE_FAST() else {                                                                     \
+  if (!h_edge) HC_H_ISSUE_FAST() else { V2G_AT(h_pi)                                                        \
     unsigned char* d_ = smem + HC_LDS_H(hp_j & 1); const long ko_ = (long)hp_p * 128;                       \
     const int ab_ = h_m0 + wave * 32 + drow, wb_ = h_n0 + wave * 16 + drow;                                  \
     H8C_A_HI_EDGE(hA + ko_, ab_, h_m0, d_)                                                                  \
@@ -85,7 +90,7 @@
     GLDS16(hW + ko_ + (unsigned long)(H8C_HOFF(min(wb_ + 8, a.N - 1), h_n0, ldwB) + (dpiece ^ 64)), d_ + lds_hw + 1024); }
 #define HC_H_ADVANCE() { ++hp_j; if (++hp_p == np) { hp_p = 0; hp_tile += G; if (hp_j < total) HC_SET_H(hp_tile) } }
 #define HC_L_ISSUE()                                                                                        \
-  if (!l_edge) HC_L_ISSUE_FAST() else {                                                                     \
+  if (!l_edge) HC_L_ISSUE_FAST() else { V2G_AT(l_pi)                                                        \
     unsigned char* d_ = smem + HC_LDS_L(lp_j & 1); const long ko_ = (long)lp_p * 128;                       \
     const int aj_ = (l_m0 >> 1) + wave * 16 + drow, wj_ = (l_n0 >> 1) + wave * 8 + drow;                     \
     GLDS16(lA + ko_ + (unsigned long)H8C_A_LO_OFF(aj_, l_m0), d_ + lds_la);                                  \
@@ -170,8 +175,9 @@
 
   for (int tdone = 0; tdone < my_tiles; ++tdone) {
     if (grp) H8C_BAR()
+    V2G_CURSOR(int c_pi;) V2G_ENTER(tile, c_pi)
     bool interior;
-    { int bz_, m0_, n0_; H8C_TILE(tile, 256, bz_, m0_, n0_) interior = m0_ + 256 <= a.M && n0_ + 128 <= a.N; }
+    { int bz_, m0_, n0_; H8C_TILE(V2G_LOCAL(tile), 256, bz_, m0_, n0_) interior = m0_ + 256 <= a.M && n0_ + 128 <= a.N; }
     int p = 0;
     HC_PAIR(0)
     ++p;
@@ -190,7 +196,9 @@
 #endif
       EPI_STAMP(0)
 #define EPI_STAGING_BASE (smem + (((j - 1) & 1) ? 2 * HC_H_UNIT + HC_L_UNIT : 2 * HC_H_UNIT))
+      V2G_EPI_OPEN(V2G_LOCAL(tile))
 #include "gemm_v2_epilogue.inc"
+      V2G_EPI_CLOSE
       EPI_STAMP(7)
 #ifdef HC_EPI_STAMP
       asm volatile("s_waitcnt lgkmcnt(0)" ::: "memory");
@@ -208,6 +216,21 @@
   }
 }
 
+#if V2_GROUPED
+int mmsa_gemm_h8c_group_dispatch(const GemmV2Group& ga, int grid, int act, hipStream_t stream) {
+  static MmsaPerDevice per_dev_ = {};
+  (void)mmsa_per_device(per_dev_, [] {
+#define HC_ATTR(GEN_, ACT_) (void)hipFuncSetAttribute((const void*)gemm_h8c_kernel<GEN_, ACT_>, hipFuncAttributeMaxDynamicSharedMemorySize, HC_LDS_TOTAL);
+    V2_GROUP_EPI_TABLE(HC_ATTR)
+#undef HC_ATTR
+  });
+#define HC_LAUNCH(GEN_, ACT_) if (v2_group_epi_serves(act, ACT_)) hipLaunchKernelGGL((gemm_h8c_kernel<GEN_, ACT_>), dim3(grid), dim3(512), HC_LDS_TOTAL, stream, ga);
+  V2_GROUP_EPI_TABLE(HC_LAUNCH)
+#undef HC_LAUNCH
+  MMSA_CHECK_LAUNCH("gemm_grouped(h8c)");
+  return MMSA_OK;
+}
+#else
 int mmsa_gemm_h8c_dispatch(const GemmV2Args& a, int grid, bool gen, int act, hipStream_t stream) {
   static MmsaPerDevice per_dev_ = {};
   (void)mmsa_per_device(per_dev_, [] {
@@ -221,3 +244,4 @@
   MMSA_CHECK_LAUNCH("gemm_split3(h8c)");
   return MMSA_OK;
 }
+#endif
diff --git a/multimodal-sam-adapter_amd/csrc/gemm_h8c_grouped.hip b/multimodal-sam-adapter_amd/csrc/gemm_h8c_grouped.hip
--- /dev/null
+++ b/multimodal-sam-adapter_amd/csrc/gemm_h8c_grouped.hip
@@ -0,0 +1,2 @@
+#define V2_GROUPED 1
+#include "gemm_h8c.hip"
diff --git a/multimodal-sam-adapter_amd/csrc/gemm_v2.hip b/multimodal-sam-adapter_amd/csrc/gemm_v2.hip
--- a/multimodal-sam-adapter_amd/csrc/gemm_v2.hip
+++ b/multimodal-sam-adapter_amd/csrc/gemm_v2.hip
@@ -1,7 +1,11 @@
 #include "common.h"
 #include "gemm_v2_shared.h"
+#if V2_GROUPED
+#define gemm_v2_kernel gemm_v2_group_kernel
+#endif
 template <bool GEN, int ACT, bool PP, int NW, int FMT>
-__global__ __launch_bounds__(NW * 64, NW == 4 ? 2 : 1) void gemm_v2_kernel(GemmV2Args a) {
+__global__ __launch_bounds__(NW * 64, NW == 4 ? 2 : 1) void gemm_v2_kernel(V2G_PARAM) {
+  V2G_PROLOGUE
   static_assert(NW == 8 || (NW == 4 && !PP), "4-wave workgroups run the in-phase main loop");
   static_assert(FMT == MMSA_FMT_B3 || (PP && NW == 8), "the h8 and f3 operand formats run on the ping-pong kernel");
   constexpr bool EPI_UNROLL = ACT >= 0;
@@ -24,9 +28,9 @@
   const int G = gridDim.x;
   int rb = blockIdx.x;
   V2_XCD_REMAP(rb, G)
-  const int my_tiles = (a.ntiles - rb + G - 1) / G;
+  const int my_tiles = (V2G_BLOCK.ntiles - rb + G - 1) / G;
   if (my_tiles <= 0) return;
-  V2_SLACK_STAGGER(a, rb, G)
+  V2_SLACK_STAGGER(V2G_BLOCK, rb, G)
   CLK_SAMPLE(0)
   const int total = my_tiles * nk;
 
@@ -41,7 +45,8 @@
 
 #define SET_TILE_SRC(tile_)                                                      \
   do {                                                                           \
-    const int t_ = (tile_);                                                      \
+    V2G_CURSOR(int pi_;) V2G_ENTER(tile_, pi_)                                   \
+    const int t_ = V2G_LOCAL((tile_));                                           \
     const int per_b_ = a.nbm * a.nbn;                                            \
     const int bz_ = t_ / per_b_;                                                 \
     const int r_ = t_ - bz_ * per_b_;                                            \
@@ -360,6 +365,7 @@
 #endif
 
   for (int tdone = 0; tdone < my_tiles; ++tdone) {
+    V2G_CURSOR(int c_pi;) V2G_ENTER(tile, c_pi)
     if constexpr (PP) {
       if (grp) __builtin_amdgcn_s_barrier();
       const bool fast_ok = V2_FAST_STEPS && nk >= 6 && (V2_DBG(a) < 3 || V2_DBG(a) == 10 || V2_DBG(a) >= 64) && (FMT != MMSA_FMT_H8 || ni4);
@@ -430,7 +436,9 @@
 
     if (V2_DBG(a) == 2 || V2_DBG(a) == 5 || V2_DBG(a) >= 64) { tile += G; continue; }
 #define EPI_STAGING_BASE (smem + st_cur * V2_STAGE)
+    V2G_EPI_OPEN(V2G_LOCAL(tile))
 #include "gemm_v2_epilogue.inc"
+    V2G_EPI_CLOSE
     if constexpr (PP) {
       asm volatile("s_waitcnt lgkmcnt(0)" ::: "memory");
       __builtin_amdgcn_s_barrier();
@@ -447,6 +455,20 @@
 #undef MFMA_FP8_ALL
 }
 
+static void v2_tile_order(GemmV2Args& a) {
+  const bool rowmajor = MMSA_KNOB("MMSA_GEMM_ROWMAJOR", 0) != 0;
+  a.tm = a.tn = 0;
+  if (rowmajor) return;
+  double best = 0.0;
+  for (int tn = 1; tn <= 32; tn <<= 1) {
+    const int tm = 32 / tn;
+    if (a.nbn % tn != 0 || a.nbm % tm != 0) continue;
+    const double cost = (double)(a.nbn / tn) * a.M + (double)(a.nbm / tm) * a.N;
+    if (a.tm == 0 || cost < best) { best = cost; a.tm = tm; a.tn = tn; }
+  }
+}
+
+#if !V2_GROUPED
 int mmsa_gemm_h8c_dispatch(const GemmV2Args& a, int grid, bool gen, int act, hipStream_t stream);
 int mmsa_gemm_h8c_w8_dispatch(const GemmV2Args& a, int grid, bool gen, int act, hipStream_t stream);
 int mmsa_gemm_stream_try(const unsigned short* Ap, long lda, const unsigned short* Wp, const float* bias, const float* colscale, const float* resid, long ldr, float beta,
@@ -529,17 +551,7 @@
       a.ntiles = (int)t96;
     }
   }
-  const bool rowmajor = MMSA_KNOB("MMSA_GEMM_ROWMAJOR", 0) != 0;
-  a.tm = a.tn = 0;
-  if (!rowmajor) {
-    double best = 0.0;
-    for (int tn = 1; tn <= 32; tn <<= 1) {
-      const int tm = 32 / tn;
-      if (a.nbn % tn != 0 || a.nbm % tm != 0) continue;
-      const double cost = (double)(a.nbn / tn) * M + (double)(a.nbm / tm) * N;
-      if (a.tm == 0 || cost < best) { best = cost; a.tm = tm; a.tn = tn; }
-    }
-  }
+  v2_tile_order(a);
   const int slots_ = cus * wg_per_cu;
   const int rounds_ = cdiv(a.ntiles, slots_);
   int grid = cdiv(a.ntiles, rounds_);
@@ -569,3 +581,94 @@
   MMSA_CHECK_LAUNCH("gemm_split3(v2)");
   return MMSA_OK;
 }
+#else
+int mmsa_gemm_h8c_group_dispatch(const GemmV2Group& ga, int grid, int act, hipStream_t stream);
+
+extern "C" int mmsa_gemm_grouped(const mmsa_gemm_problem* problems, int count, int max_grid, int flavour, float* clamp_max, hipStream_t stream) {
+  MMSA_CHECK_ARG(problems && count >= 1 && count <= V2_GROUP_MAX, "gemm_grouped: 1..%d problems (count=%d)", V2_GROUP_MAX, count);
+  MMSA_CHECK_ARG(flavour == 0 || flavour == 4 || flavour == 8, "gemm_grouped: flavour %d (0 = by shape, 4, 8)", flavour);
+  const mmsa_gemm_problem& p0 = problems[0];
+  for (int i = 0; i < count; ++i) {
+    const mmsa_gemm_problem& p = problems[i];
+    MMSA_CHECK_ARG(!p.rowstats_out, "gemm_grouped: problem %d writes row statistics: that epilogue is not grouped", i);
+    MMSA_CHECK_ARG(!p.rownorm_mean_rstd, "gemm_grouped: problem %d has a row-normalising epilogue: not grouped", i);
+    MMSA_CHECK_ARG(p.out_mode == 0, "gemm_grouped: problem %d has a pixel-shuffle store (out_mode=%d): not grouped", i, p.out_mode);
+    MMSA_CHECK_ARG(p.fmt != MMSA_FMT_W8, "gemm_grouped: problem %d has fp8 (W8) weights: not grouped", i);
+    MMSA_CHECK_ARG(p.K == p0.K, "gemm_grouped: different K (problem %d: %d, problem 0: %d)", i, p.K, p0.K);
+    MMSA_CHECK_ARG(p.fmt == p0.fmt && p.cp_fmt == p0.cp_fmt, "gemm_grouped: different formats (problem %d: operands %d / output %d, problem 0: %d / %d)", i, p.fmt, p.cp_fmt, p0.fmt, p0.cp_fmt);
+    MMSA_CHECK_ARG(p.act == p0.act, "gemm_grouped: different activations (problem %d: %d, problem 0: %d)", i, p.act, p0.act);
+    MMSA_CHECK_ARG(!p.C == !p0.C && !p.Cp == !p0.Cp, "gemm_grouped: different output kinds (fp32 rows / planes) in problem %d", i);
+  }
+  const int K = p0.K, act = p0.act, fmt = p0.fmt, cp_fmt = p0.cp_fmt;
+  const bool h8c = fmt == MMSA_FMT_H8C, cp_h8c = MMSA_CP_BASE(cp_fmt) == MMSA_FMT_H8C;
+  MMSA_CHECK_ARG(fmt == MMSA_FMT_B3 || h8c, "gemm_grouped: operand format %d (bf16 hi/lo or h8c planes)", fmt);
+  MMSA_CHECK_ARG(cp_fmt >= 0 && MMSA_CP_SPLIT(cp_fmt) == 0 && MMSA_CP_BASE(cp_fmt) >= MMSA_FMT_B3 && MMSA_CP_BASE(cp_fmt) <= MMSA_FMT_F3, "gemm_grouped: bad output plane format %d", cp_fmt);
+  MMSA_CHECK_ARG(K > 0 && K % (h8c ? 64 : V2_BK) == 0, "gemm_grouped: K=%d must be a multiple of %d", K, h8c ? 64 : V2_BK);
+  MMSA_CHECK_ARG(act >= ACT_NONE && act <= ACT_SIGMOID, "gemm_grouped: bad act %d", act);
+  for (int i = 0; i < count; ++i) {
+    const mmsa_gemm_problem& p = problems[i];
+    MMSA_CHECK_ARG(p.Ap && p.Wp && (p.C || p.Cp), "gemm_grouped: null pointer in problem %d", i);
+    MMSA_CHECK_ARG(p.M > 0 && p.N > 0, "gemm_grouped: bad shape M=%d N=%d in problem %d", p.M, p.N, i);
+    MMSA_CHECK_ARG(h8c || p.M >= 128, "gemm_grouped: bf16 hi/lo problems need M >= 128 (problem %d: M=%d runs on another kernel alone)", i, p.M);
+    MMSA_CHECK_ARG((p.lda & 63) == 0 && (((uintptr_t)p.Ap) & 127) == 0 && p.lda >= (h8c ? 3L : 2L) * K, "gemm_grouped: A planes of problem %d must be 128-byte aligned with lda%%64==0, lda=%ld >= %d*K", i, p.lda, h8c ? 3 : 2);
+    MMSA_CHECK_ARG(!h8c || p.lda == p0.lda, "gemm_grouped: h8c problems share one lda (problem %d: %ld, problem 0: %ld)", i, p.lda, p0.lda);
+    MMSA_CHECK_ARG((((uintptr_t)p.Wp) & 127) == 0, "gemm_grouped: weight planes of problem %d must be 128-byte aligned", i);
+    MMSA_CHECK_ARG(!p.C || ((((uintptr_t)p.C) & 15) == 0 && p.ldc >= p.N), "gemm_grouped: C of problem %d must be 16-byte aligned with ldc=%ld >= N=%d", i, p.ldc, p.N);
+    MMSA_CHECK_ARG(!p.Cp || ((((uintptr_t)p.Cp) & 127) == 0 && (p.ldcp & 63) == 0 && p.ldcp >= (cp_h8c ? 3L * MMSA_PAD64(p.N) : 2L * ((p.N + 31) / 32 * 32))),
+                   "gemm_grouped: output planes of problem %d must be 128-byte aligned, ldcp%%64==0, ldcp=%ld wide enough for N=%d", i, p.ldcp, p.N);
+  }
+  const int nw = h8c ? 8 : flavour ? flavour : (K <= MMSA_KNOB("MMSA_GEMM_NW4_MAXK", 256) && max_grid <= 0 ? 4 : 8);
+  MMSA_CHECK_ARG(!h8c || flavour != 4, "gemm_grouped: the 4-wave h8c kernel is not grouped (flavour 0 or 8)");
+  const int bm = nw * 32, wg_per_cu = nw == 4 ? 2 : 1;
+  int order[V2_GROUP_MAX], tiles[V2_GROUP_MAX];
+  for (int i = 0; i < count; ++i) { order[i] = i; tiles[i] = cdiv(problems[i].M, bm) * cdiv(problems[i].N, V2_BN); }
+  for (int i = 1; i < count; ++i)
+    for (int j = i; j > 0 && tiles[order[j]] > tiles[order[j - 1]]; --j) { const int t = order[j]; order[j] = order[j - 1]; order[j - 1] = t; }
+  GemmV2Group ga = {};
+  long total = 0;
+  for (int s = 0; s < V2_GROUP_MAX; ++s) {
+    ga.tstart[s] = 0x7fffffff;
+    if (s >= count) continue;
+    const mmsa_gemm_problem& p = problems[order[s]];
+    GemmV2Args& a = ga.p[s];
+    a.Ap = p.Ap; a.lda = p.lda; a.Wp = p.Wp; a.ldw = h8c ? 3L * K : 2L * K;
+    a.bias = p.bias;
+    a.C = p.C; a.ldc = p.C ? p.ldc : 0;
+    a.Cp = p.Cp; a.ldcp = p.Cp ? p.ldcp : 0;
+    a.M = p.M; a.N = p.N; a.K = K; a.act = act; a.alpha = 1.0f; a.beta = 1.0f;
+    a.ps_sw = a.ps_sh = -1;
+    a.cp_fmt = cp_fmt; a.rs_strips = p.N >> 6; a.clamp_max = clamp_max;
+    a.nbm = cdiv(p.M, bm); a.bn = V2_BN; a.nbn = cdiv(p.N, V2_BN); a.ntiles = a.nbm * a.nbn;
+#ifdef MMSA_DEBUG_KNOBS
+    a.debug = MMSA_KNOB("MMSA_GEMM_DEBUG", 0);
+#endif
+    v2_tile_order(a);
+    ga.tstart[s] = (int)total;
+    total += a.ntiles;
+  }
+  MMSA_CHECK_ARG(total < 0x7fffffffL, "gemm_grouped: too many tiles");
+  ga.ntiles = (int)total;
+  static MmsaPerDevice per_dev_ = {};
+  const int num_cus = mmsa_per_device(per_dev_, [] {
+#define V2_ATTR(GEN_, ACT_)                                                                                                   \
+  (void)hipFuncSetAttribute((const void*)gemm_v2_kernel<GEN_, ACT_, true, 8, MMSA_FMT_B3>, hipFuncAttributeMaxDynamicSharedMemorySize, V2_LDS_BYTES(8)); \
+  (void)hipFuncSetAttribute((const void*)gemm_v2_kernel<GEN_, ACT_, false, 4, MMSA_FMT_B3>, hipFuncAttributeMaxDynamicSharedMemorySize, V2_LDS_BYTES(4));
+    V2_GROUP_EPI_TABLE(V2_ATTR)
+#undef V2_ATTR
+  });
+  const int cus = (max_grid > 0 && max_grid < num_cus) ? max_grid : num_cus;
+  const int slots = cus * wg_per_cu;
+  const int rounds = cdiv(ga.ntiles, slots);
+  const int grid = cdiv(ga.ntiles, rounds);
+  if (h8c) return mmsa_gemm_h8c_group_dispatch(ga, grid, act, stream);
+#define V2_LAUNCH(GEN_, ACT_)                                                                                              \
+  if (v2_group_epi_serves(act, ACT_)) {                                                                                    \
+    if (nw == 4) hipLaunchKernelGGL((gemm_v2_kernel<GEN_, ACT_, false, 4, MMSA_FMT_B3>), dim3(grid), dim3(256), V2_LDS_BYTES(4), stream, ga);    \
+    else hipLaunchKernelGGL((gemm_v2_kernel<GEN_, ACT_, true, 8, MMSA_FMT_B3>), dim3(grid), dim3(512), V2_LDS_BYTES(8), stream, ga);            \
+  }
+  V2_GROUP_EPI_TABLE(V2_LAUNCH)
+#undef V2_LAUNCH
+  MMSA_CHECK_LAUNCH("gemm_grouped(v2)");
+  return MMSA_OK;
+}
+#endif
diff --git a/multimodal-sam-adapter_amd/csrc/gemm_v2_grouped.hip b/multimodal-sam-adapter_amd/csrc/gemm_v2_grouped.hip
--- /dev/null
+++ b/multimodal-sam-adapter_amd/csrc/gemm_v2_grouped.hip
@@ -0,0 +1,2 @@
+#define V2_GROUPED 1
+#include "gemm_v2.hip"
diff --git a/multimodal-sam-adapter_amd/csrc/gemm_v2_shared.h b/multimodal-sam-adapter_amd/csrc/gemm_v2_shared.h
--- a/multimodal-sam-adapter_amd/csrc/gemm_v2_shared.h
+++ b/multimodal-sam-adapter_amd/csrc/gemm_v2_shared.h
@@ -32,6 +32,43 @@
 #define V2_DBG(a_) ((a_).debug)
 #else
 #define V2_DBG(a_) 0
+#endif
+
+#define V2_GROUP_MAX 4
+struct GemmV2Group {
+  GemmV2Args p[V2_GROUP_MAX];
+  int tstart[V2_GROUP_MAX];
+  int ntiles;
+  int stagger;
+};
+#ifndef V2_GROUPED
+#define V2_GROUPED 0
+#endif
+#if V2_GROUPED
+__device__ __forceinline__ int v2_group_find(const GemmV2Group& g, int t, int& local) {
+  const int i = (t >= g.tstart[1] ? 1 : 0) + (t >= g.tstart[2] ? 1 : 0) + (t >= g.tstart[3] ? 1 : 0);
+  local = t - g.tstart[i];
+  return i;
+}
+#define V2G_PARAM GemmV2Group ga
+#define V2G_PROLOGUE const GemmV2Args& a = ga.p[0];
+#define V2G_BLOCK ga
+#define V2G_CURSOR(decl_) decl_
+#define V2G_ENTER(t_, pi_) int lt_; pi_ = v2_group_find(ga, (t_), lt_); const GemmV2Args& a = ga.p[pi_];
+#define V2G_LOCAL(t_) lt_
+#define V2G_AT(pi_) const GemmV2Args& a = ga.p[pi_];
+#define V2G_EPI_OPEN(lt_) { const int tile = (lt_);
+#define V2G_EPI_CLOSE }
+#else
+#define V2G_PARAM GemmV2Args a
+#define V2G_PROLOGUE
+#define V2G_BLOCK a
+#define V2G_CURSOR(decl_)
+#define V2G_ENTER(t_, pi_)
+#define V2G_LOCAL(t_) t_
+#define V2G_AT(pi_)
+#define V2G_EPI_OPEN(lt_)
+#define V2G_EPI_CLOSE
 #endif
 
 #define V2_BN 128
@@ -85,6 +122,9 @@
   return gen == GEN && (listed ? act == ACT : ACT == -1);
 }
 
+#define V2_GROUP_EPI_TABLE(X_) X_(false, ACT_NONE) X_(false, ACT_GELU) X_(false, ACT_RELU) X_(false, -1)
+inline bool v2_group_epi_serves(int act, int ACT) { return v2_epi_serves(false, act, false, ACT); }
+
 #define V2_TILE_MN(r_, mi_, ni_)                                                 \
   do {                                                                           \
     if (a.tm > 0) {                                                              \
diff --git a/multimodal-sam-adapter_amd/mmsa/backbone.py b/multimodal-sam-adapter_amd/mmsa/backbone.py
--- a/multimodal-sam-adapter_amd/mmsa/backbone.py
+++ b/multimodal-sam-adapter_amd/mmsa/backbone.py
@@ -592,11 +592,18 @@
         if vmode in ("f16", "f16lo") and not self._wide() and (dv // M) % 8 == 0 and dv % 32 == 0:
             val = ws.planes("msda_valp", B * S, dv, fmt=ops.FMT_H8)
             ops.gemm(fn, ap["val"], bias=ap["val_b"], row_norm=f_rn, out_planes=val)
+            grouped = False
         else:
             val = ws.get("msda_val", B * S, dv)
-            ops.gemm(fn, ap["val"], val, bias=ap["val_b"], row_norm=f_rn)
+            grouped = (getattr(self, "group_gemms", True) and f_rn is None and q_rn is None and ap["val"].fmt == ap["oa"].fmt
+                       and ap["val"].fmt in (ops.FMT_B3, ops.FMT_H8C) and fn.p.stride(0) == qn.p.stride(0) and min(B * S, B * Lq) >= 128)
+            if not grouped:
+                ops.gemm(fn, ap["val"], val, bias=ap["val_b"], row_norm=f_rn)
         raw = ws.get("msda_raw", B * Lq, ap["oa"].n)
-        ops.gemm(qn, ap["oa"], raw, bias=ap["oa_b"], row_norm=q_rn)
+        if grouped:
+            ops.gemm_grouped([dict(a=fn, w=ap["val"], out=val, bias=ap["val_b"]), dict(a=qn, w=ap["oa"], out=raw, bias=ap["oa_b"])])
+        else:
+            ops.gemm(qn, ap["oa"], raw, bias=ap["oa_b"], row_norm=q_rn)
         samp = ws.planes("msda_s", B * Lq, dv, fmt=ap["out"].fmt)
         ops.msda_fused(val, ss, lsi, raw, ref, None, B, S, M, dv // M, L, Lq, Pn, out_planes=samp, lo_bytes=vmode == "f16lo")
         if stream_out is not None:
diff --git a/multimodal-sam-adapter_amd/mmsa/head.py b/multimodal-sam-adapter_amd/mmsa/head.py
--- a/multimodal-sam-adapter_amd/mmsa/head.py
+++ b/multimodal-sam-adapter_amd/mmsa/head.py
@@ -125,7 +125,7 @@
         pk = self._packed
         B, _, H, W = x0.shape
         ch = self.channels
-        zs = []
+        zs, g1, g2 = [], [], []
         for i, (x, ci) in enumerate(zip(xs, self.in_channels)):
             if x.dtype != torch.float32 or x.dim() != 4 or x.shape[0] != B or x.shape[1] != ci:
                 raise RuntimeError(f"mmsa SegformerHead: input {i} must be fp32 [B={B}, {ci}, h, w], got {tuple(x.shape)} {x.dtype}")
@@ -138,10 +138,19 @@
                 lib.call("mmsa_nchw_to_planes", x.data_ptr(), ci * h * w, xp.p.data_ptr(), 2 * xp.kpad, B, ci, h * w, ops._stream())
             br = pk["branch"][i]
             yp = self._planes(f"y{i}", rows, ch, dev)
-            ops.gemm(xp, br["w"], bias=br["shift"], act="relu", out_planes=yp)
             z = self._buf(f"z{i}", (rows, ch), dev=dev)
-            ops.gemm(yp, br["wf"], z)
+            g1.append(dict(a=xp, w=br["w"], bias=br["shift"], act="relu", out_planes=yp))
+            g2.append(dict(a=yp, w=br["wf"], out=z))
             zs.append((z, h, w))
+        for grp in (g1, g2):
+            big = [q for q in grp if q["a"].n >= 128]
+            if not (getattr(self, "group_gemms", True) and 1 < len(big) <= ops.GROUP_MAX and len({q["w"].kpad for q in big}) == 1):
+                big = []
+            if big:
+                ops.gemm_grouped(big)
+            for q in grp:
+                if not any(q is b for b in big):
+                    ops.gemm(q["a"], q["w"], q.get("out"), bias=q.get("bias"), act=q.get("act", "none"), out_planes=q.get("out_planes"))
         fp = self._planes("fused", B * H * W, ch, dev)
         lv = zs[1:] + [(None, 0, 0)] * (4 - len(zs))
         lib.call("mmsa_head_fuse", zs[0][0].data_ptr(),
diff --git a/multimodal-sam-adapter_amd/mmsa/lib.py b/multimodal-sam-adapter_amd/mmsa/lib.py
--- a/multimodal-sam-adapter_amd/mmsa/lib.py
+++ b/multimodal-sam-adapter_amd/mmsa/lib.py
@@ -32,6 +32,7 @@
     "mmsa_msda_fused": [P, P, P, P, L, P, P, L, P, L, I, I, I, I, I, I, I, I, P, P],
     "mmsa_msda_fused_planes": [P, L, I, P, P, P, L, P, P, L, P, L, I, I, I, I, I, I, I, I, P, P],
     "mmsa_gemm_split3": [P, P, L, L, P, L, P, L, P, P, L, L, I, F, P, L, L, P, L, L, I, I, I, I, I, F, I, I, I, I, I, I, I, P, P, P, I, P, P],
+    "mmsa_gemm_grouped": [P, I, I, I, P, P],
     "mmsa_convnext_mlp_fused": [P, L, L, P, L, P, L, P, P, P, P, L, L, I, I, I, I, I, P, P],
     "mmsa_rowstats_finalize": [P, I, I, I, F, P, P],
     "mmsa_zero_bytes": [P, ctypes.c_size_t, P],
@@ -90,6 +91,14 @@
     "mmsa_render_u8": [P, L, L, I, I, I, P, I, I, P, I, I, I, c_double, c_double, P, P],
     "mmsa_render_denorm_f32": [P, L, L, I, I, I, P, I, I, P, I, I, I, P, P, I, I, c_double, c_double, P, P],
 }
+
+
+class GemmProblem(ctypes.Structure):
+    _fields_ = [("Ap", P), ("lda", L), ("Wp", P), ("bias", P), ("C", P), ("ldc", L), ("Cp", P), ("ldcp", L),
+                ("M", I), ("N", I), ("K", I), ("act", I), ("fmt", I), ("cp_fmt", I), ("out_mode", I),
+                ("rowstats_out", P), ("rownorm_mean_rstd", P)]
+
+
 _RESTYPES = {"mmsa_last_error": c_char_p, "mmsa_gram_tn_scratch_bytes": c_long}
 
 for _name, _args in SIGNATURES.items():
diff --git a/multimodal-sam-adapter_amd/mmsa/ops.py b/multimodal-sam-adapter_amd/mmsa/ops.py
--- a/multimodal-sam-adapter_amd/mmsa/ops.py
+++ b/multimodal-sam-adapter_amd/mmsa/ops.py
@@ -325,6 +325,54 @@
     return out if out is not None else out_planes
 
 
+GROUP_MAX = 4
+
+
+def gemm_grouped(problems):
+    if not 1 <= len(problems) <= GROUP_MAX:
+        raise RuntimeError(f"mmsa.gemm_grouped: 1..{GROUP_MAX} problems, got {len(problems)}")
+    known = {"a", "w", "out", "bias", "act", "out_planes", "rowstats_out", "row_norm", "pixel_shuffle", "m"}
+    arr = (lib.GemmProblem * len(problems))()
+    flops = by = 0.0
+    for i, (q, pr) in enumerate(zip(arr, problems)):
+        extra = set(pr) - known
+        if extra:
+            raise RuntimeError(f"mmsa.gemm_grouped: problem {i}: {sorted(extra)} cannot be grouped (no residual, column scale, alpha or batch stride in a grouped launch)")
+        a, w, out, out_planes = pr["a"], pr["w"], pr.get("out"), pr.get("out_planes")
+        if not isinstance(a, Planes):
+            raise RuntimeError(f"mmsa.gemm_grouped: problem {i}: A must come as activation Planes")
+        pap, ma, ka, lda = a.mat("A")
+        if ka < w.kpad:
+            raise RuntimeError(f"mmsa.gemm_grouped: problem {i}: A planes have {ka} columns but the packed weight expects K={w.kpad}")
+        if a.fmt != w.afmt or a.weight or (w.fmt == FMT_H8 and not w.weight) or (w.fmt == FMT_H8C and w.weight):
+            raise RuntimeError(f"mmsa.gemm_grouped: problem {i}: operand formats differ (A fmt {a.fmt}, W fmt {w.fmt} weight={w.weight})")
+        q.Ap, q.lda, q.Wp, q.bias = pap, lda, w.p.data_ptr(), _chk(pr.get("bias"), name="bias")
+        if out is not None:
+            q.C, _, _, q.ldc = _mat(out, "C")
+        if out_planes is not None:
+            q.Cp, _, _, q.ldcp = out_planes.mat("Cplanes")
+        q.M, q.N, q.K = (ma if pr.get("m") is None else pr["m"]), w.n, w.kpad
+        q.act, q.fmt, q.cp_fmt = ACT[pr.get("act", "none")], w.fmt, cp_format(out_planes)
+        q.out_mode = 1 if pr.get("pixel_shuffle") else 0
+        q.rowstats_out = _chk(pr.get("rowstats_out"))
+        q.rownorm_mean_rstd = _chk(pr["row_norm"][0]) if pr.get("row_norm") else None
+        ob = 3.0 if w.fmt in (FMT_H8C, FMT_W8) else 4.0
+        pb = 0.0 if out_planes is None else (3.0 if out_planes.fmt == FMT_H8C else 4.0)
+        flops += 2.0 * q.M * w.n * w.k
+        by += ob * q.M * w.kpad + ob * w.n * w.kpad + q.M * w.n * (pb + (4.0 if out is not None else 0.0))
+    prof = GEMM_PROFILE
+    if prof is not None:
+        e0, e1 = _event(), _event()
+        lib.call("mmsa_event_record", e0, _stream())
+    lib.call("mmsa_gemm_grouped", arr, len(problems), GEMM_MAX_GRID, GEMM_FLAVOUR, _clamp_ptr(), _stream())
+    if prof is not None:
+        lib.call("mmsa_event_record", e1, _stream())
+        prof.append((flops, e0, e1, by))
+        if GEMM_SHAPES is not None:
+            GEMM_SHAPES.append((sum(q.M for q in arr), arr[0].N, arr[0].K, len(problems), problems[0].get("act", "none"), False,
+                                ("C" if problems[0].get("out") is not None else "") + ("P" if problems[0].get("out_planes") is not None else ""), "grouped"))
+
+
 def convnext_mlp_fused(a, w1, w2, b1, b2, gamma, x, m, batch=1, stride_a=0, stride_w1=0, stride_w2=0, stride_x=0):
     pa, _, _, lda = a.mat("A")
     px, _, c, ldx = _mat(x, "x")
```

New measurement: 68.54 (median of 6 runs). Within noise of the previous version (+0.9%).
